# deevinandu/Distributed-Multi-Agent-SLAM-Swarm-Robotics-System

Measured on NVIDIA B200. Metric: beam_cell_updates_per_sec, higher is better.
Workload: dtype f64+u32

## Files before the change

distributed-multi-agent-slam-swarm-robotics-system_b200/_native.py:

```python
from __future__ import annotations

import ctypes as C
import os
import subprocess

PKG_DIR = os.path.dirname(os.path.abspath(__file__))
CSRC = os.path.join(PKG_DIR, 'csrc')
LIB_PATH = os.path.join(PKG_DIR, 'liboccgrid_b200.so')
SOURCES = ['occgrid_integrate.cu', 'occgrid_tiled.cu', 'occgrid_route.cu', 'occgrid_band.cu', 'mapmerge.cu', 'frontier.cu', 'icp.cu', 'render.cu', 'map_fuse.cu', 'frontier_assign.cu', 'slam_chain.cpp']
HEADERS = ['common.cuh', 'beam_expand.cuh', 'block_ops.cuh', 'sincos_dd.cuh', os.path.join('..', '..', 'include', 'occgrid_b200.h')]

STRATEGY = {'auto': -1, 'global_atomic': 0, 'tiled': 1}
COUNTER_NAMES = ('packets', 'accepted', 'dropped', 'bad_pose', 'beams', 'hits', 'updates', 'slowpath',
                 'owned_updates', 'records')
N_COUNTERS = 16


class OccGridError(RuntimeError):
    pass


class Geom(C.Structure):
    _fields_ = [('ox', C.c_double), ('oy', C.c_double), ('res', C.c_double),
                ('size_x', C.c_int32), ('size_y', C.c_int32),
                ('win_x0', C.c_int32), ('win_y0', C.c_int32),
                ('win_w', C.c_int32), ('win_h', C.c_int32)]


class RouteJob(C.Structure):
    _fields_ = [('d_packets', C.c_void_p), ('n', C.c_int64), ('stride', C.c_int32), ('rec_len', C.c_int32),
                ('d_agent_idx', C.c_void_p), ('d_drift', C.c_void_p), ('d_agent_off', C.c_void_p), ('n_agents', C.c_int32),
                ('ordinal_base', C.c_uint32), ('ox', C.c_double), ('oy', C.c_double), ('res', C.c_double),
                ('size_x', C.c_int32), ('n_bands', C.c_int32), ('src_rank', C.c_int32), ('band_y0', C.c_int32 * 33),
                ('d_peer_recs', C.c_void_p), ('d_peer_tiles', C.c_void_p), ('seg_capacity', C.c_int64), ('d_resv', C.c_void_p), ('d_status', C.c_void_p),
                ('d_counters', C.c_void_p)]


class BandCtx(C.Structure):
    _fields_ = [('band_geom', Geom), ('n_bands', C.c_int32), ('rank', C.c_int32), ('seg_capacity', C.c_int64),
                ('d_recv', C.c_void_p * 2), ('d_recv_tiles', C.c_void_p * 2), ('d_seg_counts', C.c_void_p * 2),
                ('d_peer_recs', C.c_void_p * 2), ('d_peer_tiles', C.c_void_p * 2), ('d_peer_seg_counts', C.c_void_p * 2),
                ('d_peer_flags', C.c_void_p), ('d_my_flags', C.c_void_p), ('d_resv', C.c_void_p), ('d_status', C.c_void_p),
                ('d_grid', C.c_void_p), ('d_workspace', C.c_void_p), ('workspace_bytes', C.c_size_t), ('d_counters', C.c_void_p),
                ('ev_fused', C.c_void_p), ('ev_published', C.c_void_p), ('published_pending', C.c_int32)]


def _stale():
    if not os.path.exists(LIB_PATH):
        return True
    t = os.path.getmtime(LIB_PATH)
    deps = [os.path.join(CSRC, s) for s in SOURCES + HEADERS]
    return any(os.path.exists(d) and os.path.getmtime(d) > t for d in deps)


def build(force=False, verbose=False):
    if not force and not _stale():
        return LIB_PATH
    srcs = [os.path.join(CSRC, s) for s in SOURCES if os.path.exists(os.path.join(CSRC, s))]
    cmd = ['nvcc', '-gencode', 'arch=compute_100a,code=sm_100a', '-O3', '-lineinfo', '-std=c++17',
           '-Xcompiler', '-fPIC', '-Xcompiler', '-ffp-contract=off', '-shared', '-o', LIB_PATH] + srcs
    if verbose:
        cmd.insert(1, '-Xptxas=-v')
    r = subprocess.run(cmd, capture_output=True, text=True)
    if r.returncode != 0:
        raise OccGridError('nvcc failed:\n' + r.stdout + r.stderr)
    if verbose:
        print(r.stderr)
    return LIB_PATH


_lib = None


def lib():
    global _lib
    if _lib is not None:
        return _lib
    if not os.path.exists(LIB_PATH):
        raise OccGridError(f'{LIB_PATH} is missing: run `python -c "import __graft_entry__ as g; g.build()"` '
                           '(needs nvcc).  There is no CPU fallback.')
    L = C.CDLL(LIB_PATH)
    vp, i64, i32, u32, sz = C.c_void_p, C.c_int64, C.c_int, C.c_uint32, C.c_size_t
    gp = C.POINTER(Geom)
    L.occgrid_abi_version.restype = i32
    L.occgrid_last_error.restype = C.c_char_p
    L.occgrid_workspace_bytes.restype = sz
    L.occgrid_workspace_bytes.argtypes = [gp, i64, i32]
    L.occgrid_workspace_reset.restype = i32
    L.occgrid_workspace_reset.argtypes = [vp, sz, vp]
    L.occgrid_integrate_packets.restype = i32
    L.occgrid_integrate_packets.argtypes = [gp, vp, i64, i32, i32, vp, vp, vp, i32, vp, vp, sz, vp, i32, vp]
    L.occgrid_agent_maps_workspace_bytes.restype = sz
    L.occgrid_agent_maps_workspace_bytes.argtypes = [gp, i32, i64, i32]
    L.occgrid_integrate_packets_agent_maps.restype = i32
    L.occgrid_integrate_packets_agent_maps.argtypes = [gp, vp, i64, i32, i32, vp, vp, vp, i32, vp, vp, sz, vp, i32, vp]
    L.occgrid_update_rays.restype = i32
    L.occgrid_update_rays.argtypes = [gp, vp, vp, i64, vp, vp, sz, vp, i32, vp]
    L.occgrid_scatter_probe.restype = i32
    L.occgrid_scatter_probe.argtypes = [i32, vp, i64, i64, u32, vp]
    L.occgrid_route_workspace_bytes.restype = sz
    L.occgrid_route_workspace_bytes.argtypes = [i64, i32]
    L.occgrid_route_packets.restype = i32
    L.occgrid_route_packets.argtypes = [gp, i32, vp, vp, i64, i32, i32, vp, vp, vp, i32, vp, i64, vp, vp, vp,
                                        vp, sz, vp]
    L.occgrid_integrate_poses.restype = i32
    L.occgrid_integrate_poses.argtypes = [gp, vp, i64, i32, vp, vp, sz, vp, i32, vp]
    L.occgrid_band_workspace_bytes.restype = sz
    L.occgrid_band_workspace_bytes.argtypes = [gp, i32, i64]
    L.occgrid_band_prepare.restype = i32
    L.occgrid_band_prepare.argtypes = [gp, vp, vp, i32, i64, vp, vp, sz, vp, vp]
    L.occgrid_band_raycast_route.restype = i32
    L.occgrid_band_raycast_route.argtypes = [gp, vp, i32, i64, i32, C.POINTER(RouteJob), vp, vp, sz, vp, vp]
    L.occgrid_band_step.restype = i32
    L.occgrid_band_step.argtypes = [C.POINTER(BandCtx), i64, i32, C.POINTER(RouteJob), i32, vp, vp]
    L.occgrid_band_join.restype = i32
    L.occgrid_band_join.argtypes = [C.POINTER(BandCtx), vp]
    L.occgrid_band_publish.restype = i32
    L.occgrid_band_publish.argtypes = [i32, i32, vp, i64, vp, vp, vp, u32, i32, vp, vp]
    L.occgrid_frontier_workspace_bytes.restype = sz
    L.occgrid_frontier_workspace_bytes.argtypes = [i64, i64]
    L.occgrid_frontiers.restype = i32
    L.occgrid_frontiers.argtypes = [vp, i32, i32, vp, i64, vp, vp, vp, sz, vp]
    L.occgrid_frontier_clusters.restype = i32
    L.occgrid_frontier_clusters.argtypes = [vp, vp, i64, i32, i32, C.c_double, C.c_double, C.c_double, vp, vp, vp, vp, vp,
                                            vp, sz, vp]
    L.occgrid_render_overlay.restype = i32
    L.occgrid_render_overlay.argtypes = [vp, i32, i32, C.c_double, C.c_double, C.c_double, C.c_double, C.c_double, C.c_double,
                                         i32, i32, vp, vp, vp, vp]
    L.occgrid_set_raycast_ctas_per_sm.restype = i32
    L.occgrid_set_raycast_ctas_per_sm.argtypes = [i32]
    L.occgrid_profile_begin.restype = i32
    L.occgrid_profile_end.restype = i32
    L.occgrid_profile_end.argtypes = [vp, vp, i32]
    _bind_merge(L)
    _lib = L
    return L


def _bind_merge(L):
    vp, i64, i32, sz, dbl = C.c_void_p, C.c_int64, C.c_int32, C.c_size_t, C.c_double
    L.mapmerge_count_occupied.restype = C.c_int
    L.mapmerge_count_occupied.argtypes = [vp, i64, vp, vp]
    L.mapmerge_extract_workspace_bytes.restype = sz
    L.mapmerge_extract_workspace_bytes.argtypes = [i64]
    L.mapmerge_extract_transform.restype = C.c_int
    L.mapmerge_extract_transform.argtypes = [vp, i32, i32, dbl, dbl, dbl, vp, vp, vp, i64, vp, vp, vp, vp, sz, vp]
    L.mapmerge_extract_batch_workspace_bytes.restype = sz
    L.mapmerge_extract_batch_workspace_bytes.argtypes = [i64, i32]
    L.mapmerge_extract_batch_count.restype = C.c_int
    L.mapmerge_extract_batch_count.argtypes = [vp, i32, i32, i32, vp, vp, sz, i32, vp]
    L.mapmerge_extract_batch_write.restype = C.c_int
    L.mapmerge_extract_batch_write.argtypes = [vp, i32, i32, i32, dbl, vp, vp, vp, vp, vp, vp, i64, vp, vp, vp, vp, sz, vp]
    L.mapmerge_append_slice.restype = C.c_int
    L.mapmerge_append_slice.argtypes = [vp, vp, vp, i32, vp, vp, i64, vp, vp, vp, vp]
    L.mapmerge_bounds_workspace_bytes.restype = sz
    L.mapmerge_bounds.restype = C.c_int
    L.mapmerge_bounds.argtypes = [vp, vp, vp, vp, vp, sz, vp]
    L.mapmerge_voxel_workspace_bytes.restype = sz
    L.mapmerge_voxel_workspace_bytes.argtypes = [i64, i64]
    L.mapmerge_voxel_downsample.restype = C.c_int
    L.mapmerge_voxel_downsample.argtypes = [vp, vp, vp, i64, dbl, vp, vp, i64, vp, vp, vp, vp, vp, sz, vp]
    L.mapmerge_bounds_enc_reset.restype = C.c_int
    L.mapmerge_bounds_enc_reset.argtypes = [vp, vp]
    L.mapmerge_chain_workspace_bytes.restype = sz
    L.mapmerge_chain_workspace_bytes.argtypes = [vp, i32]
    L.mapmerge_chain_init.restype = C.c_int
    L.mapmerge_chain_init.argtypes = [vp, sz, vp, i32, vp, vp, vp, vp, i32, vp, vp, vp, vp]
    L.mapmerge_chain_run.restype = C.c_int
    L.mapmerge_chain_run.argtypes = [vp, vp, i32, i32, i32, vp, vp, vp, dbl, vp, vp, i64, vp, vp, vp]
    L.mapmerge_chain_poll.restype = C.c_int
    L.mapmerge_chain_poll.argtypes = [vp, vp, i32, vp, vp]
    L.mapmerge_chain_rebounds.restype = C.c_int
    L.mapmerge_chain_rebounds.argtypes = [vp, vp, i32, vp, vp, vp, vp]
    L.mapmerge_chain_rebuild.restype = C.c_int
    L.mapmerge_chain_rebuild.argtypes = [vp, vp, i32, vp, vp, vp, i32, dbl, vp, vp, i64, vp, vp, vp, vp, vp, vp, sz, i64, vp]
    L.mapmerge_icp_workspace_bytes.restype = sz
    L.mapmerge_icp_workspace_bytes.argtypes = [i64, i64, i32, i32]
    L.mapmerge_icp_register.restype = C.c_int
    L.mapmerge_icp_register.argtypes = [vp, vp, i64, vp, vp, i64, dbl, dbl, dbl, i32, i32, dbl, i32, dbl, dbl, vp, vp, sz, vp]
    L.occgrid_slam_create.restype = vp
    L.occgrid_slam_create.argtypes = []
    L.occgrid_slam_destroy.restype = None
    L.occgrid_slam_destroy.argtypes = [vp]
    L.occgrid_slam_drift_table.restype = C.c_int
    L.occgrid_slam_drift_table.argtypes = [vp, vp, i64, i32, i32, vp, dbl, vp]
    L.occgrid_slam_counts.restype = C.c_int
    L.occgrid_slam_counts.argtypes = [vp, vp, vp, vp]
    L.occgrid_slam_closures.restype = C.c_int
    L.occgrid_slam_closures.argtypes = [vp, i64, vp, vp, vp, vp]
    L.occgrid_slam_correction_for_agent.restype = C.c_int
    L.occgrid_slam_correction_for_agent.argtypes = [vp, i32, vp]
    L.occgrid_accumulate_packets.restype = C.c_int
    L.occgrid_accumulate_packets.argtypes = [C.POINTER(Geom), vp, i64, i32, i32, vp, vp, vp, i32, vp, vp, sz, vp, i32, vp]
    L.occgrid_counts_to_logodds.restype = C.c_int
    L.occgrid_counts_to_logodds.argtypes = [vp, i64, dbl, dbl, dbl, dbl, vp, vp]
    L.mapmerge_rasterise.restype = C.c_int
    L.mapmerge_rasterise.argtypes = [vp, vp, vp, dbl, vp, i32, i32, vp, vp]
    L.mapmerge_fuse_max.restype = C.c_int
    L.mapmerge_fuse_max.argtypes = [vp, vp, i64, vp]
    L.mapmerge_warp_fuse_workspace_bytes.restype = sz
    L.mapmerge_warp_fuse_workspace_bytes.argtypes = [C.c_int, i32, i32]
    L.mapmerge_warp_fuse.restype = C.c_int
    L.mapmerge_warp_fuse.argtypes = [vp, C.c_int, i32, i32, dbl, vp, vp, dbl, dbl, dbl, i32, i32, vp, vp, sz, vp]
    L.occgrid_frontier_assign_workspace_bytes.restype = sz
    L.occgrid_frontier_assign_workspace_bytes.argtypes = [i32, i32, i32, i32, i64]
    L.occgrid_frontier_assign.restype = C.c_int
    L.occgrid_frontier_assign.argtypes = [vp, i32, i32, dbl, dbl, dbl, vp, i32, vp, vp, vp, vp, vp, vp, i32, i64,
                                          vp, vp, vp, vp, vp, vp, vp, vp, sz, vp]
    L.occgrid_geodesic_field.restype = C.c_int
    L.occgrid_geodesic_field.argtypes = [vp, i32, i32, dbl, dbl, dbl, vp, i64, vp, vp, vp, vp, sz, vp]


KERNEL_NAMES = ('integrate_global', 'resolve', 'update_rays', 'tile_count', 'tile_scan', 'tile_scatter',
                'tile_raycast', 'tile_resolve', 'merge_extract', 'merge_bounds', 'merge_voxel', 'merge_raster',
                'merge_fuse', 'probe', 'route', 'frontier', 'frontier_cluster', 'chain_probe', 'chain_incremental',
                'chain_rebuild', 'icp', 'band_barrier', 'render', 'merge_scan', 'merge_warp_fuse', 'frontier_assign')


def profile_begin():
    check(lib().occgrid_profile_begin(), 'occgrid_profile_begin')


def profile_end():
    n = len(KERNEL_NAMES)
    ms = (C.c_double * n)()
    cnt = (C.c_int64 * n)()
    check(lib().occgrid_profile_end(ms, cnt, n), 'occgrid_profile_end')
    return {KERNEL_NAMES[i]: (ms[i], cnt[i]) for i in range(n) if cnt[i]}


def check(rc, what):
    if rc != 0:
        msg = lib().occgrid_last_error().decode('utf-8', 'replace')
        raise OccGridError(f'{what} failed (rc={rc}): {msg}')


def last_error():
    return lib().occgrid_last_error().decode('utf-8', 'replace')
```

distributed-multi-agent-slam-swarm-robotics-system_b200/csrc/common.cuh:

```cuda
#pragma once
#include <cuda_runtime.h>
#include <stdarg.h>
#include <stdint.h>
#include <stdio.h>

#include "../../include/occgrid_b200.h"
#include "beam_expand.cuh"
#include "block_ops.cuh"

namespace occ {

void set_last_error(const char* fmt, ...);
bool cuda_ok(cudaError_t e, const char* what);

#define OCC_CUDA_TRY(call)                                  \
    do {                                                    \
        if (!occ::cuda_ok((call), #call)) return OCCGRID_E_CUDA; \
    } while (0)

inline Geom to_geom(const occgrid_geom* g) {
    Geom o;
    o.ox = g->ox; o.oy = g->oy; o.res = g->res; o.inv_res = 1.0 / g->res;
    o.size_x = g->size_x; o.size_y = g->size_y;
    o.win_x0 = g->win_x0; o.win_y0 = g->win_y0; o.win_w = g->win_w; o.win_h = g->win_h;
    return o;
}

int validate_geom(const occgrid_geom* g);

int device_sm_count();

struct __align__(16) PoseRec {
    double rx, ry;
    float yaw;
    float d[4];
    unsigned int k;
    int tile;
    unsigned int pad;
};
static_assert(sizeof(PoseRec) == 48, "PoseRec must be 48 bytes");

enum KernelId { K_INTEGRATE_GLOBAL = 0, K_RESOLVE, K_UPDATE_RAYS, K_TILE_COUNT, K_TILE_SCAN, K_TILE_SCATTER,
                K_TILE_RAYCAST, K_TILE_RESOLVE, K_MERGE_EXTRACT, K_MERGE_BOUNDS, K_MERGE_VOXEL, K_MERGE_RASTER,
                K_MERGE_FUSE, K_PROBE, K_ROUTE, K_FRONTIER, K_FRONTIER_CLUSTER, K_CHAIN_PROBE, K_CHAIN_INCR,
                K_CHAIN_REBUILD, K_ICP, K_BAND_BARRIER, K_RENDER, K_MERGE_SCAN, K_MERGE_WARP_FUSE, K_FRONTIER_ASSIGN, K_N_KERNELS };
bool profile_enabled();
void profile_mark(int kernel_id, cudaStream_t st, bool begin, int n_kernels);

struct ProfileScope {
    int id; cudaStream_t st; bool on; int nk;
    ProfileScope(int id_, cudaStream_t st_, int n_kernels = 1) : id(id_), st(st_), on(profile_enabled()), nk(n_kernels) {
        if (on) profile_mark(id, st, true, nk);
    }
    ~ProfileScope() { if (on) profile_mark(id, st, false, nk); }
};

inline size_t align_up(size_t v, size_t a) { return (v + a - 1) / a * a; }

constexpr int kMaxRecStride = 64;

struct PacketBatch {
    const uint8_t* pkts; int64_t n; int stride;
    const int32_t* agent_idx; const double* drift; const double* agent_off; int n_agents;
};

enum class Output { kGrid, kAgentMaps, kCounts };

int check_packet_batch(const PacketBatch& b, int rec_len, const char* who);

__device__ __forceinline__ void stage_records(const uint8_t* __restrict__ src, size_t bytes, uint8_t* smem) {
    const size_t nvec = ((reinterpret_cast<uintptr_t>(src) & 15) == 0) ? bytes / 16 : 0;
    const uint4* s4 = reinterpret_cast<const uint4*>(src);
    uint4* d4 = reinterpret_cast<uint4*>(smem);
    for (size_t i = threadIdx.x; i < nvec; i += blockDim.x) d4[i] = __ldg(s4 + i);
    for (size_t i = nvec * 16 + threadIdx.x; i < bytes; i += blockDim.x) smem[i] = __ldg(src + i);
}

constexpr int kTile = 64;
constexpr int kTileShift = 6;

__host__ __device__ __forceinline__ int reach_cells(double res) { return (int)ceil(OCC_MAX_DIST_M / res) + 2; }

struct TileGeom {
    int reach;
    int pad;
    int tiles_x, tiles_y, n_tiles;
    int win_side;
    int pitch;
};

inline TileGeom tile_geom(double res, int win_w, int win_h) {
    TileGeom t;
    t.reach = reach_cells(res);
    t.pad = ((t.reach + kTile - 1) / kTile) * kTile;
    t.tiles_x = (win_w + 2 * t.pad + kTile - 1) >> kTileShift;
    t.tiles_y = (win_h + 2 * t.pad + kTile - 1) >> kTileShift;
    t.n_tiles = t.tiles_x * t.tiles_y;
    t.win_side = kTile + 2 * t.reach;
    t.pitch = t.win_side | 1;
    return t;
}
inline TileGeom tile_geom(const occgrid_geom* g) { return tile_geom(g->res, g->win_w, g->win_h); }

constexpr int kSegChunk = 2048;
constexpr int kRouteItemPk = 512;
constexpr int kRouteSubsPerItem = 2;
constexpr int kMaxBands = 32;

struct SegInfo {
    int n_segs;
    unsigned int seg_cap;
    const unsigned int* d_counts;
    unsigned int host_count;
};

struct RouteJob {
    const uint8_t* pkts; long long n; int stride;
    const int32_t* agent_idx; const double* drift; const double* agent_off; int n_agents;
    unsigned int ordinal_base;
    double ox, oy, res, inv_res;
    int size_x;
    int reach, pad, tiles_x;
    int n_bands, src_rank;
    int band_y0[kMaxBands + 1];
    PoseRec* const* peer_recs;
    int* const* peer_tiles;
    unsigned int seg_cap;
    unsigned int* resv;
    int* status;
    uint64_t* counters;
    unsigned int n_route_items;
};

bool tiled_supported(const occgrid_geom* geom, int n_maps);
size_t tiled_workspace_bytes(const occgrid_geom* geom, int n_maps, int64_t max_packets);
int integrate_tiled(const occgrid_geom* geom, const PacketBatch& batch, const PoseRec* d_poses, int ordinals_in_records, Output kind,
                    void* d_out, void* d_ws, size_t ws_bytes, uint64_t* d_counters, cudaStream_t st);
void set_raycast_cta_cap(int cap);
size_t tiled_band_workspace_bytes(const occgrid_geom* geom, int n_segs, int64_t seg_cap);
int tiled_prepare_poses(const occgrid_geom* geom, const PoseRec* d_recs, const int* d_tiles, const SegInfo& seg, int tiles_in_records,
                        void* d_ws, size_t ws_bytes, uint64_t* d_counters, cudaStream_t st);
int tiled_raycast_route(const occgrid_geom* geom, const PoseRec* d_recs, int have_items, const RouteJob* job,
                        int8_t* d_grid, void* d_ws, size_t ws_bytes, int64_t max_records, uint64_t* d_counters, cudaStream_t st,
                        cudaEvent_t after_fused = nullptr);

template <int N>
__device__ __forceinline__ void block_add_counters(const unsigned long long (&v)[N],
                                                   unsigned long long* smem_acc , uint64_t* d_counters) {
    if (d_counters == nullptr) return;
    const int lane = threadIdx.x & 31, warp = threadIdx.x >> 5, nwarps = (blockDim.x + 31) >> 5;
#pragma unroll
    for (int i = 0; i < N; ++i) {
        unsigned long long x = v[i];
#pragma unroll
        for (int o = 16; o > 0; o >>= 1) x += __shfl_xor_sync(0xffffffffu, x, o);
        if (lane == 0) smem_acc[i * 32 + warp] = x;
    }
    __syncthreads();
    if (threadIdx.x < N) {
        unsigned long long t = 0;
        for (int w = 0; w < nwarps; ++w) t += smem_acc[threadIdx.x * 32 + w];
        if (t) atomicAdd(reinterpret_cast<unsigned long long*>(d_counters) + threadIdx.x, t);
    }
}

}
```

distributed-multi-agent-slam-swarm-robotics-system_b200/csrc/mapmerge.cu:

```cuda
#include <cstddef>
#include <vector>

#include "common.cuh"

namespace occ {

constexpr int kMT = 256;
constexpr int kLoadCells = 16;
constexpr int kCellsPerThread = 64;
constexpr int kChunk = kMT * kCellsPerThread;

enum { ST_POINT_OVERFLOW = 1, ST_LATTICE_OVERFLOW = 2, ST_CHAIN_ABORTED = 4 };

struct Xform { double m[16]; int identity; };


__device__ __forceinline__ unsigned int occupied_mask16(const int8_t* __restrict__ grid, long long base, long long n) {
    unsigned int mask = 0;
    if (base + 16 <= n && ((reinterpret_cast<uintptr_t>(grid + base) & 15) == 0)) {
        const int4 v = __ldg(reinterpret_cast<const int4*>(grid + base));
        const int w[4] = {v.x, v.y, v.z, v.w};
#pragma unroll
        for (int i = 0; i < 4; ++i)
#pragma unroll
            for (int b = 0; b < 4; ++b)
                if ((int8_t)((w[i] >> (8 * b)) & 0xff) > 50) mask |= 1u << (4 * i + b);
    } else {
        for (int i = 0; i < 16 && base + i < n; ++i)
            if (grid[base + i] > 50) mask |= 1u << i;
    }
    return mask;
}

__device__ __forceinline__ unsigned long long occupied_mask64(const int8_t* __restrict__ grid, long long base, long long n) {
    unsigned int m[4];
#pragma unroll
    for (int q = 0; q < 4; ++q) m[q] = occupied_mask16(grid, base + 16 * q, n);
    return (unsigned long long)m[0] | ((unsigned long long)m[1] << 16) | ((unsigned long long)m[2] << 32) |
           ((unsigned long long)m[3] << 48);
}

__global__ void __launch_bounds__(kMT)
k_extract_count(const int8_t* __restrict__ grid, long long n_cells, unsigned int* __restrict__ block_counts) {
    __shared__ unsigned int s_warp[33];
    const long long base = ((long long)blockIdx.x * kMT + threadIdx.x) * kCellsPerThread;
    unsigned int c = base < n_cells ? __popcll(occupied_mask64(grid, base, n_cells)) : 0u;
    unsigned int total;
    block_exclusive_scan(c, s_warp, &total);
    if (threadIdx.x == 0) block_counts[blockIdx.x] = total;
}

__global__ void __launch_bounds__(kMT)
k_count_occupied(const int8_t* __restrict__ grid, long long n_cells, long long* __restrict__ out) {
    unsigned int c = 0;
    for (long long base = ((long long)blockIdx.x * kMT + threadIdx.x) * kLoadCells; base < n_cells;
         base += (long long)gridDim.x * kMT * kLoadCells)
        c += __popc(occupied_mask16(grid, base, n_cells));
#pragma unroll
    for (int o = 16; o > 0; o >>= 1) c += __shfl_xor_sync(0xffffffffu, c, o);
    if ((threadIdx.x & 31) == 0 && c) atomicAdd(reinterpret_cast<unsigned long long*>(out), (unsigned long long)c);
}

__global__ void __launch_bounds__(1024)
k_extract_reserve(unsigned int* __restrict__ block_counts, int n_blocks, long long* __restrict__ d_count,
                  long long capacity, long long* __restrict__ ws_base, int* __restrict__ status,
                  long long* __restrict__ d_last_appended) {
    const unsigned long long sum = cta_scan_in_place<1>(block_counts, n_blocks, 0ull);
    if (threadIdx.x == 0) {
        const long long base = *d_count;
        long long total = (long long)sum;
        if (base + total > capacity) { atomicOr(status, ST_POINT_OVERFLOW); total = 0; }
        ws_base[0] = base;
        ws_base[1] = total;
        *d_count = base + total;
        if (d_last_appended) *d_last_appended = total;
    }
}

__global__ void __launch_bounds__(kMT)
k_extract_write(const int8_t* __restrict__ grid, long long n_cells, int width, double res, double origin_x,
                double origin_y, Xform T, const unsigned int* __restrict__ block_offsets,
                const long long* __restrict__ ws_base, double* __restrict__ px, double* __restrict__ py) {
    __shared__ unsigned int s_warp[33];
    if (ws_base[1] == 0) return;
    const long long base = ((long long)blockIdx.x * kMT + threadIdx.x) * kCellsPerThread;
    const unsigned long long mask = base < n_cells ? occupied_mask64(grid, base, n_cells) : 0ull;
    unsigned int total;
    unsigned int off = block_exclusive_scan(__popcll(mask), s_warp, &total);
    long long dst = ws_base[0] + block_offsets[blockIdx.x] + off;
    unsigned long long m = mask;
    while (m) {
        const int i = __ffsll((long long)m) - 1;
        m &= m - 1;
        const long long c = base + i;
        const long long row = c / width, col = c - row * width;
        double x = OCC_DADD(OCC_DMUL((double)col, res), origin_x);
        double y = OCC_DADD(OCC_DMUL((double)row, res), origin_y);
        if (!T.identity) {
            const double w = OCC_DADD(OCC_DADD(OCC_DMUL(T.m[12], x), OCC_DMUL(T.m[13], y)), T.m[15]);
            const double tx = OCC_DADD(OCC_DADD(OCC_DMUL(T.m[0], x), OCC_DMUL(T.m[1], y)), T.m[3]);
            const double ty = OCC_DADD(OCC_DADD(OCC_DMUL(T.m[4], x), OCC_DMUL(T.m[5], y)), T.m[7]);
            if (w == 1.0) { x = tx; y = ty; }
            else { x = OCC_DDIV(tx, w); y = OCC_DDIV(ty, w); }
        }
        px[dst] = x;
        py[dst] = y;
        ++dst;
    }
}

__device__ __forceinline__ double warp_min(double v) {
#pragma unroll
    for (int o = 16; o > 0; o >>= 1) v = fmin(v, __shfl_xor_sync(0xffffffffu, v, o));
    return v;
}
__device__ __forceinline__ double warp_max(double v) {
#pragma unroll
    for (int o = 16; o > 0; o >>= 1) v = fmax(v, __shfl_xor_sync(0xffffffffu, v, o));
    return v;
}

template <class F>
__device__ __forceinline__ void block_min_max(double mnx, double mny, double mxx, double mxy, F&& use) {
    __shared__ double s_b[4][32];
    mnx = warp_min(mnx); mny = warp_min(mny); mxx = warp_max(mxx); mxy = warp_max(mxy);
    const int lane = threadIdx.x & 31, warp = threadIdx.x >> 5;
    if (lane == 0) { s_b[0][warp] = mnx; s_b[1][warp] = mny; s_b[2][warp] = mxx; s_b[3][warp] = mxy; }
    __syncthreads();
    if (threadIdx.x == 0) {
        for (int w = 1; w < (int)(blockDim.x >> 5); ++w) {
            mnx = fmin(mnx, s_b[0][w]); mny = fmin(mny, s_b[1][w]); mxx = fmax(mxx, s_b[2][w]); mxy = fmax(mxy, s_b[3][w]);
        }
        use(mnx, mny, mxx, mxy);
    }
}

__device__ __forceinline__ unsigned long long enc_double(double d) {
    const unsigned long long u = (unsigned long long)__double_as_longlong(d);
    return (u & 0x8000000000000000ull) ? ~u : (u | 0x8000000000000000ull);
}
__device__ __forceinline__ double dec_double(unsigned long long k) {
    const unsigned long long u = (k & 0x8000000000000000ull) ? (k & 0x7fffffffffffffffull) : ~k;
    return __longlong_as_double((long long)u);
}

__device__ __forceinline__ void block_bounds_atomic(double mnx, double mny, double mxx, double mxy,
                                                    unsigned long long* __restrict__ benc) {
    block_min_max(mnx, mny, mxx, mxy, [&](double x0, double y0, double x1, double y1) {
        if (x0 <= x1) {
            atomicMin(&benc[0], enc_double(x0)); atomicMin(&benc[1], enc_double(y0));
            atomicMax(&benc[2], enc_double(x1)); atomicMax(&benc[3], enc_double(y1));
        }
    });
}

__global__ void k_benc_reset(unsigned long long* __restrict__ benc) {
    benc[0] = benc[1] = enc_double(INFINITY);
    benc[2] = benc[3] = enc_double(-INFINITY);
}

struct BatchXform { double m[6]; double w[3]; int identity; int use; };

__global__ void __launch_bounds__(kMT)
k_batch_count(const int8_t* const* __restrict__ grids, long long n_cells, int blocks_per_grid,
              unsigned int* __restrict__ block_counts ,
              unsigned long long* __restrict__ masks ) {
    __shared__ unsigned int s_warp[33];
    const int a = blockIdx.y;
    const long long base = ((long long)blockIdx.x * kMT + threadIdx.x) * kCellsPerThread;
    const unsigned long long mask = base < n_cells ? occupied_mask64(grids[a], base, n_cells) : 0ull;
    masks[((size_t)a * blocks_per_grid + blockIdx.x) * kMT + threadIdx.x] = mask;
    unsigned int total;
    block_exclusive_scan(__popcll(mask), s_warp, &total);
    if (threadIdx.x == 0) block_counts[(size_t)a * blocks_per_grid + blockIdx.x] = total;
}

constexpr int kScanStages = 4;
constexpr int kScanCtasPerSm = 3;
constexpr int kScanStageBytes = kChunk;

__device__ __forceinline__ unsigned int smem_u32(const void* p) { return (unsigned int)__cvta_generic_to_shared(p); }

__device__ __forceinline__ void mbar_init(unsigned long long* bar, unsigned int count) {
    asm volatile("mbarrier.init.shared::cta.b64 [%0], %1;" ::"r"(smem_u32(bar)), "r"(count) : "memory");
}
__device__ __forceinline__ void mbar_expect_tx(unsigned long long* bar, unsigned int bytes) {
    asm volatile("mbarrier.arrive.expect_tx.shared::cta.b64 _, [%0], %1;" ::"r"(smem_u32(bar)), "r"(bytes) : "memory");
}
__device__ __forceinline__ void mbar_wait(unsigned long long* bar, unsigned int parity) {
    asm volatile(
        "{\n\t.reg .pred p;\n\t"
        "WAIT_%=:\n\t"
        "mbarrier.try_wait.parity.shared::cta.b64 p, [%0], %1;\n\t"
        "@p bra DONE_%=;\n\t"
        "bra WAIT_%=;\n\t"
        "DONE_%=:\n\t}" ::"r"(smem_u32(bar)), "r"(parity) : "memory");
}
__device__ __forceinline__ void bulk_load(void* smem_dst, const void* gmem_src, unsigned int bytes, unsigned long long* bar) {
    asm volatile("cp.async.bulk.shared::cluster.global.mbarrier::complete_tx::bytes [%0], [%1], %2, [%3];"
                 ::"r"(smem_u32(smem_dst)), "l"(gmem_src), "r"(bytes), "r"(smem_u32(bar)) : "memory");
}

__device__ __forceinline__ unsigned int occupied_bits16(uint4 v) {
    const unsigned int w[4] = {v.x, v.y, v.z, v.w};
    unsigned int bits = 0;
#pragma unroll
    for (int i = 0; i < 4; ++i) {
        const unsigned int gt = __vcmpgts4(w[i], 0x32323232u) & 0x80808080u;
        bits |= (((gt >> 7) * 0x00204081u) >> 21 & 0xfu) << (4 * i);
    }
    return bits;
}

__global__ void __launch_bounds__(kMT)
k_batch_count_tma(const int8_t* const* __restrict__ grids, long long n_cells, int blocks_per_grid, int n_agents,
                  unsigned int* __restrict__ block_counts, unsigned long long* __restrict__ masks) {
    extern __shared__ __align__(128) unsigned char s_stage[];
    __shared__ __align__(8) unsigned long long s_full[kScanStages];
    __shared__ unsigned int s_cnt[kScanStages];
    const long long total = (long long)n_agents * blocks_per_grid;
    auto chunk_of = [&](long long i) { return (long long)blockIdx.x + i * gridDim.x; };
    auto issue = [&](long long i) {
        const long long c = chunk_of(i);
        if (c >= total) return;
        const int a = (int)(c / blocks_per_grid), blk = (int)(c - (long long)a * blocks_per_grid);
        const long long base = (long long)blk * kChunk;
        const unsigned int bytes = (unsigned int)min((long long)kChunk, n_cells - base);
        const int st = (int)(i % kScanStages);
        mbar_expect_tx(&s_full[st], bytes);
        bulk_load(s_stage + (size_t)st * kScanStageBytes, grids[a] + base, bytes, &s_full[st]);
    };
    if (threadIdx.x == 0) {
        for (int s = 0; s < kScanStages; ++s) mbar_init(&s_full[s], 1);
        asm volatile("fence.mbarrier_init.release.cluster;" ::: "memory");
        asm volatile("fence.proxy.async.shared::cta;" ::: "memory");
    }
    if (threadIdx.x < kScanStages) s_cnt[threadIdx.x] = 0u;
    __syncthreads();
    if (threadIdx.x == 0)
        for (int i = 0; i < kScanStages; ++i) issue(i);
    for (long long i = 0; chunk_of(i) < total; ++i) {
        const long long c = chunk_of(i);
        const int st = (int)(i % kScanStages);
        const int a = (int)(c / blocks_per_grid), blk = (int)(c - (long long)a * blocks_per_grid);
        const long long base = (long long)blk * kChunk;
        const int valid = (int)min((long long)kChunk, n_cells - base);
        mbar_wait(&s_full[st], (unsigned int)((i / kScanStages) & 1));
        const uint4* src = reinterpret_cast<const uint4*>(s_stage + (size_t)st * kScanStageBytes) + threadIdx.x * 4;
        unsigned long long mask = 0ull;
#pragma unroll
        for (int q = 0; q < 4; ++q)
            if ((int)threadIdx.x * kCellsPerThread + 16 * q < valid)
                mask |= (unsigned long long)occupied_bits16(src[q]) << (16 * q);
        masks[((size_t)a * blocks_per_grid + blk) * kMT + threadIdx.x] = mask;
        unsigned int n = __popcll(mask);
#pragma unroll
        for (int o = 16; o > 0; o >>= 1) n += __shfl_xor_sync(0xffffffffu, n, o);
        if ((threadIdx.x & 31) == 0 && n) atomicAdd(&s_cnt[st], n);
        __syncthreads();
        if (threadIdx.x == 0) {
            block_counts[(size_t)a * blocks_per_grid + blk] = s_cnt[st];
            s_cnt[st] = 0u;
            issue(i + kScanStages);
        }
    }
}

__global__ void __launch_bounds__(1024)
k_batch_scan(unsigned int* __restrict__ block_counts, int blocks_per_grid, long long* __restrict__ agent_total) {
    const unsigned long long total = cta_scan_in_place<1>(block_counts + (size_t)blockIdx.x * blocks_per_grid, blocks_per_grid, 0ull);
    if (threadIdx.x == 0) agent_total[blockIdx.x] = (long long)total;
}

__global__ void __launch_bounds__(1024)
k_batch_offsets(const long long* __restrict__ agent_total, const BatchXform* __restrict__ T, int n_agents,
                long long capacity, long long* __restrict__ agent_offset, int* __restrict__ status) {
    __shared__ unsigned long long s_warp[33];
    __shared__ long long s_carry;
    if (threadIdx.x == 0) s_carry = 0;
    __syncthreads();
    for (int start = 0; start < n_agents; start += blockDim.x) {
        const int a = start + threadIdx.x;
        const unsigned long long v = (a < n_agents && T[a].use) ? (unsigned long long)agent_total[a] : 0ull;
        unsigned long long total;
        const unsigned long long ex = block_exclusive_scan(v, s_warp, &total);
        if (a < n_agents) agent_offset[a] = s_carry + (long long)ex;
        __syncthreads();
        if (threadIdx.x == 0) s_carry += (long long)total;
        __syncthreads();
    }
    if (threadIdx.x == 0) {
        agent_offset[n_agents] = s_carry;
        if (s_carry > capacity) atomicOr(status, ST_POINT_OVERFLOW);
    }
}

__global__ void __launch_bounds__(kMT)
k_batch_write(const unsigned long long* __restrict__ masks, long long n_cells, int width, double res,
              const double* __restrict__ origins , const BatchXform* __restrict__ T, int blocks_per_grid,
              const unsigned int* __restrict__ block_offsets, const long long* __restrict__ agent_offset, long long capacity,
              double* __restrict__ px, double* __restrict__ py) {
    __shared__ unsigned int s_warp[33];
    __shared__ unsigned short s_cell[kChunk];
    const int a = blockIdx.y;
    const BatchXform t = T[a];
    if (!t.use || agent_offset[gridDim.y] > capacity) return;
    const long long chunk_base = (long long)blockIdx.x * kChunk;
    const unsigned long long mask = masks[((size_t)a * blocks_per_grid + blockIdx.x) * kMT + threadIdx.x];
    unsigned int total;
    unsigned int off = block_exclusive_scan(__popcll(mask), s_warp, &total);
    unsigned long long m = mask;
    while (m) {
        const int i = __ffsll((long long)m) - 1;
        m &= m - 1;
        s_cell[off++] = (unsigned short)(threadIdx.x * kCellsPerThread + i);
    }
    __syncthreads();
    const long long dst0 = agent_offset[a] + block_offsets[(size_t)a * blocks_per_grid + blockIdx.x];
    const double ox = origins[2 * a], oy = origins[2 * a + 1];
    for (unsigned int i = threadIdx.x; i < total; i += kMT) {
        const long long c = chunk_base + s_cell[i];
        long long row, col;
        if (n_cells <= 0x7fffffffll) { row = (int)c / width; col = (int)c - (int)row * width; }
        else { row = c / width; col = c - row * width; }
        double x = OCC_DADD(OCC_DMUL((double)col, res), ox);
        double y = OCC_DADD(OCC_DMUL((double)row, res), oy);
        if (!t.identity) {
            const double w = OCC_DADD(OCC_DADD(OCC_DMUL(t.w[0], x), OCC_DMUL(t.w[1], y)), t.w[2]);
            const double tx = OCC_DADD(OCC_DADD(OCC_DMUL(t.m[0], x), OCC_DMUL(t.m[1], y)), t.m[2]);
            const double ty = OCC_DADD(OCC_DADD(OCC_DMUL(t.m[3], x), OCC_DMUL(t.m[4], y)), t.m[5]);
            if (w == 1.0) { x = tx; y = ty; }
            else { x = OCC_DDIV(tx, w); y = OCC_DDIV(ty, w); }
        }
        px[dst0 + i] = x;
        py[dst0 + i] = y;
    }
}

__global__ void __launch_bounds__(kMT)
k_append_slice(const double* __restrict__ sx, const double* __restrict__ sy, const long long* __restrict__ agent_offset, int a,
               double* __restrict__ px, double* __restrict__ py, long long capacity, long long* __restrict__ d_count,
               int* __restrict__ status, unsigned long long* __restrict__ benc) {
    const long long b = agent_offset[a], e = agent_offset[a + 1];
    const long long n0 = *d_count;
    const long long k = e - b;
    if (n0 + k > capacity) { if (blockIdx.x == 0 && threadIdx.x == 0) atomicOr(status, ST_POINT_OVERFLOW); return; }
    double mnx = INFINITY, mny = INFINITY, mxx = -INFINITY, mxy = -INFINITY;
    for (long long i = (long long)blockIdx.x * kMT + threadIdx.x; i < k; i += (long long)gridDim.x * kMT) {
        const double x = sx[b + i], y = sy[b + i];
        px[n0 + i] = x;
        py[n0 + i] = y;
        mnx = fmin(mnx, x); mxx = fmax(mxx, x); mny = fmin(mny, y); mxy = fmax(mxy, y);
    }
    if (benc) block_bounds_atomic(mnx, mny, mxx, mxy, benc);
}

__global__ void k_bump_count(const long long* __restrict__ agent_offset, int a, long long capacity, long long* __restrict__ d_count) {
    const long long k = agent_offset[a + 1] - agent_offset[a];
    if (*d_count + k <= capacity) *d_count += k;
}


__global__ void __launch_bounds__(kMT)
k_bounds_partial(const double* __restrict__ px, const double* __restrict__ py, const long long* __restrict__ d_count,
                 double* __restrict__ partial ) {
    const long long n = *d_count;
    double mnx = INFINITY, mny = INFINITY, mxx = -INFINITY, mxy = -INFINITY;
    for (long long i = (long long)blockIdx.x * kMT + threadIdx.x; i < n; i += (long long)gridDim.x * kMT) {
        const double x = px[i], y = py[i];
        mnx = fmin(mnx, x); mxx = fmax(mxx, x);
        mny = fmin(mny, y); mxy = fmax(mxy, y);
    }
    block_min_max(mnx, mny, mxx, mxy, [&](double x0, double y0, double x1, double y1) {
        partial[blockIdx.x * 4 + 0] = x0; partial[blockIdx.x * 4 + 1] = y0;
        partial[blockIdx.x * 4 + 2] = x1; partial[blockIdx.x * 4 + 3] = y1;
    });
}

__global__ void __launch_bounds__(kMT)
k_bounds_final(const double* __restrict__ partial, int n_partial, double* __restrict__ bounds) {
    double mnx = INFINITY, mny = INFINITY, mxx = -INFINITY, mxy = -INFINITY;
    for (int i = threadIdx.x; i < n_partial; i += kMT) {
        mnx = fmin(mnx, partial[i * 4 + 0]); mny = fmin(mny, partial[i * 4 + 1]);
        mxx = fmax(mxx, partial[i * 4 + 2]); mxy = fmax(mxy, partial[i * 4 + 3]);
    }
    block_min_max(mnx, mny, mxx, mxy, [&](double x0, double y0, double x1, double y1) {
        bounds[0] = x0; bounds[1] = y0; bounds[2] = x1; bounds[3] = y1;
    });
}


struct VoxelHeader {
    double mbx, mby;
    long long nx, ny, cells;
    long long n_points;
    unsigned int total_slots, total_voxels;
};

__global__ void k_voxel_setup(const double* __restrict__ bounds_in, unsigned long long* __restrict__ benc,
                              const long long* __restrict__ d_count, double voxel,
                              long long capacity_cells, long long point_capacity, VoxelHeader* __restrict__ hdr,
                              int* __restrict__ status) {
    const long long n = *d_count;
    double bounds[4];
    if (benc) {
        for (int j = 0; j < 4; ++j) bounds[j] = dec_double(benc[j]);
        benc[0] = benc[1] = enc_double(INFINITY);
        benc[2] = benc[3] = enc_double(-INFINITY);
    } else {
        for (int j = 0; j < 4; ++j) bounds[j] = bounds_in[j];
    }
    VoxelHeader h;
    h.n_points = n;
    h.total_slots = h.total_voxels = 0;
    h.mbx = OCC_DADD(bounds[0], -OCC_DMUL(voxel, 0.5));
    h.mby = OCC_DADD(bounds[1], -OCC_DMUL(voxel, 0.5));
    if (n <= 0) { h.nx = h.ny = h.cells = 0; h.n_points = 0; *hdr = h; return; }
    h.nx = (long long)floor(OCC_DDIV(OCC_DADD(bounds[2], -h.mbx), voxel)) + 1;
    h.ny = (long long)floor(OCC_DDIV(OCC_DADD(bounds[3], -h.mby), voxel)) + 1;
    h.cells = h.nx * h.ny;
    if (h.nx <= 0 || h.ny <= 0 || h.cells > capacity_cells || h.cells >= 0xffffffffll || n > point_capacity ||
        n >= 0xfffffff0ll) {
        atomicOr(status, n > point_capacity ? ST_POINT_OVERFLOW : ST_LATTICE_OVERFLOW);
        h.cells = 0; h.n_points = 0;
    }
    *hdr = h;
}

constexpr unsigned int kSingle = 0xffffffffu;

__global__ void __launch_bounds__(kMT)
k_voxel_mark(const double* __restrict__ px, const double* __restrict__ py, double voxel,
             const VoxelHeader* __restrict__ hdr, uint2* __restrict__ lattice, unsigned int* __restrict__ key) {
    const long long n = hdr->n_points;
    const double mbx = hdr->mbx, mby = hdr->mby;
    const long long nx = hdr->nx;
    for (long long i = (long long)blockIdx.x * kMT + threadIdx.x; i < n; i += (long long)gridDim.x * kMT) {
        const long long ix = (long long)floor(OCC_DDIV(OCC_DADD(px[i], -mbx), voxel));
        const long long iy = (long long)floor(OCC_DDIV(OCC_DADD(py[i], -mby), voxel));
        const unsigned int k = (unsigned int)(iy * nx + ix);
        key[i] = k;
        atomicMax(&lattice[k].x, 0xffffffffu - (unsigned int)i);
        atomicAdd(&lattice[k].y, 1u);
    }
}

__global__ void __launch_bounds__(kMT)
k_voxel_gather(const VoxelHeader* __restrict__ hdr, uint2* __restrict__ lattice, const unsigned int* __restrict__ key,
               unsigned int* __restrict__ head, unsigned int* __restrict__ hcnt) {
    const long long n = hdr->n_points;
    for (long long i = (long long)blockIdx.x * kMT + threadIdx.x; i < n; i += (long long)gridDim.x * kMT) {
        const unsigned int k = key[i];
        const uint2 v = lattice[k];
        if (v.y == 1u) {
            head[i] = kSingle;
            hcnt[i] = 1u;
            lattice[k] = make_uint2(0u, 0u);
            continue;
        }
        const unsigned int h = 0xffffffffu - v.x;
        head[i] = h;
        hcnt[i] = (h == (unsigned int)i) ? v.y : 0u;
    }
}

constexpr int kScanItems = 8;
constexpr int kScanChunk = kMT * kScanItems;

__global__ void __launch_bounds__(kMT)
k_pscan_partial(const VoxelHeader* __restrict__ hdr, const unsigned int* __restrict__ hcnt, uint2* __restrict__ block_sums) {
    __shared__ unsigned int s_warp[33];
    const long long n = hdr->n_points;
    const long long nblocks = (n + kScanChunk - 1) / kScanChunk;
    for (long long b = blockIdx.x; b < nblocks; b += gridDim.x) {
        const long long base = b * kScanChunk + (long long)threadIdx.x * kScanItems;
        unsigned int s = 0, f = 0;
#pragma unroll
        for (int j = 0; j < kScanItems; ++j) {
            const unsigned int c = (base + j < n) ? hcnt[base + j] : 0u;
            s += c; f += c ? 1u : 0u;
        }
        unsigned int ts, tf;
        block_exclusive_scan(s, s_warp, &ts);
        block_exclusive_scan(f, s_warp, &tf);
        if (threadIdx.x == 0) block_sums[b] = make_uint2(ts, tf);
    }
}

__global__ void __launch_bounds__(1024)
k_pscan_top(uint2* __restrict__ block_sums, VoxelHeader* __restrict__ hdr) {
    __shared__ unsigned int s_warp[33];
    __shared__ unsigned int s_c0, s_c1;
    const long long n = hdr->n_points;
    const long long nblocks = (n + kScanChunk - 1) / kScanChunk;
    if (threadIdx.x == 0) { s_c0 = 0; s_c1 = 0; }
    __syncthreads();
    for (long long start = 0; start < nblocks; start += blockDim.x) {
        const long long i = start + threadIdx.x;
        const uint2 v = i < nblocks ? block_sums[i] : make_uint2(0u, 0u);
        unsigned int t0, t1;
        const unsigned int e0 = block_exclusive_scan(v.x, s_warp, &t0);
        const unsigned int e1 = block_exclusive_scan(v.y, s_warp, &t1);
        if (i < nblocks) block_sums[i] = make_uint2(s_c0 + e0, s_c1 + e1);
        __syncthreads();
        if (threadIdx.x == 0) { s_c0 += t0; s_c1 += t1; }
        __syncthreads();
    }
    if (threadIdx.x == 0) { hdr->total_slots = s_c0; hdr->total_voxels = s_c1; }
}

__global__ void __launch_bounds__(kMT)
k_pscan_apply(const VoxelHeader* __restrict__ hdr, const unsigned int* __restrict__ hcnt,
              const uint2* __restrict__ block_sums, unsigned int* __restrict__ vrank, unsigned int* __restrict__ soff) {
    __shared__ unsigned int s_warp[33];
    const long long n = hdr->n_points;
    const long long nblocks = (n + kScanChunk - 1) / kScanChunk;
    for (long long b = blockIdx.x; b < nblocks; b += gridDim.x) {
        const long long base = b * kScanChunk + (long long)threadIdx.x * kScanItems;
        unsigned int c[kScanItems];
        unsigned int s = 0, f = 0;
#pragma unroll
        for (int j = 0; j < kScanItems; ++j) {
            c[j] = (base + j < n) ? hcnt[base + j] : 0u;
            s += c[j]; f += c[j] ? 1u : 0u;
        }
        unsigned int ts, tf;
        unsigned int es = block_exclusive_scan(s, s_warp, &ts);
        unsigned int ef = block_exclusive_scan(f, s_warp, &tf);
        const uint2 carry = block_sums[b];
        es += carry.x;
        ef += carry.y;
#pragma unroll
        for (int j = 0; j < kScanItems; ++j) {
            if (c[j]) { vrank[base + j] = ef; soff[base + j] = es; }
            es += c[j];
            ef += c[j] ? 1u : 0u;
        }
    }
}

__global__ void __launch_bounds__(kMT)
k_voxel_fill(const VoxelHeader* __restrict__ hdr, const unsigned int* __restrict__ key, uint2* __restrict__ lattice,
             const unsigned int* __restrict__ head, const unsigned int* __restrict__ soff, unsigned int* __restrict__ slots) {
    const long long n = hdr->n_points;
    for (long long i = (long long)blockIdx.x * kMT + threadIdx.x; i < n; i += (long long)gridDim.x * kMT) {
        const unsigned int h = head[i];
        if (h == kSingle) continue;
        const unsigned int k = key[i];
        const unsigned int r = atomicSub(&lattice[k].y, 1u) - 1u;
        if (r == 0u) lattice[k].x = 0u;
        slots[soff[h] + r] = (unsigned int)i;
    }
}

__global__ void __launch_bounds__(kMT)
k_voxel_reduce(const double* __restrict__ px, const double* __restrict__ py, const VoxelHeader* __restrict__ hdr,
               const unsigned int* __restrict__ hcnt, const unsigned int* __restrict__ vrank,
               const unsigned int* __restrict__ soff, const unsigned int* __restrict__ slots,
               double* __restrict__ out_x, double* __restrict__ out_y, long long* __restrict__ out_count,
               unsigned long long* __restrict__ benc) {
    const long long n = hdr->n_points;
    if (blockIdx.x == 0 && threadIdx.x == 0) *out_count = (long long)hdr->total_voxels;
    double mnx = INFINITY, mny = INFINITY, mxx = -INFINITY, mxy = -INFINITY;
    for (long long i = (long long)blockIdx.x * kMT + threadIdx.x; i < n; i += (long long)gridDim.x * kMT) {
        const unsigned int c = hcnt[i];
        if (c == 0u) continue;
        double sx = px[i], sy = py[i];
        if (c > 1u) {
            const unsigned int b = soff[i], e = b + c;
            long long last = i;
            for (unsigned int r = b + 1; r < e; ++r) {
                unsigned int best = 0xffffffffu;
                for (unsigned int q = b; q < e; ++q) {
                    const unsigned int idx = slots[q];
                    if ((long long)idx > last && idx < best) best = idx;
                }
                last = best;
                sx = OCC_DADD(sx, px[best]);
                sy = OCC_DADD(sy, py[best]);
            }
        }
        const double cnt = (double)c;
        const double ox_ = OCC_DDIV(sx, cnt), oy_ = OCC_DDIV(sy, cnt);
        out_x[vrank[i]] = ox_;
        out_y[vrank[i]] = oy_;
        mnx = fmin(mnx, ox_); mxx = fmax(mxx, ox_); mny = fmin(mny, oy_); mxy = fmax(mxy, oy_);
    }
    if (benc) block_bounds_atomic(mnx, mny, mxx, mxy, benc);
}


struct ChainHeader {
    VoxelHeader v;
    double mbx, mby;
    unsigned long long gb_enc[4];
    unsigned long long gb2_enc[4];
    int have_lattice, force_rebuild, bounds_dirty;
    int stalled;
    int cursor;
    int aborted;
};
enum { CHAIN_RUN = 0, CHAIN_REBUILD = 1, CHAIN_OVERFLOW = 2, CHAIN_REBOUND = 3, CHAIN_ABORTED = 4 };

__device__ __forceinline__ bool voxel_key_of(double x, double y, double mbx, double mby, double voxel, long long W,
                                             long long H, unsigned int* key) {
    const long long ix = (long long)floor(OCC_DDIV(OCC_DADD(x, -mbx), voxel));
    const long long iy = (long long)floor(OCC_DDIV(OCC_DADD(y, -mby), voxel));
    if (ix < 0 || iy < 0 || ix >= W || iy >= H) return false;
    *key = (unsigned int)(iy * W + ix);
    return true;
}

__device__ __forceinline__ int chain_decide(const ChainHeader* h, const unsigned long long* sb , double voxel,
                                            long long W, long long H, double* nmbx, double* nmby) {
    const unsigned long long g0 = __ldcg(&h->gb_enc[0]), g1 = __ldcg(&h->gb_enc[1]), g2 = __ldcg(&h->gb_enc[2]), g3 = __ldcg(&h->gb_enc[3]);
    const int dirty = __ldcg(&h->bounds_dirty), have = __ldcg(&h->have_lattice), force = __ldcg(&h->force_rebuild);
    const double hmbx = __ldcg(&h->mbx), hmby = __ldcg(&h->mby);
    const double b0 = fmin(dec_double(g0), dec_double(sb[0]));
    const double b1 = fmin(dec_double(g1), dec_double(sb[1]));
    const double b2 = fmax(dec_double(g2), dec_double(sb[2]));
    const double b3 = fmax(dec_double(g3), dec_double(sb[3]));
    *nmbx = OCC_DADD(b0, -OCC_DMUL(voxel, 0.5));
    *nmby = OCC_DADD(b1, -OCC_DMUL(voxel, 0.5));
    if (dirty) return CHAIN_REBOUND;
    const long long nx = (long long)floor(OCC_DDIV(OCC_DADD(b2, -*nmbx), voxel)) + 1;
    const long long ny = (long long)floor(OCC_DDIV(OCC_DADD(b3, -*nmby), voxel)) + 1;
    if (!(nx > 0 && ny > 0 && nx <= W && ny <= H)) return CHAIN_OVERFLOW;
    if (!have || force || *nmbx != hmbx || *nmby != hmby) return CHAIN_REBUILD;
    return CHAIN_RUN;
}

__global__ void k_chain_reset(ChainHeader* __restrict__ h) {
    h->gb_enc[0] = h->gb_enc[1] = h->gb2_enc[0] = h->gb2_enc[1] = enc_double(INFINITY);
    h->gb_enc[2] = h->gb_enc[3] = h->gb2_enc[2] = h->gb2_enc[3] = enc_double(-INFINITY);
    h->have_lattice = h->force_rebuild = 0;
    h->bounds_dirty = 1;
    h->stalled = 0;
    h->cursor = 0;
    h->aborted = 0;
}

__global__ void k_chain_slice_bounds_init(unsigned long long* __restrict__ slice_benc, int n_agents) {
    for (int a = blockIdx.x * blockDim.x + threadIdx.x; a < n_agents; a += gridDim.x * blockDim.x) {
        slice_benc[4 * a + 0] = slice_benc[4 * a + 1] = enc_double(INFINITY);
        slice_benc[4 * a + 2] = slice_benc[4 * a + 3] = enc_double(-INFINITY);
    }
}
__global__ void __launch_bounds__(kMT)
k_chain_slice_bounds(const double* __restrict__ sx, const double* __restrict__ sy, const long long* __restrict__ agent_offset,
                     unsigned long long* __restrict__ slice_benc) {
    const int a = blockIdx.y;
    const long long b = agent_offset[a], e = agent_offset[a + 1];
    if (b + (long long)blockIdx.x * kMT >= e) return;
    double mnx = INFINITY, mny = INFINITY, mxx = -INFINITY, mxy = -INFINITY;
    for (long long i = b + (long long)blockIdx.x * kMT + threadIdx.x; i < e; i += (long long)gridDim.x * kMT) {
        const double x = sx[i], y = sy[i];
        mnx = fmin(mnx, x); mxx = fmax(mxx, x); mny = fmin(mny, y); mxy = fmax(mxy, y);
    }
    block_bounds_atomic(mnx, mny, mxx, mxy, slice_benc + 4 * a);
}

struct ChainRun {
    ChainHeader* h;
    const int* order;
    int n_order, n_callbacks;
    const long long* agent_offset;
    const unsigned long long* slice_benc;
    const double* sx;
    const double* sy;
    double voxel;
    long long W, H;
    uint2* LM;
    unsigned int *lkey, *next, *gkey, *flag, *blockcount;
    double *gx, *gy, *resx, *resy;
    long long* d_count;
    long long capacity;
    int* status;
    unsigned int* bar;
    int bc_stride;
};

__device__ __forceinline__ void chain_link(const ChainRun& p, long long b, long long n, double mbx, double mby) {
    for (long long j = (long long)blockIdx.x * kMT + threadIdx.x; j < n; j += (long long)gridDim.x * kMT) {
        unsigned int k = 0;
        voxel_key_of(p.sx[b + j], p.sy[b + j], mbx, mby, p.voxel, p.W, p.H, &k);
        p.lkey[j] = k;
        p.next[j] = atomicExch(&p.LM[k].y, (unsigned int)j + 1u);
    }
}

__device__ __forceinline__ void chain_fold(const ChainRun& p, long long b, long long n, double mbx, double mby,
                                           unsigned int* bc) {
    ChainHeader* h = p.h;
    const double g0 = dec_double(h->gb_enc[0]), g1 = dec_double(h->gb_enc[1]);
    double mnx = INFINITY, mny = INFINITY, mxx = -INFINITY, mxy = -INFINITY;
    const int lane = threadIdx.x & 31;
    for (long long j0 = (long long)blockIdx.x * kMT + (threadIdx.x & ~31); j0 < n; j0 += (long long)gridDim.x * kMT) {
        const long long j = j0 + lane;
        int parked = -1;
        unsigned int k = 0;
        uint2 e = make_uint2(0u, 0u);
        if (j < n) { k = p.lkey[j]; e = p.LM[k]; }
        if (j < n && e.y == (unsigned int)j + 1u) {
            unsigned int cnt = 0, head = (unsigned int)j;
            for (unsigned int q = e.y; q; q = p.next[q - 1]) { ++cnt; head = min(head, q - 1u); }
            double ax, ay;
            long long last;
            unsigned int remaining, total;
            if (e.x) { ax = p.gx[e.x - 1]; ay = p.gy[e.x - 1]; last = -1; remaining = cnt; total = cnt + 1u; }
            else     { ax = p.sx[b + head]; ay = p.sy[b + head]; last = head; remaining = cnt - 1u; total = cnt; }
            for (unsigned int r = 0; r < remaining; ++r) {
                unsigned int best = 0xffffffffu;
                for (unsigned int q = e.y; q; q = p.next[q - 1]) {
                    const unsigned int idx = q - 1u;
                    if ((long long)idx > last && idx < best) best = idx;
                }
                last = best;
                ax = OCC_DADD(ax, p.sx[b + best]);
                ay = OCC_DADD(ay, p.sy[b + best]);
            }
            const double c = (double)total;
            const double x = OCC_DDIV(ax, c), y = OCC_DDIV(ay, c);
            if (e.x) {
                const unsigned int g = e.x - 1u;
                const double oldx = p.gx[g], oldy = p.gy[g];
                if ((oldx <= g0 && x > oldx) || (oldy <= g1 && y > oldy)) h->bounds_dirty = 1;
                p.gx[g] = x; p.gy[g] = y;
                unsigned int k2 = 0;
                if (!voxel_key_of(x, y, mbx, mby, p.voxel, p.W, p.H, &k2) || k2 != k) h->force_rebuild = 1;
                mnx = fmin(mnx, x); mxx = fmax(mxx, x); mny = fmin(mny, y); mxy = fmax(mxy, y);
            } else {
                p.resx[head] = x; p.resy[head] = y;
                p.flag[head] = 1u;
                parked = (int)(head / kMT);
            }
            p.LM[k].y = 0u;
        }
        __syncwarp();
        const unsigned int peers = __match_any_sync(0xffffffffu, parked);
        if (parked >= 0 && lane == __ffs(peers) - 1) atomicAdd(&bc[parked], (unsigned int)__popc(peers));
    }
    block_bounds_atomic(mnx, mny, mxx, mxy, h->gb_enc);
}

__device__ __forceinline__ unsigned int chain_append(const ChainRun& p, long long n, long long n_g, double mbx, double mby,
                                                     const unsigned int* bc, unsigned int* s_warp) {
    ChainHeader* h = p.h;
    const unsigned int nb = (unsigned int)((n + kMT - 1) / kMT);
    double mnx = INFINITY, mny = INFINITY, mxx = -INFINITY, mxy = -INFINITY;
    unsigned int all = 0;
    for (unsigned int c0 = 0; c0 < nb; c0 += gridDim.x) {
        const unsigned int chunk = c0 + blockIdx.x;
        unsigned int part = 0, whole = 0;
        for (unsigned int q = threadIdx.x; q < nb; q += kMT) {
            const unsigned int v = bc[q];
            if (q < chunk) part += v;
            whole += v;
        }
        unsigned int before;
        block_exclusive_scan(part, s_warp, &before);
        if (c0 == 0) block_exclusive_scan(whole, s_warp, &all);
        const long long j = (long long)chunk * kMT + threadIdx.x;
        const unsigned int f = (chunk < nb && j < n) ? p.flag[j] : 0u;
        unsigned int mine;
        const unsigned int pos = block_exclusive_scan(f, s_warp, &mine);
        if (f) {
            p.flag[j] = 0u;
            const long long idx = n_g + before + pos;
            if (idx >= p.capacity) {
                atomicOr(p.status, ST_POINT_OVERFLOW);
            } else {
                const double x = p.resx[j], y = p.resy[j];
                p.gx[idx] = x; p.gy[idx] = y;
                unsigned int k = 0;
                if (!voxel_key_of(x, y, mbx, mby, p.voxel, p.W, p.H, &k)) { p.gkey[idx] = 0xffffffffu; h->force_rebuild = 1; }
                else {
                    p.gkey[idx] = k;
                    if (atomicExch(&p.LM[k].x, (unsigned int)idx + 1u) != 0u) h->force_rebuild = 1;
                }
                mnx = fmin(mnx, x); mxx = fmax(mxx, x); mny = fmin(mny, y); mxy = fmax(mxy, y);
            }
        }
    }
    block_bounds_atomic(mnx, mny, mxx, mxy, h->gb_enc);
    return all;
}

__global__ void __launch_bounds__(kMT)
k_chain_persistent(const ChainRun p) {
    __shared__ unsigned int s_warp[33];
    ChainHeader* h = p.h;
    unsigned int target = 0;
    int done = 0;
    bool alive = true;
    if (!h->stalled) {
        int cur = h->cursor;
        long long n_g = *p.d_count;
        const double mbx = h->mbx, mby = h->mby;
        bool linked = false;
        if (p.n_callbacks > 0 && cur < p.n_order) {
            const int agent = p.order[cur];
            double nmbx, nmby;
            const int need = chain_decide(h, p.slice_benc + 4 * agent, p.voxel, p.W, p.H, &nmbx, &nmby);
            if (need != CHAIN_RUN) {
                if (blockIdx.x == 0 && threadIdx.x == 0) {
                    h->stalled = need;
                    if (need == CHAIN_OVERFLOW) atomicOr(p.status, ST_LATTICE_OVERFLOW);
                }
            } else {
                const long long b = p.agent_offset[agent];
                chain_link(p, b, p.agent_offset[agent + 1] - b, mbx, mby);
                alive = grid_barrier(p.bar, target, &h->aborted);
                linked = alive;
            }
        }
        for (int it = 0; linked; ++it) {
            const int agent = p.order[cur];
            const long long b = p.agent_offset[agent], n = p.agent_offset[agent + 1] - b;
            unsigned int* bc = p.blockcount + (size_t)(it & 1) * p.bc_stride;
            unsigned int* bc_other = p.blockcount + (size_t)((it & 1) ^ 1) * p.bc_stride;
            if (blockIdx.x == 0 && it > 0)
                for (int q = threadIdx.x; q < p.bc_stride; q += kMT) bc_other[q] = 0u;
            chain_fold(p, b, n, mbx, mby, bc);
            if (!(alive = grid_barrier(p.bar, target, &h->aborted))) break;
            const unsigned int added = chain_append(p, n, n_g, mbx, mby, bc, s_warp);
            n_g += added;
            if (n_g > p.capacity) n_g = p.capacity;
            cur += 1;
            done = it + 1;
            if (blockIdx.x == 0 && threadIdx.x == 0) { *p.d_count = n_g; h->cursor = cur; }
            const bool more = it + 1 < p.n_callbacks && cur < p.n_order;
            int next_agent = 0;
            long long nb = 0, nn = 0;
            if (more) {
                next_agent = p.order[cur];
                nb = p.agent_offset[next_agent];
                nn = p.agent_offset[next_agent + 1] - nb;
                chain_link(p, nb, nn, mbx, mby);
            }
            int need = CHAIN_RUN;
            alive = grid_barrier(p.bar, target, &h->aborted, &need, [&] {
                if (!more) return (int)CHAIN_RUN;
                double ax, ay;
                return chain_decide(h, p.slice_benc + 4 * next_agent, p.voxel, p.W, p.H, &ax, &ay);
            });
            if (!alive || !more) break;
            if (need != CHAIN_RUN) {
                for (long long j = (long long)blockIdx.x * kMT + threadIdx.x; j < nn; j += (long long)gridDim.x * kMT)
                    p.LM[p.lkey[j]].y = 0u;
                if (blockIdx.x == 0 && threadIdx.x == 0) {
                    h->stalled = need;
                    if (need == CHAIN_OVERFLOW) atomicOr(p.status, ST_LATTICE_OVERFLOW);
                }
                break;
            }
        }
    }
    if (!alive) {
        if (threadIdx.x == 0) { h->stalled = CHAIN_ABORTED; atomicOr(p.status, ST_CHAIN_ABORTED); }
        return;
    }
    if (blockIdx.x == 0 && done)
        for (int q = threadIdx.x; q < p.bc_stride; q += kMT) p.blockcount[(size_t)((done - 1) & 1) * p.bc_stride + q] = 0u;
    __syncthreads();
    if (threadIdx.x == 0) {
        __threadfence();
        if (atomicAdd(p.bar + 1, 1u) == gridDim.x - 1) { p.bar[0] = 0u; p.bar[1] = 0u; p.bar[2] = 0u; p.bar[3] = 0u; }
    }
}

__global__ void __launch_bounds__(kMT)
k_chain_rebounds(const double* __restrict__ gx, const double* __restrict__ gy, const long long* __restrict__ n_ptr,
                 ChainHeader* __restrict__ h) {
    const long long n = *n_ptr;
    double mnx = INFINITY, mny = INFINITY, mxx = -INFINITY, mxy = -INFINITY;
    for (long long i = (long long)blockIdx.x * kMT + threadIdx.x; i < n; i += (long long)gridDim.x * kMT) {
        const double x = gx[i], y = gy[i];
        mnx = fmin(mnx, x); mxx = fmax(mxx, x); mny = fmin(mny, y); mxy = fmax(mxy, y);
    }
    block_bounds_atomic(mnx, mny, mxx, mxy, h->gb2_enc);
}
__global__ void k_chain_rebounds_apply(ChainHeader* __restrict__ h) {
    h->gb_enc[0] = h->gb2_enc[0]; h->gb_enc[1] = h->gb2_enc[1];
    h->gb_enc[2] = max(h->gb_enc[2], h->gb2_enc[2]); h->gb_enc[3] = max(h->gb_enc[3], h->gb2_enc[3]);
    h->gb2_enc[0] = h->gb2_enc[1] = enc_double(INFINITY);
    h->gb2_enc[2] = h->gb2_enc[3] = enc_double(-INFINITY);
    h->bounds_dirty = 0;
    if (h->stalled == CHAIN_REBOUND) h->stalled = CHAIN_RUN;
}

__global__ void __launch_bounds__(kMT)
k_chain_lm_clear(ChainHeader* __restrict__ h, uint2* __restrict__ LM, const unsigned int* __restrict__ gkey,
                 const long long* __restrict__ d_count) {
    if (!h->have_lattice) return;
    const long long n = *d_count;
    for (long long i = (long long)blockIdx.x * kMT + threadIdx.x; i < n; i += (long long)gridDim.x * kMT) {
        const unsigned int k = gkey[i];
        if (k != 0xffffffffu) LM[k] = make_uint2(0u, 0u);
    }
}

__global__ void k_chain_rebuild_hdr(ChainHeader* __restrict__ h, const unsigned long long* __restrict__ slice_benc, int agent,
                                    const long long* __restrict__ d_count, double voxel, long long W, long long H,
                                    long long point_capacity, int* __restrict__ status) {
    double nmbx, nmby;
    const int dirty = h->bounds_dirty;
    h->bounds_dirty = 0;
    int need = chain_decide(h, slice_benc + 4 * agent, voxel, W, H, &nmbx, &nmby);
    h->bounds_dirty = dirty;
    long long n = *d_count;
    if (n > point_capacity || n >= 0x7ffffff0ll) { atomicOr(status, ST_POINT_OVERFLOW); n = 0; }
    if (need == CHAIN_OVERFLOW) { atomicOr(status, ST_LATTICE_OVERFLOW); n = 0; }
    h->v.mbx = nmbx; h->v.mby = nmby;
    h->v.nx = W; h->v.ny = H; h->v.cells = W * H;
    h->v.n_points = n;
    h->v.total_slots = h->v.total_voxels = 0;
    h->force_rebuild = 0;
    h->gb_enc[0] = h->gb_enc[1] = enc_double(INFINITY);
    h->gb_enc[2] = h->gb_enc[3] = enc_double(-INFINITY);
}

__global__ void __launch_bounds__(kMT)
k_chain_lm_build(ChainHeader* __restrict__ h, const double* __restrict__ gx, const double* __restrict__ gy,
                 const long long* __restrict__ d_count, double voxel, uint2* __restrict__ LM, unsigned int* __restrict__ gkey) {
    const long long n = *d_count;
    const double mbx = h->v.mbx, mby = h->v.mby;
    const long long W = h->v.nx, H = h->v.ny;
    for (long long i = (long long)blockIdx.x * kMT + threadIdx.x; i < n; i += (long long)gridDim.x * kMT) {
        unsigned int k;
        if (!voxel_key_of(gx[i], gy[i], mbx, mby, voxel, W, H, &k)) { gkey[i] = 0xffffffffu; h->force_rebuild = 1; continue; }
        gkey[i] = k;
        if (atomicExch(&LM[k].x, (unsigned int)i + 1u) != 0u) h->force_rebuild = 1;
    }
}

__global__ void k_chain_rebuild_done(ChainHeader* __restrict__ h) {
    h->mbx = h->v.mbx; h->mby = h->v.mby;
    h->have_lattice = 1;
    h->bounds_dirty = 0;
    h->stalled = CHAIN_RUN;
    h->cursor += 1;
}


__global__ void __launch_bounds__(kMT)
k_raster_fill(int8_t* __restrict__ grid, long long n) {
    const long long n16 = ((reinterpret_cast<uintptr_t>(grid) & 15) == 0) ? n / 16 : 0;
    int4* g4 = reinterpret_cast<int4*>(grid);
    const int4 v = make_int4(-1, -1, -1, -1);
    for (long long i = (long long)blockIdx.x * kMT + threadIdx.x; i < n16; i += (long long)gridDim.x * kMT) g4[i] = v;
    for (long long i = n16 * 16 + (long long)blockIdx.x * kMT + threadIdx.x; i < n; i += (long long)gridDim.x * kMT) grid[i] = -1;
}

__global__ void __launch_bounds__(kMT)
k_raster_scatter(const double* __restrict__ px, const double* __restrict__ py, const long long* __restrict__ d_count,
                 const double* __restrict__ bounds, double res, int width, int height, int8_t* __restrict__ grid) {
    const long long n = *d_count;
    const double min_x = bounds[0], min_y = bounds[1];
    for (long long i = (long long)blockIdx.x * kMT + threadIdx.x; i < n; i += (long long)gridDim.x * kMT) {
        long long xi = (long long)OCC_DDIV(OCC_DADD(px[i], -min_x), res);
        long long yi = (long long)OCC_DDIV(OCC_DADD(py[i], -min_y), res);
        xi = xi < 0 ? 0 : (xi > width - 1 ? width - 1 : xi);
        yi = yi < 0 ? 0 : (yi > height - 1 ? height - 1 : yi);
        grid[yi * width + xi] = OCCGRID_CELL_OCCUPIED;
    }
}

__global__ void __launch_bounds__(kMT)
k_fuse_max(int8_t* __restrict__ dst, const int8_t* __restrict__ src, long long n) {
    for (long long i = (long long)blockIdx.x * kMT + threadIdx.x; i < n; i += (long long)gridDim.x * kMT) {
        const int8_t a = dst[i], b = src[i];
        dst[i] = a > b ? a : b;
    }
}

static int grid_for(long long work_items) {
    long long b = (work_items + kMT - 1) / kMT;
    if (b < 1) b = 1;
    if (b > device_sm_count() * 16) b = device_sm_count() * 16;
    return (int)b;
}

}

using namespace occ;

extern "C" {

int mapmerge_count_occupied(const int8_t* d_grid, int64_t n_cells, int64_t* d_out, void* stream) {
    if (!d_grid || !d_out || n_cells < 0) { set_last_error("mapmerge_count_occupied: bad arguments"); return OCCGRID_E_ARG; }
    if (n_cells == 0) return OCCGRID_OK;
    cudaStream_t st = (cudaStream_t)stream;
    ProfileScope ps(K_MERGE_EXTRACT, st, 1);
    k_count_occupied<<<grid_for(n_cells / kLoadCells + 1), kMT, 0, st>>>(d_grid, n_cells, (long long*)d_out);
    OCC_CUDA_TRY(cudaGetLastError());
    return OCCGRID_OK;
}

size_t mapmerge_extract_workspace_bytes(int64_t n_cells) {
    const int64_t blocks = (n_cells + kChunk - 1) / kChunk;
    return align_up((size_t)blocks * sizeof(unsigned int), 256) + 256;
}

int mapmerge_extract_transform(const int8_t* d_grid, int32_t width, int32_t height, double res, double origin_x,
                               double origin_y, const double* T_host, double* d_px, double* d_py, int64_t capacity,
                               int64_t* d_count, int64_t* d_last_appended, int32_t* d_status, void* d_ws, size_t ws_bytes,
                               void* stream) {
    if (!d_grid || !d_px || !d_py || !d_count || !d_status || !d_ws || width <= 0 || height <= 0 || !(res > 0.0)) {
        set_last_error("mapmerge_extract_transform: bad arguments");
        return OCCGRID_E_ARG;
    }
    const long long n_cells = (long long)width * height;
    if (ws_bytes < mapmerge_extract_workspace_bytes(n_cells)) { set_last_error("mapmerge_extract_transform: workspace too small"); return OCCGRID_E_WORKSPACE; }
    cudaStream_t st = (cudaStream_t)stream;
    const int blocks = (int)((n_cells + kChunk - 1) / kChunk);
    long long* ws_base = reinterpret_cast<long long*>(d_ws);
    unsigned int* block_counts = reinterpret_cast<unsigned int*>(reinterpret_cast<char*>(d_ws) + 256);
    Xform T;
    T.identity = 1;
    for (int i = 0; i < 16; ++i) T.m[i] = (i % 5 == 0) ? 1.0 : 0.0;
    if (T_host) {
        for (int i = 0; i < 16; ++i) { T.m[i] = T_host[i]; if (T_host[i] != ((i % 5 == 0) ? 1.0 : 0.0)) T.identity = 0; }
    }
    ProfileScope ps(K_MERGE_EXTRACT, st, 3);
    k_extract_count<<<blocks, kMT, 0, st>>>(d_grid, n_cells, block_counts);
    k_extract_reserve<<<1, 1024, 0, st>>>(block_counts, blocks, (long long*)d_count, capacity, ws_base, d_status,
                                           (long long*)d_last_appended);
    k_extract_write<<<blocks, kMT, 0, st>>>(d_grid, n_cells, width, res, origin_x, origin_y, T, block_counts, ws_base, d_px, d_py);
    OCC_CUDA_TRY(cudaGetLastError());
    return OCCGRID_OK;
}

static size_t batch_counts_bytes(int64_t n_cells, int n_agents) {
    const int64_t blocks = (n_cells + kChunk - 1) / kChunk;
    return align_up((size_t)blocks * (size_t)n_agents * sizeof(unsigned int), 256);
}

size_t mapmerge_extract_batch_workspace_bytes(int64_t n_cells, int n_agents) {
    const int64_t blocks = (n_cells + kChunk - 1) / kChunk;
    return batch_counts_bytes(n_cells, n_agents) + align_up((size_t)blocks * kMT * (size_t)n_agents * sizeof(unsigned long long), 256);
}

int mapmerge_extract_batch_count(const int8_t* const* d_grids, int n_agents, int32_t width, int32_t height,
                                 int64_t* d_agent_total, void* d_ws, size_t ws_bytes, int grids_bulk_ok, void* stream) {
    if (!d_grids || n_agents <= 0 || n_agents > 65535 || width <= 0 || height <= 0 || !d_agent_total || !d_ws) {
        set_last_error("mapmerge_extract_batch_count: bad arguments");
        return OCCGRID_E_ARG;
    }
    const long long n_cells = (long long)width * height;
    if (ws_bytes < mapmerge_extract_batch_workspace_bytes(n_cells, n_agents)) { set_last_error("mapmerge_extract_batch_count: workspace too small"); return OCCGRID_E_WORKSPACE; }
    cudaStream_t st = (cudaStream_t)stream;
    const int bpg = (int)((n_cells + kChunk - 1) / kChunk);
    unsigned int* block_counts = reinterpret_cast<unsigned int*>(d_ws);
    ProfileScope ps(K_MERGE_EXTRACT, st, 1);
    dim3 grid((unsigned)bpg, (unsigned)n_agents);
    unsigned long long* masks = reinterpret_cast<unsigned long long*>(reinterpret_cast<char*>(d_ws) + batch_counts_bytes(n_cells, n_agents));
    {
        ProfileScope scan(K_MERGE_SCAN, st, 1);
        if (grids_bulk_ok && (n_cells % 16) == 0) {
            const int ctas = device_sm_count() * kScanCtasPerSm;
            const size_t smem = (size_t)kScanStages * kScanStageBytes;
            static bool configured = false;
            if (!configured) {
                OCC_CUDA_TRY(cudaFuncSetAttribute(k_batch_count_tma, cudaFuncAttributeMaxDynamicSharedMemorySize, (int)smem));
                configured = true;
            }
            k_batch_count_tma<<<ctas, kMT, smem, st>>>(d_grids, n_cells, bpg, n_agents, block_counts, masks);
        } else {
            k_batch_count<<<grid, kMT, 0, st>>>(d_grids, n_cells, bpg, block_counts, masks);
        }
    }
    k_batch_scan<<<n_agents, 1024, 0, st>>>(block_counts, bpg, (long long*)d_agent_total);
    OCC_CUDA_TRY(cudaGetLastError());
    return OCCGRID_OK;
}

int mapmerge_extract_batch_write(const int8_t* const* d_grids, int n_agents, int32_t width, int32_t height, double res,
                                 const double* d_origins, const double* T_host ,
                                 const uint8_t* use_host , void* d_xforms ,
                                 double* d_px, double* d_py, int64_t capacity, const int64_t* d_agent_total,
                                 int64_t* d_agent_offset, int32_t* d_status, void* d_ws, size_t ws_bytes, void* stream) {
    if (!d_grids || n_agents <= 0 || n_agents > 65535 || width <= 0 || height <= 0 || !(res > 0.0) || !d_origins || !d_xforms ||
        !d_px || !d_py || !d_agent_total || !d_agent_offset || !d_status || !d_ws) {
        set_last_error("mapmerge_extract_batch_write: bad arguments");
        return OCCGRID_E_ARG;
    }
    const long long n_cells = (long long)width * height;
    if (ws_bytes < mapmerge_extract_batch_workspace_bytes(n_cells, n_agents)) { set_last_error("mapmerge_extract_batch_write: workspace too small"); return OCCGRID_E_WORKSPACE; }
    static_assert(sizeof(BatchXform) <= 96, "BatchXform must fit the 96-byte slot");
    cudaStream_t st = (cudaStream_t)stream;
    std::vector<BatchXform> hx((size_t)n_agents);
    for (int a = 0; a < n_agents; ++a) {
        BatchXform& t = hx[a];
        t.use = use_host ? (use_host[a] != 0) : 1;
        t.identity = 1;
        const double I[16] = {1, 0, 0, 0, 0, 1, 0, 0, 0, 0, 1, 0, 0, 0, 0, 1};
        const double* M = T_host ? T_host + 16 * (size_t)a : I;
        for (int i = 0; i < 16; ++i) if (M[i] != I[i]) t.identity = 0;
        t.m[0] = M[0]; t.m[1] = M[1]; t.m[2] = M[3];
        t.m[3] = M[4]; t.m[4] = M[5]; t.m[5] = M[7];
        t.w[0] = M[12]; t.w[1] = M[13]; t.w[2] = M[15];
    }
    OCC_CUDA_TRY(cudaMemcpyAsync(d_xforms, hx.data(), sizeof(BatchXform) * (size_t)n_agents, cudaMemcpyHostToDevice, st));
    OCC_CUDA_TRY(cudaStreamSynchronize(st));
    const int bpg = (int)((n_cells + kChunk - 1) / kChunk);
    unsigned int* block_counts = reinterpret_cast<unsigned int*>(d_ws);
    const BatchXform* dT = reinterpret_cast<const BatchXform*>(d_xforms);
    ProfileScope ps(K_MERGE_EXTRACT, st, 2);
    dim3 grid((unsigned)bpg, (unsigned)n_agents);
    k_batch_offsets<<<1, 1024, 0, st>>>((const long long*)d_agent_total, dT, n_agents, capacity, (long long*)d_agent_offset, d_status);
    const unsigned long long* masks = reinterpret_cast<const unsigned long long*>(reinterpret_cast<const char*>(d_ws) + batch_counts_bytes(n_cells, n_agents));
    k_batch_write<<<grid, kMT, 0, st>>>(masks, n_cells, width, res, d_origins, dT, bpg, block_counts, (const long long*)d_agent_offset,
                                        capacity, d_px, d_py);
    OCC_CUDA_TRY(cudaGetLastError());
    return OCCGRID_OK;
}

int mapmerge_bounds_enc_reset(uint64_t* d_bounds_enc, void* stream) {
    if (!d_bounds_enc) { set_last_error("mapmerge_bounds_enc_reset: NULL"); return OCCGRID_E_ARG; }
    k_benc_reset<<<1, 1, 0, (cudaStream_t)stream>>>((unsigned long long*)d_bounds_enc);
    OCC_CUDA_TRY(cudaGetLastError());
    return OCCGRID_OK;
}

int mapmerge_append_slice(const double* d_sx, const double* d_sy, const int64_t* d_agent_offset, int agent,
                          double* d_px, double* d_py, int64_t capacity, int64_t* d_count, int32_t* d_status,
                          uint64_t* d_bounds_enc, void* stream) {
    if (!d_sx || !d_sy || !d_agent_offset || agent < 0 || !d_px || !d_py || !d_count || !d_status) {
        set_last_error("mapmerge_append_slice: bad arguments");
        return OCCGRID_E_ARG;
    }
    cudaStream_t st = (cudaStream_t)stream;
    ProfileScope ps(K_MERGE_EXTRACT, st, 2);
    k_append_slice<<<device_sm_count(), kMT, 0, st>>>(d_sx, d_sy, (const long long*)d_agent_offset, agent, d_px, d_py, capacity,
                                         (long long*)d_count, d_status, (unsigned long long*)d_bounds_enc);
    k_bump_count<<<1, 1, 0, st>>>((const long long*)d_agent_offset, agent, capacity, (long long*)d_count);
    OCC_CUDA_TRY(cudaGetLastError());
    return OCCGRID_OK;
}

size_t mapmerge_bounds_workspace_bytes(void) { return (size_t)1024 * 8 * 4 * sizeof(double); }

int mapmerge_bounds(const double* d_px, const double* d_py, const int64_t* d_count, double* d_bounds, void* d_ws,
                    size_t ws_bytes, void* stream) {
    if (!d_px || !d_py || !d_count || !d_bounds || !d_ws || ws_bytes < mapmerge_bounds_workspace_bytes()) {
        set_last_error("mapmerge_bounds: bad arguments");
        return OCCGRID_E_ARG;
    }
    cudaStream_t st = (cudaStream_t)stream;
    const int blocks = device_sm_count() * 8;
    ProfileScope ps(K_MERGE_BOUNDS, st, 2);
    k_bounds_partial<<<blocks, kMT, 0, st>>>(d_px, d_py, (const long long*)d_count, (double*)d_ws);
    k_bounds_final<<<1, kMT, 0, st>>>((const double*)d_ws, blocks, d_bounds);
    OCC_CUDA_TRY(cudaGetLastError());
    return OCCGRID_OK;
}

static size_t voxel_layout(int64_t cells, int64_t points, size_t off[9]) {
    size_t o = 0;
    off[0] = o; o += 256;
    off[1] = o; o += align_up((size_t)(cells + 1) * 8, 256);
    off[2] = o; o += align_up((size_t)((points + kScanChunk - 1) / kScanChunk + 1) * 8, 256);
    for (int j = 3; j < 9; ++j) { off[j] = o; o += align_up((size_t)points * 4, 256); }
    return o;
}

size_t mapmerge_voxel_workspace_bytes(int64_t lattice_capacity_cells, int64_t point_capacity) {
    size_t off[9];
    return voxel_layout(lattice_capacity_cells, point_capacity, off);
}

struct VoxelArrays {
    VoxelHeader* hdr;
    uint2* lattice;
    uint2* block_sums;
    unsigned int *key, *head, *hcnt, *vrank, *soff, *slots;
};

static VoxelArrays voxel_arrays(void* d_ws, const size_t off[9]) {
    char* ws = reinterpret_cast<char*>(d_ws);
    VoxelArrays a;
    a.hdr = reinterpret_cast<VoxelHeader*>(ws + off[0]);
    a.lattice = reinterpret_cast<uint2*>(ws + off[1]);
    a.block_sums = reinterpret_cast<uint2*>(ws + off[2]);
    a.key = reinterpret_cast<unsigned int*>(ws + off[3]);
    a.head = reinterpret_cast<unsigned int*>(ws + off[4]);
    a.hcnt = reinterpret_cast<unsigned int*>(ws + off[5]);
    a.vrank = reinterpret_cast<unsigned int*>(ws + off[6]);
    a.soff = reinterpret_cast<unsigned int*>(ws + off[7]);
    a.slots = reinterpret_cast<unsigned int*>(ws + off[8]);
    return a;
}

static void launch_voxel_core(const double* px, const double* py, const VoxelHeader* hdr_c, VoxelHeader* hdr, const VoxelArrays& a,
                              int64_t launch_points, double voxel, double* out_px, double* out_py, long long* out_count,
                              unsigned long long* benc, cudaStream_t st) {
    const int gp = grid_for(launch_points);
    const int gs = grid_for((launch_points + kScanItems - 1) / kScanItems);
    k_voxel_mark<<<gp, kMT, 0, st>>>(px, py, voxel, hdr_c, a.lattice, a.key);
    k_voxel_gather<<<gp, kMT, 0, st>>>(hdr_c, a.lattice, a.key, a.head, a.hcnt);
    k_pscan_partial<<<gs, kMT, 0, st>>>(hdr_c, a.hcnt, a.block_sums);
    k_pscan_top<<<1, 1024, 0, st>>>(a.block_sums, hdr);
    k_pscan_apply<<<gs, kMT, 0, st>>>(hdr_c, a.hcnt, a.block_sums, a.vrank, a.soff);
    k_voxel_fill<<<gp, kMT, 0, st>>>(hdr_c, a.key, a.lattice, a.head, a.soff, a.slots);
    k_voxel_reduce<<<gp, kMT, 0, st>>>(px, py, hdr_c, a.hcnt, a.vrank, a.soff, a.slots, out_px, out_py, out_count, benc);
}

int mapmerge_voxel_downsample(const double* d_px, const double* d_py, const int64_t* d_count, int64_t point_capacity,
                              double voxel, const double* d_bounds, uint64_t* d_bounds_enc, int64_t lattice_capacity_cells,
                              double* d_out_px, double* d_out_py, int64_t* d_out_count, int32_t* d_status,
                              void* d_ws, size_t ws_bytes, void* stream) {
    if (!d_px || !d_py || !d_count || (!d_bounds && !d_bounds_enc) || !d_out_px || !d_out_py || !d_out_count || !d_status || !d_ws ||
        !(voxel > 0.0) || lattice_capacity_cells <= 0 || point_capacity <= 0) {
        set_last_error("mapmerge_voxel_downsample: bad arguments");
        return OCCGRID_E_ARG;
    }
    size_t off[9];
    if (ws_bytes < voxel_layout(lattice_capacity_cells, point_capacity, off)) {
        set_last_error("mapmerge_voxel_downsample: workspace too small");
        return OCCGRID_E_WORKSPACE;
    }
    const VoxelArrays a = voxel_arrays(d_ws, off);
    cudaStream_t st = (cudaStream_t)stream;
    ProfileScope ps(K_MERGE_VOXEL, st, 8);
    k_voxel_setup<<<1, 1, 0, st>>>(d_bounds, (unsigned long long*)d_bounds_enc, (const long long*)d_count, voxel,
                                   lattice_capacity_cells, point_capacity, a.hdr, d_status);
    launch_voxel_core(d_px, d_py, a.hdr, a.hdr, a, point_capacity, voxel, d_out_px, d_out_py, (long long*)d_out_count,
                      (unsigned long long*)d_bounds_enc, st);
    OCC_CUDA_TRY(cudaGetLastError());
    return OCCGRID_OK;
}

struct ChainArrays {
    ChainHeader* h;
    uint2* LM;
    unsigned int *gkey, *lkey, *next, *flag, *blockcount, *bar;
    double *resx, *resy;
    int bc_stride;
    unsigned long long* slice_benc;
    int* order;
};

static size_t chain_layout(const int64_t* dims, int n_agents, ChainArrays* a, void* base) {
    const size_t cells = (size_t)dims[0] * (size_t)dims[1], points = (size_t)dims[2], sl = (size_t)dims[3] + 16;
    char* ws = reinterpret_cast<char*>(base);
    size_t o = 0;
    auto take = [&](size_t bytes) { size_t at = o; o += align_up(bytes, 256); return at; };
    const size_t o_h = take(sizeof(ChainHeader)), o_lm = take((cells + 1) * 8), o_gk = take(points * 4);
    const size_t bc_stride = sl / kMT + 2;
    const size_t o_lk = take(sl * 4), o_nx = take(sl * 4), o_fl = take(sl * 4), o_bc = take(2 * bc_stride * 4), o_bar = take(16);
    const size_t o_rx = take(sl * 8), o_ry = take(sl * 8), o_sb = take((size_t)n_agents * 32), o_or = take((size_t)n_agents * 4);
    if (a) {
        a->h = reinterpret_cast<ChainHeader*>(ws + o_h);
        a->LM = reinterpret_cast<uint2*>(ws + o_lm);
        a->gkey = reinterpret_cast<unsigned int*>(ws + o_gk);
        a->lkey = reinterpret_cast<unsigned int*>(ws + o_lk);
        a->next = reinterpret_cast<unsigned int*>(ws + o_nx);
        a->flag = reinterpret_cast<unsigned int*>(ws + o_fl);
        a->blockcount = reinterpret_cast<unsigned int*>(ws + o_bc);
        a->bar = reinterpret_cast<unsigned int*>(ws + o_bar);
        a->bc_stride = (int)bc_stride;
        a->resx = reinterpret_cast<double*>(ws + o_rx);
        a->resy = reinterpret_cast<double*>(ws + o_ry);
        a->slice_benc = reinterpret_cast<unsigned long long*>(ws + o_sb);
        a->order = reinterpret_cast<int*>(ws + o_or);
    }
    return o;
}

static bool chain_dims_ok(const int64_t* dims, int n_agents) {
    return dims && n_agents > 0 && n_agents <= 65535 && dims[0] > 0 && dims[1] > 0 && dims[2] > 0 && dims[3] > 0 &&
           dims[0] * dims[1] < 0x7fffffffll && dims[2] < 0x7ffffff0ll && dims[3] < 0x7ffffff0ll;
}

size_t mapmerge_chain_workspace_bytes(const int64_t* dims, int n_agents) {
    if (!chain_dims_ok(dims, n_agents)) return 0;
    return chain_layout(dims, n_agents, nullptr, nullptr);
}

int mapmerge_chain_init(void* d_chain, size_t chain_bytes, const int64_t* dims, int n_agents, const double* d_sx,
                        const double* d_sy, const int64_t* d_agent_offset, const int32_t* order_host, int n_order,
                        const double* d_px, const double* d_py, const int64_t* d_count, void* stream) {
    if (!d_chain || !chain_dims_ok(dims, n_agents) || !d_sx || !d_sy || !d_agent_offset || !order_host || n_order < 0 ||
        n_order > n_agents || !d_px || !d_py || !d_count) {
        set_last_error("mapmerge_chain_init: bad arguments");
        return OCCGRID_E_ARG;
    }
    if (chain_bytes < chain_layout(dims, n_agents, nullptr, nullptr)) { set_last_error("mapmerge_chain_init: workspace too small"); return OCCGRID_E_WORKSPACE; }
    for (int i = 0; i < n_order; ++i)
        if (order_host[i] < 0 || order_host[i] >= n_agents) { set_last_error("mapmerge_chain_init: order entry out of range"); return OCCGRID_E_ARG; }
    ChainArrays c;
    chain_layout(dims, n_agents, &c, d_chain);
    cudaStream_t st = (cudaStream_t)stream;
    if (n_order) {
        OCC_CUDA_TRY(cudaMemcpyAsync(c.order, order_host, sizeof(int) * (size_t)n_order, cudaMemcpyHostToDevice, st));
        OCC_CUDA_TRY(cudaStreamSynchronize(st));
    }
    ProfileScope ps(K_CHAIN_PROBE, st, 5);
    k_chain_reset<<<1, 1, 0, st>>>(c.h);
    k_chain_slice_bounds_init<<<(n_agents + 255) / 256, 256, 0, st>>>(c.slice_benc, n_agents);
    dim3 grid((unsigned)grid_for(dims[3]), (unsigned)n_agents);
    if (grid.x > 64) grid.x = 64;
    k_chain_slice_bounds<<<grid, kMT, 0, st>>>(d_sx, d_sy, (const long long*)d_agent_offset, c.slice_benc);
    k_chain_rebounds<<<device_sm_count() * 8, kMT, 0, st>>>(d_px, d_py, (const long long*)d_count, c.h);
    k_chain_rebounds_apply<<<1, 1, 0, st>>>(c.h);
    OCC_CUDA_TRY(cudaGetLastError());
    return OCCGRID_OK;
}

int mapmerge_chain_run(void* d_chain, const int64_t* dims, int n_agents, int n_order, int n_callbacks, const double* d_sx,
                       const double* d_sy, const int64_t* d_agent_offset, double voxel, double* d_px, double* d_py,
                       int64_t capacity, int64_t* d_count, int32_t* d_status, void* stream) {
    if (!d_chain || !chain_dims_ok(dims, n_agents) || n_order < 0 || n_order > n_agents || n_callbacks < 0 || !d_sx || !d_sy ||
        !d_agent_offset || !(voxel > 0.0) || !d_px || !d_py || capacity > dims[2] || !d_count || !d_status) {
        set_last_error("mapmerge_chain_run: bad arguments");
        return OCCGRID_E_ARG;
    }
    if (n_callbacks == 0) return OCCGRID_OK;
    ChainArrays c;
    chain_layout(dims, n_agents, &c, d_chain);
    cudaStream_t st = (cudaStream_t)stream;
    static int resident_by_device[64] = {};
    int dev = 0;
    OCC_CUDA_TRY(cudaGetDevice(&dev));
    int resident_ctas = (dev >= 0 && dev < 64) ? resident_by_device[dev] : 0;
    if (resident_ctas == 0) {
        int sms = 0, per_sm = 0;
        OCC_CUDA_TRY(cudaDeviceGetAttribute(&sms, cudaDevAttrMultiProcessorCount, dev));
        OCC_CUDA_TRY(cudaOccupancyMaxActiveBlocksPerMultiprocessor(&per_sm, k_chain_persistent, kMT, 0));
        if (sms <= 0 || per_sm <= 0) { set_last_error("mapmerge_chain_run: persistent kernel does not fit the device"); return OCCGRID_E_CUDA; }
        resident_ctas = sms * per_sm;
        if (dev >= 0 && dev < 64) resident_by_device[dev] = resident_ctas;
    }
    int grid = grid_for(dims[3]);
    if (grid > resident_ctas) grid = resident_ctas;
    ChainRun r;
    r.h = c.h; r.order = c.order; r.n_order = n_order; r.n_callbacks = n_callbacks;
    r.agent_offset = (const long long*)d_agent_offset; r.slice_benc = c.slice_benc;
    r.sx = d_sx; r.sy = d_sy; r.voxel = voxel; r.W = dims[0]; r.H = dims[1];
    r.LM = c.LM; r.lkey = c.lkey; r.next = c.next; r.gkey = c.gkey; r.flag = c.flag; r.blockcount = c.blockcount;
    r.gx = d_px; r.gy = d_py; r.resx = c.resx; r.resy = c.resy;
    r.d_count = (long long*)d_count; r.capacity = capacity; r.status = d_status; r.bar = c.bar; r.bc_stride = c.bc_stride;
    void* args[] = {&r};
    ProfileScope ps(K_CHAIN_INCR, st, 1);
    OCC_CUDA_TRY(cudaLaunchCooperativeKernel((const void*)k_chain_persistent, dim3((unsigned)grid), dim3(kMT), args, 0, st));
    return OCCGRID_OK;
}

int mapmerge_chain_poll(void* d_chain, const int64_t* dims, int n_agents, int32_t* state_out, void* stream) {
    if (!d_chain || !chain_dims_ok(dims, n_agents) || !state_out) { set_last_error("mapmerge_chain_poll: bad arguments"); return OCCGRID_E_ARG; }
    ChainArrays c;
    chain_layout(dims, n_agents, &c, d_chain);
    cudaStream_t st = (cudaStream_t)stream;
    int two[2] = {0, 0};
    static_assert(offsetof(ChainHeader, cursor) == offsetof(ChainHeader, stalled) + sizeof(int), "stalled and cursor are read as one pair");
    OCC_CUDA_TRY(cudaMemcpyAsync(two, &c.h->stalled, sizeof(two), cudaMemcpyDeviceToHost, st));
    OCC_CUDA_TRY(cudaStreamSynchronize(st));
    state_out[0] = two[1];
    state_out[1] = two[0];
    return OCCGRID_OK;
}

int mapmerge_chain_rebounds(void* d_chain, const int64_t* dims, int n_agents, const double* d_px, const double* d_py,
                            const int64_t* d_count, void* stream) {
    if (!d_chain || !chain_dims_ok(dims, n_agents) || !d_px || !d_py || !d_count) { set_last_error("mapmerge_chain_rebounds: bad arguments"); return OCCGRID_E_ARG; }
    ChainArrays c;
    chain_layout(dims, n_agents, &c, d_chain);
    cudaStream_t st = (cudaStream_t)stream;
    ProfileScope ps(K_CHAIN_PROBE, st, 2);
    k_chain_rebounds<<<device_sm_count() * 8, kMT, 0, st>>>(d_px, d_py, (const long long*)d_count, c.h);
    k_chain_rebounds_apply<<<1, 1, 0, st>>>(c.h);
    OCC_CUDA_TRY(cudaGetLastError());
    return OCCGRID_OK;
}

int mapmerge_chain_rebuild(void* d_chain, const int64_t* dims, int n_agents, const double* d_sx, const double* d_sy,
                           const int64_t* d_agent_offset, int agent, double voxel, double* d_px, double* d_py, int64_t capacity,
                           int64_t* d_count, double* d_out_px, double* d_out_py, int64_t* d_out_count, int32_t* d_status,
                           void* d_voxel_ws, size_t voxel_ws_bytes, int64_t lattice_capacity_cells, void* stream) {
    if (!d_chain || !chain_dims_ok(dims, n_agents) || !d_sx || !d_sy || !d_agent_offset || agent < 0 || agent >= n_agents ||
        !(voxel > 0.0) || !d_px || !d_py || capacity > dims[2] || !d_count || !d_out_px || !d_out_py || !d_out_count || !d_status) {
        set_last_error("mapmerge_chain_rebuild: bad arguments");
        return OCCGRID_E_ARG;
    }
    size_t off[9];
    if (!d_voxel_ws || lattice_capacity_cells < dims[0] * dims[1] || voxel_ws_bytes < voxel_layout(lattice_capacity_cells, dims[2], off)) {
        set_last_error("mapmerge_chain_rebuild: voxel workspace too small");
        return OCCGRID_E_WORKSPACE;
    }
    const VoxelArrays va = voxel_arrays(d_voxel_ws, off);
    ChainArrays c;
    chain_layout(dims, n_agents, &c, d_chain);
    cudaStream_t st = (cudaStream_t)stream;
    const int gp = grid_for(capacity);
    ProfileScope ps(K_CHAIN_REBUILD, st, 13);
    k_chain_lm_clear<<<gp, kMT, 0, st>>>(c.h, c.LM, c.gkey, (const long long*)d_count);
    k_append_slice<<<device_sm_count(), kMT, 0, st>>>(d_sx, d_sy, (const long long*)d_agent_offset, agent, d_px, d_py, capacity, (long long*)d_count,
                                         d_status, nullptr);
    k_bump_count<<<1, 1, 0, st>>>((const long long*)d_agent_offset, agent, capacity, (long long*)d_count);
    k_chain_rebuild_hdr<<<1, 1, 0, st>>>(c.h, c.slice_benc, agent, (const long long*)d_count, voxel, dims[0], dims[1], dims[2], d_status);
    launch_voxel_core(d_px, d_py, &c.h->v, &c.h->v, va, capacity, voxel, d_out_px, d_out_py, (long long*)d_out_count, c.h->gb_enc, st);
    k_chain_lm_build<<<gp, kMT, 0, st>>>(c.h, d_out_px, d_out_py, (const long long*)d_out_count, voxel, c.LM, c.gkey);
    k_chain_rebuild_done<<<1, 1, 0, st>>>(c.h);
    OCC_CUDA_TRY(cudaGetLastError());
    return OCCGRID_OK;
}

int mapmerge_rasterise(const double* d_px, const double* d_py, const int64_t* d_count, double res, const double* d_bounds,
                       int32_t width, int32_t height, int8_t* d_grid_out, void* stream) {
    if (!d_px || !d_py || !d_count || !d_bounds || !d_grid_out || width <= 0 || height <= 0 || !(res > 0.0)) {
        set_last_error("mapmerge_rasterise: bad arguments");
        return OCCGRID_E_ARG;
    }
    cudaStream_t st = (cudaStream_t)stream;
    const long long n = (long long)width * height;
    ProfileScope ps(K_MERGE_RASTER, st, 2);
    k_raster_fill<<<grid_for(n / 16 + 1), kMT, 0, st>>>(d_grid_out, n);
    k_raster_scatter<<<device_sm_count() * 8, kMT, 0, st>>>(d_px, d_py, (const long long*)d_count, d_bounds, res, width, height, d_grid_out);
    OCC_CUDA_TRY(cudaGetLastError());
    return OCCGRID_OK;
}

int mapmerge_fuse_max(int8_t* d_dst, const int8_t* d_src, int64_t n, void* stream) {
    if (!d_dst || !d_src || n < 0) { set_last_error("mapmerge_fuse_max: bad arguments"); return OCCGRID_E_ARG; }
    if (n == 0) return OCCGRID_OK;
    cudaStream_t st = (cudaStream_t)stream;
    ProfileScope ps(K_MERGE_FUSE, st);
    k_fuse_max<<<grid_for(n), kMT, 0, st>>>(d_dst, d_src, n);
    OCC_CUDA_TRY(cudaGetLastError());
    return OCCGRID_OK;
}

}
```

distributed-multi-agent-slam-swarm-robotics-system_b200/csrc/occgrid_tiled.cu:

```cuda
#include "common.cuh"

namespace occ {

constexpr int kTT = 256;
constexpr int kChunkPk = 2048;
constexpr int kChunkMin = 256;
constexpr int kItemsPerCta = 3;
constexpr int kMaxWindowBytes = 100 * 1024;

struct TilePlanHeader {
    unsigned int n_items, n_active, total_records, work_counter, resolve_counter, overflow;
    unsigned int active_count;
    unsigned int pad;
};

__device__ __forceinline__ int home_tile(const Geom& g, const TileGeom& tg, double rx, double ry) {
    const double qx = cell_quotient(rx, g.ox, g.res), qy = cell_quotient(ry, g.oy, g.res);
    if (!quotient_in_range(qx) || !quotient_in_range(qy)) return -1;
    const int px = trunc_cell(qx) - g.win_x0 + tg.pad, py = trunc_cell(qy) - g.win_y0 + tg.pad;
    if (px < tg.pad - tg.reach || py < tg.pad - tg.reach || px >= tg.pad + g.win_w + tg.reach ||
        py >= tg.pad + g.win_h + tg.reach)
        return -1;
    return (py >> kTileShift) * tg.tiles_x + (px >> kTileShift);
}

constexpr int kPkPerCta = 2048;
constexpr int kSub = kPkPerCta / kTT;
constexpr int kHash = 4096;
constexpr unsigned int kEmpty = 0xffffffffu;
static_assert(kHash >= 2 * kPkPerCta, "hash table must stay at most half full");

__device__ __forceinline__ int hash_insert(unsigned int* keys, unsigned int tile) {
    unsigned int h = (tile * 2654435761u) >> 20;
    for (;;) {
        const unsigned int old = atomicCAS(&keys[h], kEmpty, tile);
        if (old == kEmpty || old == tile) return (int)h;
        h = (h + 1) & (kHash - 1);
    }
}

constexpr int kHashPerThread = kHash / kTT;

__device__ __forceinline__ void flush_tile_counts(const unsigned int* s_keys, const unsigned int* s_vals,
                                                  unsigned int* __restrict__ tile_count, unsigned int* __restrict__ active,
                                                  TilePlanHeader* __restrict__ hdr) {
    unsigned int key[kHashPerThread], old[kHashPerThread];
#pragma unroll
    for (int j = 0; j < kHashPerThread; ++j) {
        const int i = j * kTT + threadIdx.x;
        key[j] = s_keys[i];
        old[j] = 1u;
        if (key[j] != kEmpty) old[j] = atomicAdd(&tile_count[key[j]], s_vals[i]);
    }
#pragma unroll
    for (int j = 0; j < kHashPerThread; ++j)
        if (key[j] != kEmpty && old[j] == 0u) active[atomicAdd(&hdr->active_count, 1u)] = key[j];
}

__device__ __forceinline__ void reserve_tile_ranges(const unsigned int* s_keys, unsigned int* s_vals,
                                                    const unsigned int* __restrict__ tile_offset, unsigned int* __restrict__ tile_cursor) {
    unsigned int key[kHashPerThread], base[kHashPerThread], off[kHashPerThread];
#pragma unroll
    for (int j = 0; j < kHashPerThread; ++j) {
        const int i = j * kTT + threadIdx.x;
        key[j] = s_keys[i];
        base[j] = off[j] = 0u;
        if (key[j] != kEmpty) { off[j] = tile_offset[key[j]]; base[j] = atomicAdd(&tile_cursor[key[j]], s_vals[i]); }
    }
#pragma unroll
    for (int j = 0; j < kHashPerThread; ++j)
        if (key[j] != kEmpty) s_vals[j * kTT + threadIdx.x] = off[j] + base[j];
}

constexpr size_t kBinSmem = (size_t)kTT * kMaxRecStride + 2 * kHash * sizeof(unsigned int) + kPkPerCta * sizeof(unsigned short);
constexpr unsigned int kNoSlot = 0xffffu;

template <bool kMaps = false>
__global__ void __launch_bounds__(kTT)
k_home_bin(Geom g, TileGeom tg, const uint8_t* __restrict__ pkts, long long n, int stride,
           const int32_t* __restrict__ agent_idx, const double* __restrict__ drift,
           const double* __restrict__ agent_off, int n_agents,
           unsigned int* __restrict__ tile_count, PoseRec* __restrict__ recs, unsigned int* __restrict__ local_bins, uint2* __restrict__ runs,
           unsigned int* __restrict__ seg_count, unsigned int* __restrict__ active, TilePlanHeader* __restrict__ hdr,
           uint64_t* counters) {
    extern __shared__ __align__(16) uint8_t s_bin[];
    uint8_t* const s_rec = s_bin;
    unsigned int* const s_keys = reinterpret_cast<unsigned int*>(s_bin + kTT * kMaxRecStride);
    unsigned int* const s_vals = s_keys + kHash;
    unsigned short* const s_slot = reinterpret_cast<unsigned short*>(s_vals + kHash);
    __shared__ unsigned int s_wsum[kTT / 32];
    for (int i = threadIdx.x; i < kHash; i += kTT) { s_keys[i] = kEmpty; s_vals[i] = 0u; }
    unsigned long long c[OCCGRID_C_HITS + 1] = {};
    const long long cta_first = (long long)blockIdx.x * kPkPerCta;
    constexpr int kVec = (kTT * kMaxRecStride / 16 + kTT - 1) / kTT;
    uint4 pre[kVec];
    auto prefetch = [&](int sub) {
        const long long first = cta_first + (long long)sub * kTT;
        const long long left = n - first;
        const size_t bytes = left <= 0 ? 0 : (size_t)min((long long)kTT, left) * stride;
        const uint4* s4 = reinterpret_cast<const uint4*>(pkts + (size_t)first * stride);
#pragma unroll
        for (int j = 0; j < kVec; ++j) {
            const size_t i = (size_t)j * kTT + threadIdx.x;
            pre[j] = (i * 16 + 16 <= bytes) ? __ldg(s4 + i) : make_uint4(0u, 0u, 0u, 0u);
        }
    };
    const bool vec_ok = (reinterpret_cast<uintptr_t>(pkts) & 15) == 0 && ((kTT * stride) & 15) == 0;
    if (vec_ok) prefetch(0);
    for (int sub = 0; sub < kSub; ++sub) {
        const long long first = cta_first + (long long)sub * kTT;
        if (first >= n) break;
        const int count = (int)min((long long)kTT, n - first);
        __syncthreads();
        if (vec_ok) {
            const size_t bytes = (size_t)count * stride;
            uint4* d4 = reinterpret_cast<uint4*>(s_rec);
#pragma unroll
            for (int j = 0; j < kVec; ++j) {
                const size_t i = (size_t)j * kTT + threadIdx.x;
                if (i * 16 + 16 <= bytes) d4[i] = pre[j];
            }
            for (size_t i = (bytes / 16) * 16 + threadIdx.x; i < bytes; i += kTT) s_rec[i] = __ldg(pkts + (size_t)first * stride + i);
            if (sub + 1 < kSub) prefetch(sub + 1);
        } else {
            stage_records(pkts + (size_t)first * stride, (size_t)count * stride, s_rec);
        }
        __syncthreads();
        if ((int)threadIdx.x < count) {
            const long long k = first + threadIdx.x;
            double rx, ry, ryaw;
            float dist[4];
            c[OCCGRID_C_PACKETS] += 1;
            unsigned int slot = kNoSlot;
            int agent = 1;
            const int st = decode_packet(s_rec + threadIdx.x * stride, k, agent_idx, drift, agent_off, n_agents, &rx, &ry, &ryaw, dist,
                                         kMaps ? &agent : nullptr);
            if (st == PKT_DROPPED) c[OCCGRID_C_DROPPED] += 1;
            else if (st == PKT_BAD_POSE) c[OCCGRID_C_BAD_POSE] += 1;
            else {
                c[OCCGRID_C_ACCEPTED] += 1;
                c[OCCGRID_C_BEAMS] += 4;
#pragma unroll
                for (int s = 0; s < 4; ++s) {
                    const double d = (double)dist[s];
                    c[OCCGRID_C_HITS] += (OCC_MIN_DIST_M < d && d <= OCC_MAX_DIST_M) ? 1 : 0;
                }
                int tile = home_tile(g, tg, rx, ry);
                if (kMaps && tile >= 0) tile += (agent - 1) * tg.n_tiles;
                if (tile >= 0) {
                    slot = (unsigned int)hash_insert(s_keys, (unsigned int)tile);
                    atomicAdd(&s_vals[slot], 1u);
                    PoseRec r;
                    r.rx = rx; r.ry = ry; r.yaw = (float)ryaw;
                    r.d[0] = dist[0]; r.d[1] = dist[1]; r.d[2] = dist[2]; r.d[3] = dist[3];
                    r.k = (unsigned int)k;
                    r.tile = tile; r.pad = 0;
                    recs[k] = r;
                }
            }
            s_slot[sub * kTT + threadIdx.x] = (unsigned short)slot;
        }
    }
    __syncthreads();
    unsigned int key[kHashPerThread], rank[kHashPerThread];
#pragma unroll
    for (int j = 0; j < kHashPerThread; ++j) {
        const int i = j * kTT + threadIdx.x;
        key[j] = s_keys[i];
        rank[j] = 0u;
        if (key[j] != kEmpty) rank[j] = atomicAdd(&tile_count[key[j]], s_vals[i]);
    }
    const int lane = threadIdx.x & 31, warp = threadIdx.x >> 5;
    unsigned int mine = 0u;
#pragma unroll
    for (int j = 0; j < kHashPerThread; ++j) mine += key[j] != kEmpty ? s_vals[j * kTT + threadIdx.x] + 0x10000u : 0u;
    unsigned int inc = mine;
#pragma unroll
    for (int o = 1; o < 32; o <<= 1) { const unsigned int u = __shfl_up_sync(0xffffffffu, inc, o); if (lane >= o) inc += u; }
    if (lane == 31) s_wsum[warp] = inc;
    __syncthreads();
    unsigned int pos = inc - mine, n_local = 0u;
#pragma unroll
    for (int w = 0; w < kTT / 32; ++w) {
        pos += w < warp ? s_wsum[w] : 0u;
        n_local += s_wsum[w];
    }
    n_local &= 0xffffu;
    if (threadIdx.x == 0) seg_count[blockIdx.x] = n_local;
    const size_t seg0 = (size_t)blockIdx.x * kPkPerCta;
#pragma unroll
    for (int j = 0; j < kHashPerThread; ++j) {
        if (key[j] == kEmpty) continue;
        const int i = j * kTT + threadIdx.x;
        const unsigned int run = pos >> 16, begin = pos & 0xffffu;
        runs[seg0 + run] = make_uint2(key[j], rank[j] - begin);
        pos += s_vals[i] + 0x10000u;
        s_keys[i] = run;
        s_vals[i] = begin;
        if (rank[j] == 0u) active[atomicAdd(&hdr->active_count, 1u)] = key[j];
    }
    __syncthreads();
    unsigned int* const s_local = reinterpret_cast<unsigned int*>(s_rec);
    const int n_seg = (int)min((long long)kPkPerCta, n - (long long)seg0);
    for (int j = threadIdx.x; j < n_seg; j += kTT) {
        const unsigned int slot = s_slot[j];
        if (slot != kNoSlot) s_local[atomicAdd(&s_vals[slot], 1u)] = (s_keys[slot] << 16) | (unsigned int)j;
    }
    __syncthreads();
    for (unsigned int j = threadIdx.x; j < n_local; j += kTT) local_bins[seg0 + j] = s_local[j];
    __syncthreads();
    block_add_counters(c, reinterpret_cast<unsigned long long*>(s_rec), counters);
}

__global__ void __launch_bounds__(kTT)
k_place_runs(const unsigned int* __restrict__ local_bins, const uint2* __restrict__ runs, const unsigned int* __restrict__ seg_count,
             const unsigned int* __restrict__ tile_offset, const TilePlanHeader* __restrict__ hdr, unsigned int* __restrict__ bins) {
    if (hdr->overflow) return;
    const size_t seg0 = (size_t)blockIdx.x * kPkPerCta;
    const int n_local = (int)seg_count[blockIdx.x];
    unsigned int e[kSub], off[kSub];
    uint2 d[kSub];
#pragma unroll
    for (int sub = 0; sub < kSub; ++sub) {
        const int j = sub * kTT + threadIdx.x;
        e[sub] = j < n_local ? local_bins[seg0 + j] : kEmpty;
    }
#pragma unroll
    for (int sub = 0; sub < kSub; ++sub) d[sub] = e[sub] != kEmpty ? runs[seg0 + (e[sub] >> 16)] : make_uint2(0u, 0u);
#pragma unroll
    for (int sub = 0; sub < kSub; ++sub) off[sub] = e[sub] != kEmpty ? tile_offset[d[sub].x] : 0u;
#pragma unroll
    for (int sub = 0; sub < kSub; ++sub)
        if (e[sub] != kEmpty) bins[off[sub] + d[sub].y + (unsigned int)(sub * kTT + threadIdx.x)] = (unsigned int)(seg0 + (e[sub] & 0xffffu));
}

__device__ __forceinline__ int chunk_valid(const SegInfo& seg, long long chunk, long long* addr0) {
    const long long a0 = chunk * kSegChunk;
    *addr0 = a0;
    const unsigned int sg = (unsigned int)(a0 / seg.seg_cap);
    const unsigned int j0 = (unsigned int)(a0 - (long long)sg * seg.seg_cap);
    unsigned int cnt = seg.d_counts ? seg.d_counts[sg] : seg.host_count;
    if (cnt > seg.seg_cap) cnt = seg.seg_cap;
    return cnt > j0 ? (int)min((unsigned int)kSegChunk, cnt - j0) : 0;
}

__global__ void __launch_bounds__(kTT)
k_home_count_poses(Geom g, TileGeom tg, const PoseRec* __restrict__ recs, const int* __restrict__ in_tiles, SegInfo seg, long long n_chunks,
                   int tiles_in_records,
                   unsigned int* __restrict__ tile_count, int* __restrict__ tile_ids,
                   unsigned int* __restrict__ active, TilePlanHeader* __restrict__ hdr, uint64_t* counters) {
    __shared__ unsigned int s_keys[kHash];
    __shared__ unsigned int s_vals[kHash];
    __shared__ unsigned long long s_acc[(OCCGRID_C_HITS + 1) * 32];
    unsigned long long c[OCCGRID_C_HITS + 1] = {};
    for (long long chunk = blockIdx.x; chunk < n_chunks; chunk += gridDim.x) {
        long long addr0;
        const int valid = chunk_valid(seg, chunk, &addr0);
        if (valid == 0) continue;
        for (int i = threadIdx.x; i < kHash; i += kTT) { s_keys[i] = kEmpty; s_vals[i] = 0u; }
        __syncthreads();
        if (tiles_in_records) {
            int tl[kSub];
#pragma unroll
            for (int sub = 0; sub < kSub; ++sub) {
                const int j = sub * kTT + threadIdx.x;
                tl[sub] = -1;
                if (j < valid) tl[sub] = in_tiles ? in_tiles[addr0 + j] : recs[addr0 + j].tile;
            }
#pragma unroll
            for (int sub = 0; sub < kSub; ++sub) {
                const int j = sub * kTT + threadIdx.x;
                if (j >= valid) continue;
                int tile = tl[sub];
                if (tile >= tg.n_tiles) tile = -1;
                if (tile >= 0) atomicAdd(&s_vals[hash_insert(s_keys, (unsigned int)tile)], 1u);
                tile_ids[addr0 + j] = tile;
            }
        } else {
            for (int sub = 0; sub < kSub; ++sub) {
                const int j = sub * kTT + threadIdx.x;
                if (j >= valid) break;
                const long long k = addr0 + j;
                int tile = -1;
                const PoseRec r = recs[k];
                c[OCCGRID_C_PACKETS] += 1;
                if (!(isfinite(r.rx) && isfinite(r.ry) && isfinite(r.yaw))) c[OCCGRID_C_BAD_POSE] += 1;
                else {
                    c[OCCGRID_C_ACCEPTED] += 1;
                    c[OCCGRID_C_BEAMS] += 4;
#pragma unroll
                    for (int s2 = 0; s2 < 4; ++s2) {
                        const double dd = (double)r.d[s2];
                        c[OCCGRID_C_HITS] += (OCC_MIN_DIST_M < dd && dd <= OCC_MAX_DIST_M) ? 1 : 0;
                    }
                    tile = home_tile(g, tg, r.rx, r.ry);
                }
                if (tile >= 0) atomicAdd(&s_vals[hash_insert(s_keys, (unsigned int)tile)], 1u);
                tile_ids[k] = tile;
            }
        }
        __syncthreads();
        flush_tile_counts(s_keys, s_vals, tile_count, active, hdr);
        __syncthreads();
    }
    block_add_counters(c, s_acc, counters);
}

__global__ void __launch_bounds__(kTT)
k_home_scatter_segs(SegInfo seg, long long n_chunks, const int* __restrict__ tile_ids, const unsigned int* __restrict__ tile_offset,
                    unsigned int* __restrict__ tile_cursor, const TilePlanHeader* __restrict__ hdr, unsigned int* __restrict__ bins) {
    __shared__ unsigned int s_keys[kHash];
    __shared__ unsigned int s_vals[kHash];
    if (hdr->overflow) return;
    for (long long chunk = blockIdx.x; chunk < n_chunks; chunk += gridDim.x) {
        long long addr0;
        const int valid = chunk_valid(seg, chunk, &addr0);
        if (valid == 0) continue;
        for (int i = threadIdx.x; i < kHash; i += kTT) { s_keys[i] = kEmpty; s_vals[i] = 0u; }
        __syncthreads();
        unsigned int where[kSub];
        int tl[kSub];
#pragma unroll
        for (int sub = 0; sub < kSub; ++sub) {
            const int j = sub * kTT + threadIdx.x;
            tl[sub] = j < valid ? tile_ids[addr0 + j] : -1;
        }
#pragma unroll
        for (int sub = 0; sub < kSub; ++sub) {
            const int j = sub * kTT + threadIdx.x;
            where[sub] = kEmpty;
            if (j < valid) {
                const int tile = tl[sub];
                if (tile >= 0) {
                    const int h = hash_insert(s_keys, (unsigned int)tile);
                    where[sub] = ((unsigned int)h << 16) | atomicAdd(&s_vals[h], 1u);
                }
            }
        }
        __syncthreads();
        reserve_tile_ranges(s_keys, s_vals, tile_offset, tile_cursor);
        __syncthreads();
#pragma unroll
        for (int sub = 0; sub < kSub; ++sub)
            if (where[sub] != kEmpty)
                bins[s_vals[where[sub] >> 16] + (where[sub] & 0xffffu)] = (unsigned int)(addr0 + sub * kTT + threadIdx.x);
        __syncthreads();
    }
}

__global__ void __launch_bounds__(1024)
k_tile_plan(unsigned int* __restrict__ tile_count, unsigned int* __restrict__ tile_offset,
            unsigned int* __restrict__ tile_cursor, uint4* __restrict__ items, unsigned int max_items,
            const unsigned int* __restrict__ active, unsigned long long max_records, TilePlanHeader* __restrict__ hdr,
            uint64_t* counters, unsigned int target_items) {
    __shared__ unsigned int s_warp[2][33];
    __shared__ unsigned int s_carry[2];
    __shared__ unsigned int s_total;
    if (threadIdx.x < 2) s_carry[threadIdx.x] = 0;
    if (threadIdx.x == 0) s_total = 0;
    __syncthreads();
    const int n_active = (int)hdr->active_count;
    const int lane = threadIdx.x & 31, warp = threadIdx.x >> 5;
    {
        unsigned int mine = 0;
        for (int i = threadIdx.x; i < n_active; i += blockDim.x) mine += tile_count[active[i]];
#pragma unroll
        for (int o = 16; o > 0; o >>= 1) mine += __shfl_xor_sync(0xffffffffu, mine, o);
        if (lane == 0 && mine) atomicAdd(&s_total, mine);
    }
    __syncthreads();
    unsigned int chunk_pk = (s_total / target_items + kChunkMin) / kChunkMin * kChunkMin;
    chunk_pk = chunk_pk > (unsigned int)kChunkPk ? (unsigned int)kChunkPk : chunk_pk;
    for (int start = 0; start < n_active; start += blockDim.x) {
        const int i = start + threadIdx.x;
        const unsigned int t = i < n_active ? active[i] : 0u;
        const unsigned int cnt = i < n_active ? tile_count[t] : 0u;
        unsigned int v[2] = {cnt, (cnt + chunk_pk - 1) / chunk_pk};
        unsigned int ex[2];
#pragma unroll
        for (int j = 0; j < 2; ++j) {
            unsigned int inc = v[j];
#pragma unroll
            for (int o = 1; o < 32; o <<= 1) { unsigned int u = __shfl_up_sync(0xffffffffu, inc, o); if (lane >= o) inc += u; }
            if (lane == 31) s_warp[j][warp] = inc;
            ex[j] = inc - v[j];
        }
        __syncthreads();
        if (warp < 2) {
            unsigned int w = s_warp[warp][lane], winc = w;
#pragma unroll
            for (int o = 1; o < 32; o <<= 1) { unsigned int u = __shfl_up_sync(0xffffffffu, winc, o); if (lane >= o) winc += u; }
            s_warp[warp][lane] = winc - w;
            if (lane == 31) s_warp[warp][32] = winc;
        }
        __syncthreads();
        const unsigned int off = s_carry[0] + s_warp[0][warp] + ex[0];
        const unsigned int item0 = s_carry[1] + s_warp[1][warp] + ex[1];
        if (i < n_active) {
            tile_offset[t] = off;
            tile_cursor[t] = 0u;
            tile_count[t] = 0u;
            for (unsigned int j = 0; j < v[1]; ++j) {
                const unsigned int b = off + j * chunk_pk;
                const unsigned int e = min(off + cnt, b + chunk_pk);
                if (item0 + j < max_items) items[item0 + j] = make_uint4(t, b, e, 0u);
            }
        }
        __syncthreads();
        if (threadIdx.x < 2) s_carry[threadIdx.x] += s_warp[threadIdx.x][32];
        __syncthreads();
    }
    if (threadIdx.x == 0) {
        TilePlanHeader h;
        h.total_records = s_carry[0];
        h.n_items = s_carry[1];
        h.n_active = (unsigned int)n_active;
        h.work_counter = 0;
        h.resolve_counter = 0;
        h.active_count = 0;
        h.overflow = (s_carry[0] > max_records || s_carry[1] > max_items) ? 1u : 0u;
        if (h.overflow) { h.n_items = 0; h.n_active = 0; }
        h.pad = 0;
        *hdr = h;
        if (counters) atomicAdd(reinterpret_cast<unsigned long long*>(counters) + OCCGRID_C_RECORDS, (unsigned long long)s_carry[0]);
    }
}

__device__ __noinline__ void draw_beam_smem(unsigned int* __restrict__ s_win, int side, int pitch, int x, int y,
                                               int ddx, int ddy, unsigned int free_stamp, bool hit, bool skip_first) {
    const int dx = abs(ddx), dy = abs(ddy);
    int err = dx - dy;
    const int n = max(dx, dy);
    const unsigned int us = (unsigned int)side;
    if ((unsigned int)x < us && (unsigned int)y < us && (unsigned int)(x + ddx) < us && (unsigned int)(y + ddy) < us) {
        const int sxo = ddx > 0 ? 1 : -1;
        const int syo = ddy > 0 ? pitch : -pitch;
        const bool xmajor = dx >= dy;
        const int dmaj = xmajor ? dx : dy, dmin = xmajor ? dy : dx;
        const int step_maj = xmajor ? sxo : syo;
        const int step_both = sxo + syo;
        const int e_minor = dmaj - dmin;
        int E = dmaj - dmin;
        int off = y * pitch + x;
        int i = 0;
        if (skip_first) {
            if (n == 0) return;
            const bool minor = 2 * E < dmaj;
            off += minor ? step_both : step_maj;
            E += minor ? e_minor : -dmin;
            i = 1;
        }
        for (; i < n; ++i) {
            atomicMax(&s_win[off], free_stamp);
            const bool minor = 2 * E < dmaj;
            off += minor ? step_both : step_maj;
            E += minor ? e_minor : -dmin;
        }
        if (hit) atomicMax(&s_win[off], free_stamp | 1u);
        return;
    }
    const int sx = ddx > 0 ? 1 : -1, sy = ddy > 0 ? 1 : -1;
    for (int i = 0; i < n; ++i) {
        if (!(i == 0 && skip_first) && (unsigned int)x < us && (unsigned int)y < us) atomicMax(&s_win[y * pitch + x], free_stamp);
        const int e2 = 2 * err;
        if (e2 > -dy) { err -= dy; x += sx; }
        if (e2 < dx)  { err += dx; y += sy; }
    }
    if (hit && !(n == 0 && skip_first) && (unsigned int)x < us && (unsigned int)y < us) atomicMax(&s_win[y * pitch + x], free_stamp | 1u);
}

__device__ __noinline__ void count_beam_smem(unsigned int* __restrict__ s_win, int side, int pitch, int x, int y,
                                                int ddx, int ddy, bool hit) {
    const int dx = abs(ddx), dy = abs(ddy);
    const int n = max(dx, dy);
    const unsigned int us = (unsigned int)side;
    if ((unsigned int)x < us && (unsigned int)y < us && (unsigned int)(x + ddx) < us && (unsigned int)(y + ddy) < us) {
        const int sxo = ddx > 0 ? 1 : -1;
        const int syo = ddy > 0 ? pitch : -pitch;
        const bool xmajor = dx >= dy;
        const int dmaj = xmajor ? dx : dy, dmin = xmajor ? dy : dx;
        const int step_maj = xmajor ? sxo : syo;
        const int step_both = sxo + syo;
        const int e_minor = dmaj - dmin;
        int E = dmaj - dmin;
        int off = y * pitch + x;
        for (int i = 0; i < n; ++i) {
            atomicAdd(&s_win[off], 1u);
            const bool minor = 2 * E < dmaj;
            off += minor ? step_both : step_maj;
            E += minor ? e_minor : -dmin;
        }
        if (hit) atomicAdd(&s_win[off], 0x10000u);
        return;
    }
    int err = dx - dy;
    const int sx = ddx > 0 ? 1 : -1, sy = ddy > 0 ? 1 : -1;
    for (int i = 0; i < n; ++i) {
        if ((unsigned int)x < us && (unsigned int)y < us) atomicAdd(&s_win[y * pitch + x], 1u);
        const int e2 = 2 * err;
        if (e2 > -dy) { err -= dy; x += sx; }
        if (e2 < dx)  { err += dx; y += sy; }
    }
    if (hit && (unsigned int)x < us && (unsigned int)y < us) atomicAdd(&s_win[y * pitch + x], 0x10000u);
}



constexpr int kMaskMaxLen = 32;
constexpr int kMaskEntries = (kMaskMaxLen + 1) * (kMaskMaxLen + 2) / 2;

__device__ __forceinline__ unsigned int walk_mask_of(int dmaj, int dmin) {
    unsigned int m = 0u;
    int E = dmaj - dmin;
    for (int i = 0; i < dmaj; ++i) {
        const bool minor = 2 * E < dmaj;
        m |= (minor ? 1u : 0u) << i;
        E += minor ? (dmaj - dmin) : -dmin;
    }
    return m;
}

__device__ __forceinline__ void build_walk_masks(unsigned int* s_mask) {
    for (int e = threadIdx.x; e < kMaskEntries; e += blockDim.x) {
        int dmaj = 0;
        while ((dmaj + 1) * (dmaj + 2) / 2 <= e) ++dmaj;
        s_mask[e] = walk_mask_of(dmaj, e - dmaj * (dmaj + 1) / 2);
    }
}

template <bool kAdd>
__device__ __forceinline__ void smem_red(unsigned int addr, unsigned int v) {
    if (kAdd) asm volatile("red.shared.add.u32 [%0], %1;" ::"r"(addr), "r"(v) : "memory");
    else      asm volatile("red.shared.max.u32 [%0], %1;" ::"r"(addr), "r"(v) : "memory");
}

template <bool kAdd>
__device__ __forceinline__ void walk_beam_masked(unsigned int win, int pitch, int x, int y, int ddx, int ddy,
                                                 unsigned int v_free, bool hit, bool skip_first, const unsigned int* s_mask) {
    const int dx = abs(ddx), dy = abs(ddy);
    const bool xmajor = dx >= dy;
    const int dmaj = xmajor ? dx : dy, dmin = xmajor ? dy : dx;
    const int sx4 = ddx > 0 ? 4 : -4;
    const int sy4 = (ddy > 0 ? pitch : -pitch) * 4;
    const int step_maj = xmajor ? sx4 : sy4, step_min = xmajor ? sy4 : sx4;
    unsigned int mask = s_mask[dmaj * (dmaj + 1) / 2 + dmin];
    unsigned int a = win + (unsigned int)(y * pitch + x) * 4u;
    const unsigned int a_end = a + (unsigned int)((ddy * pitch + ddx) * 4);
    int rem = dmaj;
    if (rem > 0) {
        if (!skip_first) smem_red<kAdd>(a, v_free);
        a += step_maj + ((mask & 1u) ? step_min : 0);
        mask >>= 1;
        --rem;
    }
    while (rem >= 8) {
#pragma unroll
        for (int j = 0; j < 8; ++j) {
            smem_red<kAdd>(a, v_free);
            a += step_maj + ((mask & (1u << j)) ? step_min : 0);
        }
        mask >>= 8;
        rem -= 8;
    }
    if (rem >= 4) {
#pragma unroll
        for (int j = 0; j < 4; ++j) {
            smem_red<kAdd>(a, v_free);
            a += step_maj + ((mask & (1u << j)) ? step_min : 0);
        }
        mask >>= 4;
        rem -= 4;
    }
    for (; rem > 0; --rem) {
        smem_red<kAdd>(a, v_free);
        a += step_maj + ((mask & 1u) ? step_min : 0);
        mask >>= 1;
    }
    if (hit && !(dmaj == 0 && skip_first && !kAdd)) smem_red<kAdd>(a_end, kAdd ? 0x10000u : (v_free | 1u));
}

struct RouteSmem {
    unsigned int cnt[kMaxBands];
    unsigned int off[kMaxBands + 1];
    unsigned int base[kMaxBands];
};

__device__ __forceinline__ unsigned int lds_u32_at(const unsigned int* __restrict__ words, unsigned int byte_off) {
    const unsigned int w = byte_off >> 2, sh = (byte_off & 3u) * 8u;
    return __funnelshift_r(words[w], words[w + 1], sh);
}

__device__ __forceinline__ int decode_packet_smem(const unsigned int* __restrict__ words, unsigned int byte_off, long long k,
                                                  const int32_t* agent_idx, const double* drift, const double* agent_off,
                                                  int n_agents, double* rx, double* ry, float* yaw, float dist[4]) {
    if (lds_u32_at(words, byte_off) != 0x4c525351u) return PKT_DROPPED;
    const unsigned int b4 = lds_u32_at(words, byte_off + 4);
    const long long agent = agent_idx ? (long long)agent_idx[k] : (long long)(b4 & 0xffu);
    if (agent < 1 || agent > n_agents) return PKT_DROPPED;
    const unsigned int b8 = lds_u32_at(words, byte_off + 8), b12 = lds_u32_at(words, byte_off + 12),
                       b16 = lds_u32_at(words, byte_off + 16);
    double x = (double)__uint_as_float(__funnelshift_r(b4, b8, 8));
    double y = (double)__uint_as_float(__funnelshift_r(b8, b12, 8));
    const float fyaw = __uint_as_float(__funnelshift_r(b12, b16, 8));
    x = OCC_DADD(x, agent_off[2 * agent + 0]);
    y = OCC_DADD(y, agent_off[2 * agent + 1]);
    if (drift) {
        const double2 dv = *reinterpret_cast<const double2*>(drift + 2 * k);
        x = OCC_DADD(x, dv.x);
        y = OCC_DADD(y, dv.y);
    }
    if (!(isfinite(x) && isfinite(y) && isfinite(fyaw))) return PKT_BAD_POSE;
    *rx = x; *ry = y; *yaw = fyaw;
    const unsigned int c24 = lds_u32_at(words, byte_off + 24), c28 = lds_u32_at(words, byte_off + 28),
                       c32 = lds_u32_at(words, byte_off + 32), c36 = lds_u32_at(words, byte_off + 36),
                       c40 = lds_u32_at(words, byte_off + 40);
    dist[0] = __uint_as_float(__funnelshift_r(c24, c28, 8));
    dist[1] = __uint_as_float(__funnelshift_r(c28, c32, 8));
    dist[2] = __uint_as_float(__funnelshift_r(c32, c36, 8));
    dist[3] = __uint_as_float(__funnelshift_r(c36, c40, 8));
    return PKT_OK;
}

__device__ __forceinline__ bool robot_cell(double r, double o, double res, double inv_res, int* cell) {
    double q = OCC_DMUL(OCC_DADD(r, -o), inv_res);
    const double tol = OCC_DMUL(OCC_DMUL(fabs(r) + fabs(o) + 11.0, inv_res), 0x1p-47);
    if (near_cell_boundary(q, tol)) q = cell_quotient(r, o, res);
    if (!quotient_in_range(q)) return false;
    *cell = trunc_cell(q);
    return true;
}

struct RouteStats { unsigned int a, b; };

constexpr int kRouteSubs = kRouteSubsPerItem;
constexpr int kRoutePerThread = kRouteItemPk / kTT;
static_assert(kRouteItemPk % kTT == 0 && kRoutePerThread >= 1 && kRoutePerThread <= 4, "route sub-batch = 1..4 packets per thread");

struct RoutePk {
    double rx, ry;
    float yaw, d[4];
    int band0, nb, tile0, tile1;
    unsigned int rank0, rank1;
};

__device__ __forceinline__ void route_decode(const RouteJob& J, const unsigned int* s_buf, int slot, long long k, RoutePk& P,
                                             RouteStats& st_acc) {
    P.band0 = -1; P.nb = 0; P.tile0 = P.tile1 = -1; P.rank0 = P.rank1 = 0u;
    const int st = decode_packet_smem(s_buf, (unsigned int)slot * (unsigned int)J.stride, k, J.agent_idx, J.drift, J.agent_off,
                                      J.n_agents, &P.rx, &P.ry, &P.yaw, P.d);
    st_acc.a += 1u + (st == PKT_OK ? 0x10000u : 0u);
    st_acc.b += st == PKT_DROPPED ? 1u : 0u;
    if (st != PKT_OK) return;
    unsigned int hits = 0;
#pragma unroll
    for (int s2 = 0; s2 < 4; ++s2) {
        const double dd = (double)P.d[s2];
        hits += (OCC_MIN_DIST_M < dd && dd <= OCC_MAX_DIST_M) ? 1u : 0u;
    }
    st_acc.b += hits << 16;
    int gx, gy;
    if (!(robot_cell(P.rx, J.ox, J.res, J.inv_res, &gx) && robot_cell(P.ry, J.oy, J.res, J.inv_res, &gy))) return;
    const int reach = J.reach;
    if (gx < -reach || gx >= J.size_x + reach) return;
    const int tcol = (gx + J.pad) >> kTileShift;
    for (int b = 0; b < J.n_bands; ++b) {
        if (gy - reach < J.band_y0[b + 1]) {
            const int py = gy - J.band_y0[b];
            if (py >= -reach) {
                P.band0 = b; P.nb = 1;
                P.tile0 = ((py + J.pad) >> kTileShift) * J.tiles_x + tcol;
                if (b + 1 < J.n_bands && gy + reach >= J.band_y0[b + 1]) {
                    P.nb = 2;
                    P.tile1 = ((gy - J.band_y0[b + 1] + J.pad) >> kTileShift) * J.tiles_x + tcol;
                }
            }
            break;
        }
    }
}

__device__ __forceinline__ void route_rank(RouteSmem& S, RoutePk& P, int lane, unsigned int lt) {
    const unsigned int p0 = __match_any_sync(0xffffffffu, P.band0);
    if (P.band0 >= 0) {
        const int leader = __ffs(p0) - 1;
        unsigned int b0 = 0;
        if (lane == leader) b0 = atomicAdd(&S.cnt[P.band0], (unsigned int)__popc(p0));
        P.rank0 = __shfl_sync(p0, b0, leader) + __popc(p0 & lt);
    }
    if (__any_sync(0xffffffffu, P.nb == 2)) {
        const unsigned int p1 = __match_any_sync(0xffffffffu, P.nb == 2 ? P.band0 + 1 : -1);
        if (P.nb == 2) {
            const int leader = __ffs(p1) - 1;
            unsigned int b1 = 0;
            if (lane == leader) b1 = atomicAdd(&S.cnt[P.band0 + 1], (unsigned int)__popc(p1));
            P.rank1 = __shfl_sync(p1, b1, leader) + __popc(p1 & lt);
        }
    }
}

__device__ __forceinline__ void route_store(const RouteJob& J, uint4* s16, const RoutePk& P, unsigned int my_off, long long k) {
    const unsigned int o0 = __shfl_sync(0xffffffffu, my_off, P.band0 < 0 ? 0 : P.band0);
    const unsigned long long ux = (unsigned long long)__double_as_longlong(P.rx), uy = (unsigned long long)__double_as_longlong(P.ry);
    const uint4 w0 = make_uint4((unsigned int)ux, (unsigned int)(ux >> 32), (unsigned int)uy, (unsigned int)(uy >> 32));
    const uint4 w1 = make_uint4(__float_as_uint(P.yaw), __float_as_uint(P.d[0]), __float_as_uint(P.d[1]), __float_as_uint(P.d[2]));
    const unsigned int ord = J.ordinal_base + (unsigned int)k;
    if (P.band0 >= 0) {
        uint4* dst = s16 + (size_t)(o0 + P.rank0) * 3;
        dst[0] = w0; dst[1] = w1; dst[2] = make_uint4(__float_as_uint(P.d[3]), ord, (unsigned int)P.tile0, 0u);
    }
    if (__any_sync(0xffffffffu, P.nb == 2)) {
        const unsigned int o1 = __shfl_sync(0xffffffffu, my_off, P.nb == 2 ? P.band0 + 1 : 0);
        if (P.nb == 2) {
            uint4* dst = s16 + (size_t)(o1 + P.rank1) * 3;
            dst[0] = w0; dst[1] = w1; dst[2] = make_uint4(__float_as_uint(P.d[3]), ord, (unsigned int)P.tile1, 0u);
        }
    }
}

__device__ __noinline__ RouteStats route_item(const RouteJob& J, unsigned int item, unsigned int* s_buf ,
                                              RouteSmem& S, RouteStats st_in) {
    const int lane = threadIdx.x & 31, warp = threadIdx.x >> 5;
    const unsigned int lt = (1u << lane) - 1u;
    long long first = (long long)item * (kRouteItemPk * kRouteSubs);
    for (int sub = 0; sub < kRouteSubs; ++sub, first += kRouteItemPk) {
        const int count = (int)max(0ll, min((long long)kRouteItemPk, J.n - first));
        if (count == 0) break;
        __syncthreads();
        if (threadIdx.x < kMaxBands) S.cnt[threadIdx.x] = 0u;
        {
            const uint8_t* src = J.pkts + (size_t)first * J.stride;
            const size_t bytes = (size_t)count * J.stride;
            constexpr int kVec = kRouteItemPk * kMaxRecStride / 16 / kTT;
            if ((reinterpret_cast<uintptr_t>(src) & 15) == 0) {
                const uint4* s4 = reinterpret_cast<const uint4*>(src);
                uint4* d4 = reinterpret_cast<uint4*>(s_buf);
                const size_t nvec = bytes / 16;
                uint4 v[kVec];
#pragma unroll
                for (int j = 0; j < kVec; ++j) {
                    const size_t i = (size_t)j * kTT + threadIdx.x;
                    if (i < nvec) v[j] = __ldg(s4 + i);
                }
#pragma unroll
                for (int j = 0; j < kVec; ++j) {
                    const size_t i = (size_t)j * kTT + threadIdx.x;
                    if (i < nvec) d4[i] = v[j];
                }
                for (size_t i = nvec * 16 + threadIdx.x; i < bytes; i += kTT) reinterpret_cast<uint8_t*>(s_buf)[i] = __ldg(src + i);
            } else {
                stage_records(src, bytes, reinterpret_cast<uint8_t*>(s_buf));
            }
        }
        {
            const long long nf = first + kRouteItemPk;
            const long long nbytes = max(0ll, min((long long)kRouteItemPk, J.n - nf)) * J.stride;
            const long long o = (long long)threadIdx.x * 128;
            if (sub + 1 < kRouteSubs && o < nbytes) asm volatile("prefetch.global.L2 [%0];" ::"l"(J.pkts + (size_t)nf * J.stride + o));
        }
        __syncthreads();
        RoutePk P[kRoutePerThread];
#pragma unroll
        for (int u = 0; u < kRoutePerThread; ++u) {
            const int slot = u * kTT + threadIdx.x;
            P[u].band0 = -1; P[u].nb = 0;
            if (slot < count) route_decode(J, s_buf, slot, first + slot, P[u], st_in);
        }
#pragma unroll
        for (int u = 0; u < kRoutePerThread; ++u) route_rank(S, P[u], lane, lt);
        __syncthreads();
        const unsigned int n_b = lane < J.n_bands ? S.cnt[lane] : 0u;
        unsigned int inc = n_b;
#pragma unroll
        for (int o = 1; o < 32; o <<= 1) { const unsigned int t = __shfl_up_sync(0xffffffffu, inc, o); if (lane >= o) inc += t; }
        const unsigned int my_off = inc - n_b;
        if (warp == 0) {
            unsigned int base = 0u;
            if (n_b) {
                base = atomicAdd(&J.resv[lane], n_b);
                if (base + n_b > J.seg_cap) { atomicOr(J.status, 2); base = 0xffffffffu; }
            }
            S.base[lane] = base;
            S.off[lane] = my_off;
            if (lane == 31) S.off[32] = inc;
        }
        uint4* s16 = reinterpret_cast<uint4*>(s_buf);
#pragma unroll
        for (int u = 0; u < kRoutePerThread; ++u) route_store(J, s16, P[u], my_off, first + u * kTT + threadIdx.x);
        __syncthreads();
        for (int b = 0; b < J.n_bands; ++b) {
            const unsigned int base = S.base[b];
            const unsigned int n_rec = S.off[b + 1] - S.off[b];
            if (n_rec == 0u || base == 0xffffffffu) continue;
            const size_t slot0 = (size_t)J.src_rank * J.seg_cap + base;
            uint4* out = reinterpret_cast<uint4*>(J.peer_recs[b] + slot0);
            const uint4* in = s16 + (size_t)S.off[b] * 3;
            for (unsigned int q = threadIdx.x; q < n_rec * 3u; q += kTT) out[q] = in[q];
            int* tout = J.peer_tiles[b] + slot0;
            const unsigned int* tin = s_buf + (size_t)S.off[b] * 12 + 10;
            for (unsigned int q = threadIdx.x; q < n_rec; q += kTT) tout[q] = (int)tin[(size_t)q * 12];
        }
    }
    return st_in;
}

#define OCC_ROUTE_TAIL_DIV 2
__device__ __forceinline__ unsigned int route_items_before(unsigned int i, unsigned int n_items, unsigned int n_route) {
    const unsigned int tail = n_items ? n_route / OCC_ROUTE_TAIL_DIV : 0u;
    const unsigned int n_body = n_route - tail, n_head = n_items + n_body;
    if (i >= n_head) return n_body + (i - n_head);
    return (unsigned int)(((unsigned long long)i * n_body) / n_head);
}

template <bool kCounts, bool kRoute, bool kMaps = false>
__global__ void __launch_bounds__(kTT, 3)
k_home_raycast(Geom g, TileGeom tg, const uint4* __restrict__ items, TilePlanHeader* __restrict__ hdr,
               const unsigned int* __restrict__ bins, const PoseRec* __restrict__ recs, int ordinals_in_records,
               unsigned int* __restrict__ stamps, uint64_t* counters, int have_items, const RouteJob job) {
    extern __shared__ __align__(16) unsigned int s_win[];
    unsigned long long* const s_acc = reinterpret_cast<unsigned long long*>(s_win);
    __shared__ RouteSmem s_route;
    __shared__ unsigned int s_mask[kMaskEntries];
    __shared__ RouteJob s_job;
    if (kRoute && threadIdx.x == 0) s_job = job;
    build_walk_masks(s_mask);
    const unsigned int win_addr = (unsigned int)__cvta_generic_to_shared(s_win);
    const unsigned int n_items = have_items ? hdr->n_items : 0u;
    const unsigned int n_route = kRoute ? job.n_route_items : 0u;
    const unsigned int n_total = n_items + n_route;
    const int side = tg.win_side, pitch = tg.pitch, words = side * pitch;
    unsigned long long c[3] = {0, 0, 0};
    RouteStats rs = {0u, 0u};
    __shared__ unsigned int s_next[2];
    if (threadIdx.x == 0) s_next[0] = atomicAdd(&hdr->work_counter, 1u);
    for (int i = threadIdx.x; i < words; i += kTT) s_win[i] = 0u;
    __syncthreads();
    for (int turn = 0;; turn ^= 1) {
        unsigned int it = s_next[turn];
        if (it >= n_total) break;
        if (kRoute) {
            const unsigned int r0 = route_items_before(it, n_items, n_route), r1 = route_items_before(it + 1u, n_items, n_route);
            if (r1 > r0) {
                if (threadIdx.x == 0) s_next[turn ^ 1] = atomicAdd(&hdr->work_counter, 1u);
                rs = route_item(s_job, r0, s_win, s_route, rs);
                __syncthreads();
                continue;
            }
            it -= r0;
            for (int i = threadIdx.x; i < words; i += kTT) s_win[i] = 0u;
            __syncthreads();
        }
        const uint4 item = items[it];
        const unsigned int map = kMaps ? item.x / (unsigned int)tg.n_tiles : 0u;
        const unsigned int tile = item.x - map * (unsigned int)tg.n_tiles;
        unsigned int* __restrict__ const plane = kMaps ? stamps + (size_t)map * ((size_t)g.win_w * g.win_h) : stamps;
        const int ttx = tile % tg.tiles_x, tty = tile / tg.tiles_x;
        const int wx0 = g.win_x0 - tg.pad + (ttx << kTileShift) - tg.reach;
        const int wy0 = g.win_y0 - tg.pad + (tty << kTileShift) - tg.reach;
        for (unsigned int r = item.y + threadIdx.x; r < item.z; r += kTT) {
            const unsigned int idx = bins[r];
            const PoseRec rec = recs[idx];
            const unsigned int k = ordinals_in_records ? rec.k : idx;
            PacketFrame F;
            packet_frame(g, rec.rx, rec.ry, (double)rec.yaw, LibSinCos(), &F);
            const bool owned = F.x0 >= g.win_x0 && F.x0 < g.win_x0 + g.win_w && F.y0 >= g.win_y0 && F.y0 < g.win_y0 + g.win_h;
            const int lx = F.x0 - wx0, ly = F.y0 - wy0;
            const unsigned int us = (unsigned int)side;
            bool later_writes_first = false;
#pragma unroll 1
            for (int s = 3; s >= 0; --s) {
                Beam b;
                expand_beam_of(g, F, s, s == 0 ? rec.d[0] : (s == 1 ? rec.d[1] : (s == 2 ? rec.d[2] : rec.d[3])), LibSinCos(), &b);
                if (!b.valid) continue;
                const int cells = beam_cells(b);
                c[0] += cells;
                c[1] += b.slow;
                if (owned) c[2] += cells;
                const int ddx = b.x1 - b.x0, ddy = b.y1 - b.y0;
                const bool fast = (unsigned int)lx < us && (unsigned int)ly < us && (unsigned int)(lx + ddx) < us &&
                                  (unsigned int)(ly + ddy) < us && cells <= kMaskMaxLen + 1;
                if (kCounts) {
                    if (fast) walk_beam_masked<true>(win_addr, pitch, lx, ly, ddx, ddy, 1u, b.hit != 0, false, s_mask);
                    else count_beam_smem(s_win, side, pitch, lx, ly, ddx, ddy, b.hit != 0);
                } else {
                    const unsigned int stamp = (k * 4u + (unsigned int)s + 1u) << 1;
                    if (fast) walk_beam_masked<false>(win_addr, pitch, lx, ly, ddx, ddy, stamp, b.hit != 0, later_writes_first, s_mask);
                    else draw_beam_smem(s_win, side, pitch, lx, ly, ddx, ddy, stamp, b.hit != 0, later_writes_first);
                }
                later_writes_first = later_writes_first || (cells > 1 || b.hit);
            }
        }
        unsigned int next_pos = 0u;
        if (threadIdx.x == 0) next_pos = atomicAdd(&hdr->work_counter, 1u);
        __syncthreads();
        {
            const int lx_lo = max(0, g.win_x0 - wx0), lx_hi = min(side, g.win_x0 + g.win_w - wx0);
            const int ly_lo = max(0, g.win_y0 - wy0), ly_hi = min(side, g.win_y0 + g.win_h - wy0);
            const int lane = threadIdx.x & 31, warp = threadIdx.x >> 5;
            for (int ly = warp; ly < side; ly += kTT / 32) {
                unsigned int* row = s_win + ly * pitch;
                const bool row_in = ly >= ly_lo && ly < ly_hi;
                unsigned int* out = plane + (size_t)(wy0 + ly - g.win_y0) * g.win_w + (wx0 - g.win_x0);
                for (int lx = lane; lx < side; lx += 32) {
                    const unsigned int v = row[lx];
                    if (!v) continue;
                    if (!kRoute) row[lx] = 0u;
                    if (!(row_in && lx >= lx_lo && lx < lx_hi)) continue;
                    if (kCounts)
                        atomicAdd(reinterpret_cast<unsigned long long*>(plane) + ((size_t)(wy0 + ly - g.win_y0) * g.win_w + (wx0 - g.win_x0) + lx),
                                  ((unsigned long long)(v >> 16) << 32) | (unsigned long long)(v & 0xffffu));
                    else
                        atomicMax(out + lx, v);
                }
            }
        }
        if (threadIdx.x == 0) s_next[turn ^ 1] = next_pos;
        __syncthreads();
    }
    if (kRoute && job.counters) {
        __syncthreads();
        const unsigned long long pk = rs.a & 0xffffu, acc = rs.a >> 16, drp = rs.b & 0xffffu, hits = rs.b >> 16;
        const unsigned long long rc[6] = {pk, acc, drp, pk - acc - drp, 4ull * acc, hits};
        block_add_counters(rc, s_acc, job.counters);
    }
    if (counters) {
        __syncthreads();
        const int lane = threadIdx.x & 31, warp = threadIdx.x >> 5;
#pragma unroll
        for (int i = 0; i < 3; ++i) {
            unsigned long long x = c[i];
#pragma unroll
            for (int o = 16; o > 0; o >>= 1) x += __shfl_xor_sync(0xffffffffu, x, o);
            if (lane == 0) s_acc[i * 32 + warp] = x;
        }
        __syncthreads();
        if (threadIdx.x < 3) {
            unsigned long long t = 0;
            for (int w = 0; w < kTT / 32; ++w) t += s_acc[threadIdx.x * 32 + w];
            const int slot = threadIdx.x == 0 ? OCCGRID_C_UPDATES : (threadIdx.x == 1 ? OCCGRID_C_SLOWPATH : OCCGRID_C_OWNED_UPDATES);
            if (t) atomicAdd(reinterpret_cast<unsigned long long*>(counters) + slot, t);
        }
    }
}

constexpr int kResolveSplit = 8;

template <bool kMaps = false>
__global__ void __launch_bounds__(kTT)
k_home_resolve(Geom g, TileGeom tg, const unsigned int* __restrict__ active, TilePlanHeader* __restrict__ hdr,
               unsigned int* __restrict__ stamps, int8_t* __restrict__ grid) {
    __shared__ unsigned int s_item;
    const unsigned int n_work = hdr->n_active * kResolveSplit;
    const int side = tg.win_side;
    const int lane = threadIdx.x & 31, warp = threadIdx.x >> 5;
    for (;;) {
        __syncthreads();
        if (threadIdx.x == 0) s_item = atomicAdd(&hdr->resolve_counter, 1u);
        __syncthreads();
        const unsigned int it = s_item;
        if (it >= n_work) break;
        const unsigned int key = active[it / kResolveSplit];
        const unsigned int map = kMaps ? key / (unsigned int)tg.n_tiles : 0u;
        const unsigned int t = key - map * (unsigned int)tg.n_tiles;
        const size_t map_off = kMaps ? (size_t)map * ((size_t)g.win_w * g.win_h) : 0;
        unsigned int* __restrict__ const plane = stamps + map_off;
        int8_t* __restrict__ const map_grid = grid + map_off;
        const int part = (int)(it % kResolveSplit);
        const int ttx = t % tg.tiles_x, tty = t / tg.tiles_x;
        const int wx0 = -tg.pad + (ttx << kTileShift) - tg.reach;
        const int wy0 = -tg.pad + (tty << kTileShift) - tg.reach;
        const int lx_lo = max(0, -wx0), lx_hi = min(side, g.win_w - wx0);
        const int ly_lo = max(0, -wy0), ly_hi = min(side, g.win_h - wy0);
        if (lx_hi <= lx_lo) continue;
        for (int ly = ly_lo + part * (kTT / 32) + warp; ly < ly_hi; ly += kResolveSplit * (kTT / 32)) {
            const size_t row = (size_t)(wy0 + ly) * g.win_w + wx0;
            for (int lx = lx_lo + lane; lx < lx_hi; lx += 32) {
                const unsigned int s = plane[row + lx];
                if (s) {
                    map_grid[row + lx] = (s & 1u) ? OCCGRID_CELL_OCCUPIED : OCCGRID_CELL_FREE;
                    plane[row + lx] = 0u;
                }
            }
        }
    }
}


static int g_raycast_cta_cap = 0;
void set_raycast_cta_cap(int cap) { g_raycast_cta_cap = cap < 0 ? 0 : cap; }

struct TiledLayout {
    size_t off_stamps, off_count, off_offset, off_cursor, off_active, off_hdr, off_items, off_ids, off_bins, off_local, off_runs,
        off_segs, off_recs, total;
    unsigned long long max_records;
    unsigned int max_items;
};

static TiledLayout tiled_layout(const occgrid_geom* geom, int64_t max_records, bool packets, int n_maps = 1) {
    TiledLayout L;
    const TileGeom tg = tile_geom(geom);
    const size_t n_keys = (size_t)n_maps * tg.n_tiles;
    L.max_records = (unsigned long long)max_records;
    unsigned long long items = L.max_records / kChunkMin + (unsigned long long)n_keys + 1;
    if (items > L.max_records + 1) items = L.max_records + 1;
    L.max_items = (unsigned int)items;
    size_t o = 0;
    L.off_stamps = o; o += align_up((size_t)geom->win_w * geom->win_h * 4 * (size_t)n_maps, 256);
    L.off_count = o;  o += align_up((n_keys + 1) * 4, 256);
    L.off_offset = o; o += align_up((n_keys + 1) * 4, 256);
    L.off_cursor = o; o += align_up((n_keys + 1) * 4, 256);
    L.off_active = o; o += align_up((n_keys + 1) * 4, 256);
    L.off_hdr = o;    o += 256;
    L.off_items = o;  o += align_up((size_t)L.max_items * sizeof(uint4), 256);
    L.off_ids = o;    o += packets ? 0 : align_up((size_t)L.max_records * sizeof(int), 256);
    L.off_bins = o;   o += align_up((size_t)L.max_records * sizeof(unsigned int), 256);
    L.off_local = o;  o += packets ? align_up((size_t)L.max_records * sizeof(unsigned int), 256) : 0;
    L.off_runs = o;   o += packets ? align_up((size_t)L.max_records * sizeof(uint2), 256) : 0;
    L.off_segs = o;   o += packets ? align_up((size_t)(L.max_records + kPkPerCta - 1) / kPkPerCta * sizeof(unsigned int), 256) : 0;
    L.off_recs = o;   o += packets ? align_up((size_t)L.max_records * sizeof(PoseRec), 256) : 0;
    L.total = o;
    return L;
}

bool tiled_supported(const occgrid_geom* geom, int n_maps) {
    const TileGeom tg = tile_geom(geom);
    return (size_t)tg.win_side * tg.pitch * 4 <= (size_t)kMaxWindowBytes && (long long)n_maps * tg.n_tiles <= (1ll << 24);
}

size_t tiled_workspace_bytes(const occgrid_geom* geom, int n_maps, int64_t max_packets) {
    return tiled_layout(geom, max_packets < 1 ? 1 : max_packets, true, n_maps).total;
}

size_t tiled_band_workspace_bytes(const occgrid_geom* geom, int n_segs, int64_t seg_cap) {
    return tiled_layout(geom, (int64_t)n_segs * seg_cap, false).total;
}

struct TiledPtrs {
    unsigned int *stamps, *tile_count, *tile_offset, *tile_cursor, *active, *bins, *local_bins, *seg_count;
    TilePlanHeader* hdr;
    uint4* items;
    int* tile_ids;
    uint2* runs;
    PoseRec* recs;
};

static TiledPtrs tiled_ptrs(const TiledLayout& L, void* d_ws) {
    char* ws = reinterpret_cast<char*>(d_ws);
    TiledPtrs p;
    p.stamps = reinterpret_cast<unsigned int*>(ws + L.off_stamps);
    p.tile_count = reinterpret_cast<unsigned int*>(ws + L.off_count);
    p.tile_offset = reinterpret_cast<unsigned int*>(ws + L.off_offset);
    p.tile_cursor = reinterpret_cast<unsigned int*>(ws + L.off_cursor);
    p.active = reinterpret_cast<unsigned int*>(ws + L.off_active);
    p.hdr = reinterpret_cast<TilePlanHeader*>(ws + L.off_hdr);
    p.items = reinterpret_cast<uint4*>(ws + L.off_items);
    p.bins = reinterpret_cast<unsigned int*>(ws + L.off_bins);
    p.tile_ids = reinterpret_cast<int*>(ws + L.off_ids);
    p.local_bins = reinterpret_cast<unsigned int*>(ws + L.off_local);
    p.runs = reinterpret_cast<uint2*>(ws + L.off_runs);
    p.seg_count = reinterpret_cast<unsigned int*>(ws + L.off_segs);
    p.recs = reinterpret_cast<PoseRec*>(ws + L.off_recs);
    return p;
}

static size_t raycast_smem(const TileGeom& tg, bool route) {
    size_t b = (size_t)tg.win_side * tg.pitch * 4;
    const size_t r = (size_t)kRouteItemPk * 2 * sizeof(PoseRec);
    const size_t raw = (size_t)kRouteItemPk * kMaxRecStride;
    if (route) b = b > r ? b : r;
    if (route) b = b > raw ? b : raw;
    return b;
}

template <bool kCounts, bool kRoute, bool kMaps = false>
static int launch_raycast(const Geom& g, const TileGeom& tg, const TiledPtrs& P, const PoseRec* recs, int ordinals_in_records,
                          unsigned int* plane, uint64_t* d_counters, int have_items, const RouteJob& job, cudaStream_t st) {
    const size_t smem = raycast_smem(tg, kRoute);
    static thread_local size_t configured = 0;
    if (smem > configured) {
        OCC_CUDA_TRY(cudaFuncSetAttribute(k_home_raycast<kCounts, kRoute, kMaps>, cudaFuncAttributeMaxDynamicSharedMemorySize, (int)smem));
        configured = smem;
    }
    int ctas_per_sm = 1;
    if (cudaOccupancyMaxActiveBlocksPerMultiprocessor(&ctas_per_sm, k_home_raycast<kCounts, kRoute, kMaps>, kTT, smem) != cudaSuccess || ctas_per_sm < 1)
        ctas_per_sm = 1;
    if (g_raycast_cta_cap > 0 && ctas_per_sm > g_raycast_cta_cap) ctas_per_sm = g_raycast_cta_cap;
    ProfileScope ps(K_TILE_RAYCAST, st);
    k_home_raycast<kCounts, kRoute, kMaps><<<device_sm_count() * ctas_per_sm, kTT, smem, st>>>(g, tg, P.items, P.hdr, P.bins, recs,
                                                                                               ordinals_in_records, plane, d_counters,
                                                                                               have_items, job);
    return OCCGRID_OK;
}

static unsigned int plan_target_items() { return (unsigned int)device_sm_count() * 3u * (unsigned int)kItemsPerCta; }

static int grid_chunks(long long n_chunks) {
    long long b = n_chunks < 1 ? 1 : n_chunks;
    const long long cap = (long long)device_sm_count() * 8;
    return (int)(b < cap ? b : cap);
}

int integrate_tiled(const occgrid_geom* geom, const PacketBatch& batch, const PoseRec* d_poses, int ordinals_in_records, Output kind,
                    void* d_out, void* d_ws, size_t ws_bytes, uint64_t* d_counters, cudaStream_t st) {
    const int64_t n = batch.n;
    const bool maps = kind == Output::kAgentMaps;
    const TiledLayout L = tiled_layout(geom, n, d_poses == nullptr, maps ? batch.n_agents : 1);
    if (ws_bytes < L.total) {
        set_last_error("workspace %zu B < %zu B needed by TILED for %lld records", ws_bytes, L.total, (long long)n);
        return OCCGRID_E_WORKSPACE;
    }
    const TiledPtrs P = tiled_ptrs(L, d_ws);
    const PoseRec* recs = d_poses ? d_poses : P.recs;
    const Geom g = to_geom(geom);
    const TileGeom tg = tile_geom(geom);
    const unsigned int blocks = (unsigned int)((n + kPkPerCta - 1) / kPkPerCta);
    SegInfo seg;
    seg.n_segs = 1; seg.seg_cap = (unsigned int)align_up((size_t)n, kSegChunk); seg.d_counts = nullptr; seg.host_count = (unsigned int)n;
    const long long n_chunks = (n + kSegChunk - 1) / kSegChunk;
    {
        ProfileScope ps(K_TILE_COUNT, st);
        if (d_poses) {
            k_home_count_poses<<<grid_chunks(n_chunks), kTT, 0, st>>>(g, tg, d_poses, nullptr, seg, n_chunks, 0, P.tile_count, P.tile_ids, P.active,
                                                                      P.hdr, d_counters);
        } else {
            const auto bin = maps ? k_home_bin<true> : k_home_bin<false>;
            OCC_CUDA_TRY(cudaFuncSetAttribute(bin, cudaFuncAttributeMaxDynamicSharedMemorySize, (int)kBinSmem));
            bin<<<blocks, kTT, kBinSmem, st>>>(g, tg, batch.pkts, n, batch.stride, batch.agent_idx, batch.drift, batch.agent_off, batch.n_agents,
                                               P.tile_count, P.recs, P.local_bins, P.runs, P.seg_count, P.active, P.hdr, d_counters);
        }
    }
    {
        ProfileScope ps(K_TILE_SCAN, st);
        k_tile_plan<<<1, 1024, 0, st>>>(P.tile_count, P.tile_offset, P.tile_cursor, P.items, L.max_items, P.active, L.max_records, P.hdr,
                                        d_counters, plan_target_items());
    }
    {
        ProfileScope ps(K_TILE_SCATTER, st);
        if (d_poses) k_home_scatter_segs<<<grid_chunks(n_chunks), kTT, 0, st>>>(seg, n_chunks, P.tile_ids, P.tile_offset, P.tile_cursor, P.hdr, P.bins);
        else         k_place_runs<<<blocks, kTT, 0, st>>>(P.local_bins, P.runs, P.seg_count, P.tile_offset, P.hdr, P.bins);
    }
    RouteJob none = {};
    unsigned int* const plane = kind == Output::kCounts ? reinterpret_cast<unsigned int*>(d_out) : P.stamps;
    if (kind == Output::kCounts) launch_raycast<true, false>(g, tg, P, recs, ordinals_in_records, plane, d_counters, 1, none, st);
    else if (maps)               launch_raycast<false, false, true>(g, tg, P, recs, ordinals_in_records, plane, d_counters, 1, none, st);
    else                         launch_raycast<false, false>(g, tg, P, recs, ordinals_in_records, plane, d_counters, 1, none, st);
    if (kind != Output::kCounts) {
        ProfileScope ps(K_TILE_RESOLVE, st);
        const auto resolve = maps ? k_home_resolve<true> : k_home_resolve<false>;
        resolve<<<device_sm_count() * 8, kTT, 0, st>>>(g, tg, P.active, P.hdr, P.stamps, reinterpret_cast<int8_t*>(d_out));
    }
    OCC_CUDA_TRY(cudaGetLastError());
    return OCCGRID_OK;
}

int tiled_prepare_poses(const occgrid_geom* geom, const PoseRec* d_recs, const int* d_tiles, const SegInfo& seg, int tiles_in_records,
                        void* d_ws, size_t ws_bytes, uint64_t* d_counters, cudaStream_t st) {
    const int64_t max_records = (int64_t)seg.n_segs * seg.seg_cap;
    const TiledLayout L = tiled_layout(geom, max_records, false);
    if (ws_bytes < L.total) {
        set_last_error("workspace %zu B < %zu B needed by the band step for %lld record addresses", ws_bytes, L.total, (long long)max_records);
        return OCCGRID_E_WORKSPACE;
    }
    const TiledPtrs P = tiled_ptrs(L, d_ws);
    const Geom g = to_geom(geom);
    const TileGeom tg = tile_geom(geom);
    const long long n_chunks = max_records / kSegChunk;
    {
        ProfileScope ps(K_TILE_COUNT, st);
        k_home_count_poses<<<grid_chunks(n_chunks), kTT, 0, st>>>(g, tg, d_recs, d_tiles, seg, n_chunks, tiles_in_records, P.tile_count, P.tile_ids,
                                                                  P.active, P.hdr, d_counters);
    }
    {
        ProfileScope ps(K_TILE_SCAN, st);
        k_tile_plan<<<1, 1024, 0, st>>>(P.tile_count, P.tile_offset, P.tile_cursor, P.items, L.max_items, P.active, L.max_records, P.hdr,
                                        d_counters, plan_target_items());
    }
    {
        ProfileScope ps(K_TILE_SCATTER, st);
        k_home_scatter_segs<<<grid_chunks(n_chunks), kTT, 0, st>>>(seg, n_chunks, P.tile_ids, P.tile_offset, P.tile_cursor, P.hdr, P.bins);
    }
    OCC_CUDA_TRY(cudaGetLastError());
    return OCCGRID_OK;
}

int tiled_raycast_route(const occgrid_geom* geom, const PoseRec* d_recs, int have_items, const RouteJob* job,
                        int8_t* d_grid, void* d_ws, size_t ws_bytes, int64_t max_records, uint64_t* d_counters, cudaStream_t st,
                        cudaEvent_t after_fused) {
    const TiledLayout L = tiled_layout(geom, max_records, false);
    if (ws_bytes < L.total) { set_last_error("workspace too small for the band step"); return OCCGRID_E_WORKSPACE; }
    const TiledPtrs P = tiled_ptrs(L, d_ws);
    const Geom g = to_geom(geom);
    const TileGeom tg = tile_geom(geom);
    if (!have_items) {
        OCC_CUDA_TRY(cudaMemsetAsync(P.hdr, 0, sizeof(TilePlanHeader), st));
    }
    if (job) {
        launch_raycast<false, true>(g, tg, P, d_recs, 1, P.stamps, d_counters, have_items, *job, st);
    } else {
        RouteJob none = {};
        launch_raycast<false, false>(g, tg, P, d_recs, 1, P.stamps, d_counters, have_items, none, st);
    }
    if (after_fused) OCC_CUDA_TRY(cudaEventRecord(after_fused, st));
    if (have_items) {
        ProfileScope ps(K_TILE_RESOLVE, st);
        k_home_resolve<false><<<device_sm_count() * 8, kTT, 0, st>>>(g, tg, P.active, P.hdr, P.stamps, d_grid);
    }
    OCC_CUDA_TRY(cudaGetLastError());
    return OCCGRID_OK;
}

}
```

Baseline: 674.2 billion.

## Fuse tile binning, planning and run placement into one persistent cooperative kernel with TMA ring

Replaces the three-kernel front end for raw packets (bin, single-CTA tile plan, place runs) with one persistent cooperative kernel. Packet records are staged through a three-stage shared-memory ring filled by cp.async.bulk with mbarrier waits, and a grid-wide barrier counter in the workspace header slot separates binning, planning and run placement. The aim is to remove two kernel launches and their gaps and to overlap packet loads with decoding. The cost is cooperative-launch constraints, a grid limited to resident CTAs, and the tile plan running inside the fused kernel.

```diff
diff --git a/distributed-multi-agent-slam-swarm-robotics-system_b200/_native.py b/distributed-multi-agent-slam-swarm-robotics-system_b200/_native.py
--- a/distributed-multi-agent-slam-swarm-robotics-system_b200/_native.py
+++ b/distributed-multi-agent-slam-swarm-robotics-system_b200/_native.py
@@ -8,7 +8,7 @@
 CSRC = os.path.join(PKG_DIR, 'csrc')
 LIB_PATH = os.path.join(PKG_DIR, 'liboccgrid_b200.so')
 SOURCES = ['occgrid_integrate.cu', 'occgrid_tiled.cu', 'occgrid_route.cu', 'occgrid_band.cu', 'mapmerge.cu', 'frontier.cu', 'icp.cu', 'render.cu', 'map_fuse.cu', 'frontier_assign.cu', 'slam_chain.cpp']
-HEADERS = ['common.cuh', 'beam_expand.cuh', 'block_ops.cuh', 'sincos_dd.cuh', os.path.join('..', '..', 'include', 'occgrid_b200.h')]
+HEADERS = ['common.cuh', 'beam_expand.cuh', 'block_ops.cuh', 'bulk_copy.cuh', 'sincos_dd.cuh', os.path.join('..', '..', 'include', 'occgrid_b200.h')]
 
 STRATEGY = {'auto': -1, 'global_atomic': 0, 'tiled': 1}
 COUNTER_NAMES = ('packets', 'accepted', 'dropped', 'bad_pose', 'beams', 'hits', 'updates', 'slowpath',
diff --git a/distributed-multi-agent-slam-swarm-robotics-system_b200/csrc/bulk_copy.cuh b/distributed-multi-agent-slam-swarm-robotics-system_b200/csrc/bulk_copy.cuh
--- /dev/null
+++ b/distributed-multi-agent-slam-swarm-robotics-system_b200/csrc/bulk_copy.cuh
@@ -0,0 +1,33 @@
+#pragma once
+#include <cuda_runtime.h>
+
+namespace occ {
+
+__device__ __forceinline__ unsigned int smem_u32(const void* p) { return (unsigned int)__cvta_generic_to_shared(p); }
+
+__device__ __forceinline__ void mbar_init(unsigned long long* bar, unsigned int count) {
+    asm volatile("mbarrier.init.shared::cta.b64 [%0], %1;" ::"r"(smem_u32(bar)), "r"(count) : "memory");
+}
+__device__ __forceinline__ void mbar_init_fence() {
+    asm volatile("fence.mbarrier_init.release.cluster;" ::: "memory");
+    asm volatile("fence.proxy.async.shared::cta;" ::: "memory");
+}
+__device__ __forceinline__ void fence_proxy_async_smem() { asm volatile("fence.proxy.async.shared::cta;" ::: "memory"); }
+__device__ __forceinline__ void mbar_expect_tx(unsigned long long* bar, unsigned int bytes) {
+    asm volatile("mbarrier.arrive.expect_tx.shared::cta.b64 _, [%0], %1;" ::"r"(smem_u32(bar)), "r"(bytes) : "memory");
+}
+__device__ __forceinline__ void mbar_wait(unsigned long long* bar, unsigned int parity) {
+    asm volatile(
+        "{\n\t.reg .pred p;\n\t"
+        "WAIT_%=:\n\t"
+        "mbarrier.try_wait.parity.shared::cta.b64 p, [%0], %1;\n\t"
+        "@p bra DONE_%=;\n\t"
+        "bra WAIT_%=;\n\t"
+        "DONE_%=:\n\t}" ::"r"(smem_u32(bar)), "r"(parity) : "memory");
+}
+__device__ __forceinline__ void bulk_load(void* smem_dst, const void* gmem_src, unsigned int bytes, unsigned long long* bar) {
+    asm volatile("cp.async.bulk.shared::cluster.global.mbarrier::complete_tx::bytes [%0], [%1], %2, [%3];"
+                 ::"r"(smem_u32(smem_dst)), "l"(gmem_src), "r"(bytes), "r"(smem_u32(bar)) : "memory");
+}
+
+}
diff --git a/distributed-multi-agent-slam-swarm-robotics-system_b200/csrc/common.cuh b/distributed-multi-agent-slam-swarm-robotics-system_b200/csrc/common.cuh
--- a/distributed-multi-agent-slam-swarm-robotics-system_b200/csrc/common.cuh
+++ b/distributed-multi-agent-slam-swarm-robotics-system_b200/csrc/common.cuh
@@ -7,6 +7,7 @@
 #include "../../include/occgrid_b200.h"
 #include "beam_expand.cuh"
 #include "block_ops.cuh"
+#include "bulk_copy.cuh"
 
 namespace occ {
 
diff --git a/distributed-multi-agent-slam-swarm-robotics-system_b200/csrc/mapmerge.cu b/distributed-multi-agent-slam-swarm-robotics-system_b200/csrc/mapmerge.cu
--- a/distributed-multi-agent-slam-swarm-robotics-system_b200/csrc/mapmerge.cu
+++ b/distributed-multi-agent-slam-swarm-robotics-system_b200/csrc/mapmerge.cu
@@ -179,28 +179,6 @@
 constexpr int kScanCtasPerSm = 3;
 constexpr int kScanStageBytes = kChunk;
 
-__device__ __forceinline__ unsigned int smem_u32(const void* p) { return (unsigned int)__cvta_generic_to_shared(p); }
-
-__device__ __forceinline__ void mbar_init(unsigned long long* bar, unsigned int count) {
-    asm volatile("mbarrier.init.shared::cta.b64 [%0], %1;" ::"r"(smem_u32(bar)), "r"(count) : "memory");
-}
-__device__ __forceinline__ void mbar_expect_tx(unsigned long long* bar, unsigned int bytes) {
-    asm volatile("mbarrier.arrive.expect_tx.shared::cta.b64 _, [%0], %1;" ::"r"(smem_u32(bar)), "r"(bytes) : "memory");
-}
-__device__ __forceinline__ void mbar_wait(unsigned long long* bar, unsigned int parity) {
-    asm volatile(
-        "{\n\t.reg .pred p;\n\t"
-        "WAIT_%=:\n\t"
-        "mbarrier.try_wait.parity.shared::cta.b64 p, [%0], %1;\n\t"
-        "@p bra DONE_%=;\n\t"
-        "bra WAIT_%=;\n\t"
-        "DONE_%=:\n\t}" ::"r"(smem_u32(bar)), "r"(parity) : "memory");
-}
-__device__ __forceinline__ void bulk_load(void* smem_dst, const void* gmem_src, unsigned int bytes, unsigned long long* bar) {
-    asm volatile("cp.async.bulk.shared::cluster.global.mbarrier::complete_tx::bytes [%0], [%1], %2, [%3];"
-                 ::"r"(smem_u32(smem_dst)), "l"(gmem_src), "r"(bytes), "r"(smem_u32(bar)) : "memory");
-}
-
 __device__ __forceinline__ unsigned int occupied_bits16(uint4 v) {
     const unsigned int w[4] = {v.x, v.y, v.z, v.w};
     unsigned int bits = 0;
@@ -232,8 +210,7 @@
     };
     if (threadIdx.x == 0) {
         for (int s = 0; s < kScanStages; ++s) mbar_init(&s_full[s], 1);
-        asm volatile("fence.mbarrier_init.release.cluster;" ::: "memory");
-        asm volatile("fence.proxy.async.shared::cta;" ::: "memory");
+        mbar_init_fence();
     }
     if (threadIdx.x < kScanStages) s_cnt[threadIdx.x] = 0u;
     __syncthreads();
diff --git a/distributed-multi-agent-slam-swarm-robotics-system_b200/csrc/occgrid_tiled.cu b/distributed-multi-agent-slam-swarm-robotics-system_b200/csrc/occgrid_tiled.cu
--- a/distributed-multi-agent-slam-swarm-robotics-system_b200/csrc/occgrid_tiled.cu
+++ b/distributed-multi-agent-slam-swarm-robotics-system_b200/csrc/occgrid_tiled.cu
@@ -72,166 +72,290 @@
         if (key[j] != kEmpty) s_vals[j * kTT + threadIdx.x] = off[j] + base[j];
 }
 
-constexpr size_t kBinSmem = (size_t)kTT * kMaxRecStride + 2 * kHash * sizeof(unsigned int) + kPkPerCta * sizeof(unsigned short);
+__device__ __forceinline__ void plan_tiles(unsigned int* __restrict__ tile_count, unsigned int* __restrict__ tile_offset,
+                                           unsigned int* __restrict__ tile_cursor, uint4* __restrict__ items, unsigned int max_items,
+                                           const unsigned int* __restrict__ active, unsigned long long max_records,
+                                           TilePlanHeader* __restrict__ hdr, uint64_t* counters, unsigned int target_items) {
+    __shared__ unsigned int s_warp[2][33];
+    __shared__ unsigned int s_carry[2];
+    __shared__ unsigned int s_total;
+    if (threadIdx.x < 2) s_carry[threadIdx.x] = 0;
+    if (threadIdx.x == 0) s_total = 0;
+    __syncthreads();
+    const int n_active = (int)__ldcg(&hdr->active_count);
+    const int lane = threadIdx.x & 31, warp = threadIdx.x >> 5, n_warps = (int)(blockDim.x >> 5);
+    {
+        unsigned int mine = 0;
+        for (int i = threadIdx.x; i < n_active; i += blockDim.x) mine += __ldcg(tile_count + __ldcg(active + i));
+#pragma unroll
+        for (int o = 16; o > 0; o >>= 1) mine += __shfl_xor_sync(0xffffffffu, mine, o);
+        if (lane == 0 && mine) atomicAdd(&s_total, mine);
+    }
+    __syncthreads();
+    unsigned int chunk_pk = (s_total / target_items + kChunkMin) / kChunkMin * kChunkMin;
+    chunk_pk = chunk_pk > (unsigned int)kChunkPk ? (unsigned int)kChunkPk : chunk_pk;
+    for (int start = 0; start < n_active; start += blockDim.x) {
+        const int i = start + threadIdx.x;
+        const unsigned int t = i < n_active ? __ldcg(active + i) : 0u;
+        const unsigned int cnt = i < n_active ? __ldcg(tile_count + t) : 0u;
+        unsigned int v[2] = {cnt, (cnt + chunk_pk - 1) / chunk_pk};
+        unsigned int ex[2];
+#pragma unroll
+        for (int j = 0; j < 2; ++j) {
+            unsigned int inc = v[j];
+#pragma unroll
+            for (int o = 1; o < 32; o <<= 1) { unsigned int u = __shfl_up_sync(0xffffffffu, inc, o); if (lane >= o) inc += u; }
+            if (lane == 31) s_warp[j][warp] = inc;
+            ex[j] = inc - v[j];
+        }
+        __syncthreads();
+        if (warp < 2) {
+            unsigned int w = lane < n_warps ? s_warp[warp][lane] : 0u, winc = w;
+#pragma unroll
+            for (int o = 1; o < 32; o <<= 1) { unsigned int u = __shfl_up_sync(0xffffffffu, winc, o); if (lane >= o) winc += u; }
+            s_warp[warp][lane] = winc - w;
+            if (lane == 31) s_warp[warp][32] = winc;
+        }
+        __syncthreads();
+        const unsigned int off = s_carry[0] + s_warp[0][warp] + ex[0];
+        const unsigned int item0 = s_carry[1] + s_warp[1][warp] + ex[1];
+        if (i < n_active) {
+            tile_offset[t] = off;
+            tile_cursor[t] = 0u;
+            tile_count[t] = 0u;
+            for (unsigned int j = 0; j < v[1]; ++j) {
+                const unsigned int b = off + j * chunk_pk;
+                const unsigned int e = min(off + cnt, b + chunk_pk);
+                if (item0 + j < max_items) items[item0 + j] = make_uint4(t, b, e, 0u);
+            }
+        }
+        __syncthreads();
+        if (threadIdx.x < 2) s_carry[threadIdx.x] += s_warp[threadIdx.x][32];
+        __syncthreads();
+    }
+    if (threadIdx.x == 0) {
+        TilePlanHeader h;
+        h.total_records = s_carry[0];
+        h.n_items = s_carry[1];
+        h.n_active = (unsigned int)n_active;
+        h.work_counter = 0;
+        h.resolve_counter = 0;
+        h.active_count = 0;
+        h.overflow = (s_carry[0] > max_records || s_carry[1] > max_items) ? 1u : 0u;
+        if (h.overflow) { h.n_items = 0; h.n_active = 0; }
+        h.pad = 0;
+        *hdr = h;
+        if (counters) atomicAdd(reinterpret_cast<unsigned long long*>(counters) + OCCGRID_C_RECORDS, (unsigned long long)s_carry[0]);
+    }
+}
+
+constexpr int kFrontStages = 3;
+constexpr size_t kFrontHashBytes = 2 * kHash * sizeof(unsigned int) + kPkPerCta * sizeof(unsigned short);
+static_assert(kFrontHashBytes % 128 == 0, "the staging ring starts 128-byte aligned");
+static_assert(kTT * 41 >= kPkPerCta * (int)sizeof(unsigned int), "a stage holds a segment's local-bin list");
 constexpr unsigned int kNoSlot = 0xffffu;
 
+inline size_t front_smem(int stride) { return kFrontHashBytes + (size_t)kFrontStages * kTT * stride; }
+
+struct FrontArgs {
+    Geom g; TileGeom tg;
+    const uint8_t* pkts; long long n; int stride;
+    const int32_t* agent_idx; const double* drift; const double* agent_off; int n_agents;
+    unsigned int *tile_count, *tile_offset, *tile_cursor, *active, *local_bins, *seg_count, *bins;
+    uint2* runs;
+    PoseRec* recs;
+    uint4* items;
+    unsigned int max_items, target_items;
+    unsigned long long max_records;
+    TilePlanHeader* hdr;
+    unsigned int* bar;
+    uint64_t* counters;
+};
+
 template <bool kMaps = false>
-__global__ void __launch_bounds__(kTT)
-k_home_bin(Geom g, TileGeom tg, const uint8_t* __restrict__ pkts, long long n, int stride,
-           const int32_t* __restrict__ agent_idx, const double* __restrict__ drift,
-           const double* __restrict__ agent_off, int n_agents,
-           unsigned int* __restrict__ tile_count, PoseRec* __restrict__ recs, unsigned int* __restrict__ local_bins, uint2* __restrict__ runs,
-           unsigned int* __restrict__ seg_count, unsigned int* __restrict__ active, TilePlanHeader* __restrict__ hdr,
-           uint64_t* counters) {
-    extern __shared__ __align__(16) uint8_t s_bin[];
-    uint8_t* const s_rec = s_bin;
-    unsigned int* const s_keys = reinterpret_cast<unsigned int*>(s_bin + kTT * kMaxRecStride);
+__global__ void __launch_bounds__(kTT, 3)
+k_tile_front(const FrontArgs A) {
+    extern __shared__ __align__(128) uint8_t s_front[];
+    unsigned int* const s_keys = reinterpret_cast<unsigned int*>(s_front);
     unsigned int* const s_vals = s_keys + kHash;
     unsigned short* const s_slot = reinterpret_cast<unsigned short*>(s_vals + kHash);
+    uint8_t* const s_ring = s_front + kFrontHashBytes;
+    __shared__ __align__(8) unsigned long long s_full[kFrontStages];
     __shared__ unsigned int s_wsum[kTT / 32];
+    const long long n = A.n;
+    const int stride = A.stride;
+    const unsigned int stage_bytes = (unsigned int)(kTT * stride);
+    const long long n_segs = (n + kPkPerCta - 1) / kPkPerCta;
+    const bool bulk = (reinterpret_cast<uintptr_t>(A.pkts) & 15) == 0;
+    auto sub_first = [&](long long q) {
+        return ((long long)blockIdx.x + (q / kSub) * gridDim.x) * kPkPerCta + (q % kSub) * kTT;
+    };
+    auto issue = [&](long long q) {
+        const long long first = sub_first(q);
+        if (!bulk || first >= n) return;
+        const unsigned int bytes = (unsigned int)(min((long long)kTT, n - first) * stride) & ~15u;
+        const int st = (int)(q % kFrontStages);
+        fence_proxy_async_smem();
+        mbar_expect_tx(&s_full[st], bytes);
+        bulk_load(s_ring + (size_t)st * stage_bytes, A.pkts + (size_t)first * stride, bytes, &s_full[st]);
+    };
+    if (threadIdx.x == 0) {
+        for (int s = 0; s < kFrontStages; ++s) mbar_init(&s_full[s], 1);
+        mbar_init_fence();
+    }
     for (int i = threadIdx.x; i < kHash; i += kTT) { s_keys[i] = kEmpty; s_vals[i] = 0u; }
+    __syncthreads();
+    if (threadIdx.x == 0)
+        for (int q = 0; q < kFrontStages - 1; ++q) issue(q);
     unsigned long long c[OCCGRID_C_HITS + 1] = {};
-    const long long cta_first = (long long)blockIdx.x * kPkPerCta;
-    constexpr int kVec = (kTT * kMaxRecStride / 16 + kTT - 1) / kTT;
-    uint4 pre[kVec];
-    auto prefetch = [&](int sub) {
-        const long long first = cta_first + (long long)sub * kTT;
-        const long long left = n - first;
-        const size_t bytes = left <= 0 ? 0 : (size_t)min((long long)kTT, left) * stride;
-        const uint4* s4 = reinterpret_cast<const uint4*>(pkts + (size_t)first * stride);
-#pragma unroll
-        for (int j = 0; j < kVec; ++j) {
-            const size_t i = (size_t)j * kTT + threadIdx.x;
-            pre[j] = (i * 16 + 16 <= bytes) ? __ldg(s4 + i) : make_uint4(0u, 0u, 0u, 0u);
-        }
-    };
-    const bool vec_ok = (reinterpret_cast<uintptr_t>(pkts) & 15) == 0 && ((kTT * stride) & 15) == 0;
-    if (vec_ok) prefetch(0);
-    for (int sub = 0; sub < kSub; ++sub) {
-        const long long first = cta_first + (long long)sub * kTT;
-        if (first >= n) break;
-        const int count = (int)min((long long)kTT, n - first);
-        __syncthreads();
-        if (vec_ok) {
-            const size_t bytes = (size_t)count * stride;
-            uint4* d4 = reinterpret_cast<uint4*>(s_rec);
-#pragma unroll
-            for (int j = 0; j < kVec; ++j) {
-                const size_t i = (size_t)j * kTT + threadIdx.x;
-                if (i * 16 + 16 <= bytes) d4[i] = pre[j];
-            }
-            for (size_t i = (bytes / 16) * 16 + threadIdx.x; i < bytes; i += kTT) s_rec[i] = __ldg(pkts + (size_t)first * stride + i);
-            if (sub + 1 < kSub) prefetch(sub + 1);
-        } else {
-            stage_records(pkts + (size_t)first * stride, (size_t)count * stride, s_rec);
-        }
-        __syncthreads();
-        if ((int)threadIdx.x < count) {
-            const long long k = first + threadIdx.x;
-            double rx, ry, ryaw;
-            float dist[4];
-            c[OCCGRID_C_PACKETS] += 1;
-            unsigned int slot = kNoSlot;
-            int agent = 1;
-            const int st = decode_packet(s_rec + threadIdx.x * stride, k, agent_idx, drift, agent_off, n_agents, &rx, &ry, &ryaw, dist,
-                                         kMaps ? &agent : nullptr);
-            if (st == PKT_DROPPED) c[OCCGRID_C_DROPPED] += 1;
-            else if (st == PKT_BAD_POSE) c[OCCGRID_C_BAD_POSE] += 1;
-            else {
-                c[OCCGRID_C_ACCEPTED] += 1;
-                c[OCCGRID_C_BEAMS] += 4;
-#pragma unroll
-                for (int s = 0; s < 4; ++s) {
-                    const double d = (double)dist[s];
-                    c[OCCGRID_C_HITS] += (OCC_MIN_DIST_M < d && d <= OCC_MAX_DIST_M) ? 1 : 0;
+    long long q = 0;
+    for (long long seg = blockIdx.x; seg < n_segs; seg += gridDim.x, q += kSub) {
+        const long long seg0 = seg * kPkPerCta;
+        for (int sub = 0; sub < kSub; ++sub) {
+            const long long first = seg0 + (long long)sub * kTT;
+            if (first >= n) break;
+            const int count = (int)min((long long)kTT, n - first);
+            const long long qs = q + sub;
+            uint8_t* const s_rec = s_ring + (size_t)(qs % kFrontStages) * stage_bytes;
+            if (bulk) {
+                const unsigned int bytes = (unsigned int)(count * stride);
+                mbar_wait(&s_full[qs % kFrontStages], (unsigned int)((qs / kFrontStages) & 1));
+                for (unsigned int i = (bytes & ~15u) + threadIdx.x; i < bytes; i += kTT) s_rec[i] = __ldg(A.pkts + (size_t)first * stride + i);
+            } else {
+                stage_records(A.pkts + (size_t)first * stride, (size_t)count * stride, s_rec);
+            }
+            __syncthreads();
+            if (threadIdx.x == 0) issue(qs + kFrontStages - 1);
+            if ((int)threadIdx.x < count) {
+                const long long k = first + threadIdx.x;
+                double rx, ry, ryaw;
+                float dist[4];
+                c[OCCGRID_C_PACKETS] += 1;
+                unsigned int slot = kNoSlot;
+                int agent = 1;
+                const int st = decode_packet(s_rec + threadIdx.x * stride, k, A.agent_idx, A.drift, A.agent_off, A.n_agents, &rx, &ry,
+                                             &ryaw, dist, kMaps ? &agent : nullptr);
+                if (st == PKT_DROPPED) c[OCCGRID_C_DROPPED] += 1;
+                else if (st == PKT_BAD_POSE) c[OCCGRID_C_BAD_POSE] += 1;
+                else {
+                    c[OCCGRID_C_ACCEPTED] += 1;
+                    c[OCCGRID_C_BEAMS] += 4;
+#pragma unroll
+                    for (int s = 0; s < 4; ++s) {
+                        const double d = (double)dist[s];
+                        c[OCCGRID_C_HITS] += (OCC_MIN_DIST_M < d && d <= OCC_MAX_DIST_M) ? 1 : 0;
+                    }
+                    int tile = home_tile(A.g, A.tg, rx, ry);
+                    if (kMaps && tile >= 0) tile += (agent - 1) * A.tg.n_tiles;
+                    if (tile >= 0) {
+                        slot = (unsigned int)hash_insert(s_keys, (unsigned int)tile);
+                        atomicAdd(&s_vals[slot], 1u);
+                        PoseRec r;
+                        r.rx = rx; r.ry = ry; r.yaw = (float)ryaw;
+                        r.d[0] = dist[0]; r.d[1] = dist[1]; r.d[2] = dist[2]; r.d[3] = dist[3];
+                        r.k = (unsigned int)k;
+                        r.tile = tile; r.pad = 0;
+                        A.recs[k] = r;
+                    }
                 }
-                int tile = home_tile(g, tg, rx, ry);
-                if (kMaps && tile >= 0) tile += (agent - 1) * tg.n_tiles;
-                if (tile >= 0) {
-                    slot = (unsigned int)hash_insert(s_keys, (unsigned int)tile);
-                    atomicAdd(&s_vals[slot], 1u);
-                    PoseRec r;
-                    r.rx = rx; r.ry = ry; r.yaw = (float)ryaw;
-                    r.d[0] = dist[0]; r.d[1] = dist[1]; r.d[2] = dist[2]; r.d[3] = dist[3];
-                    r.k = (unsigned int)k;
-                    r.tile = tile; r.pad = 0;
-                    recs[k] = r;
-                }
-            }
-            s_slot[sub * kTT + threadIdx.x] = (unsigned short)slot;
-        }
+                s_slot[sub * kTT + threadIdx.x] = (unsigned short)slot;
+            }
+        }
+        __syncthreads();
+        unsigned int key[kHashPerThread], rank[kHashPerThread];
+#pragma unroll
+        for (int j = 0; j < kHashPerThread; ++j) {
+            const int i = j * kTT + threadIdx.x;
+            key[j] = s_keys[i];
+            rank[j] = 0u;
+            if (key[j] != kEmpty) rank[j] = atomicAdd(&A.tile_count[key[j]], s_vals[i]);
+        }
+        const int lane = threadIdx.x & 31, warp = threadIdx.x >> 5;
+        unsigned int mine = 0u;
+#pragma unroll
+        for (int j = 0; j < kHashPerThread; ++j) mine += key[j] != kEmpty ? s_vals[j * kTT + threadIdx.x] + 0x10000u : 0u;
+        unsigned int inc = mine;
+#pragma unroll
+        for (int o = 1; o < 32; o <<= 1) { const unsigned int u = __shfl_up_sync(0xffffffffu, inc, o); if (lane >= o) inc += u; }
+        if (lane == 31) s_wsum[warp] = inc;
+        __syncthreads();
+        unsigned int pos = inc - mine, n_local = 0u;
+#pragma unroll
+        for (int w = 0; w < kTT / 32; ++w) {
+            pos += w < warp ? s_wsum[w] : 0u;
+            n_local += s_wsum[w];
+        }
+        n_local &= 0xffffu;
+        if (threadIdx.x == 0) A.seg_count[seg] = n_local;
+#pragma unroll
+        for (int j = 0; j < kHashPerThread; ++j) {
+            if (key[j] == kEmpty) continue;
+            const int i = j * kTT + threadIdx.x;
+            const unsigned int run = pos >> 16, begin = pos & 0xffffu;
+            A.runs[seg0 + run] = make_uint2(key[j], rank[j] - begin);
+            pos += s_vals[i] + 0x10000u;
+            s_keys[i] = run;
+            s_vals[i] = begin;
+            if (rank[j] == 0u) A.active[atomicAdd(&A.hdr->active_count, 1u)] = key[j];
+        }
+        __syncthreads();
+        unsigned int* const s_local = reinterpret_cast<unsigned int*>(s_ring + (size_t)((q + kSub - 1) % kFrontStages) * stage_bytes);
+        const int n_seg = (int)min((long long)kPkPerCta, n - seg0);
+        for (int j = threadIdx.x; j < n_seg; j += kTT) {
+            const unsigned int slot = s_slot[j];
+            if (slot != kNoSlot) s_local[atomicAdd(&s_vals[slot], 1u)] = (s_keys[slot] << 16) | (unsigned int)j;
+        }
+        __syncthreads();
+        for (unsigned int j = threadIdx.x; j < n_local; j += kTT) A.local_bins[seg0 + j] = s_local[j];
+        for (int i = threadIdx.x; i < kHash; i += kTT) { s_keys[i] = kEmpty; s_vals[i] = 0u; }
+        fence_proxy_async_smem();
     }
     __syncthreads();
-    unsigned int key[kHashPerThread], rank[kHashPerThread];
-#pragma unroll
-    for (int j = 0; j < kHashPerThread; ++j) {
-        const int i = j * kTT + threadIdx.x;
-        key[j] = s_keys[i];
-        rank[j] = 0u;
-        if (key[j] != kEmpty) rank[j] = atomicAdd(&tile_count[key[j]], s_vals[i]);
-    }
-    const int lane = threadIdx.x & 31, warp = threadIdx.x >> 5;
-    unsigned int mine = 0u;
-#pragma unroll
-    for (int j = 0; j < kHashPerThread; ++j) mine += key[j] != kEmpty ? s_vals[j * kTT + threadIdx.x] + 0x10000u : 0u;
-    unsigned int inc = mine;
-#pragma unroll
-    for (int o = 1; o < 32; o <<= 1) { const unsigned int u = __shfl_up_sync(0xffffffffu, inc, o); if (lane >= o) inc += u; }
-    if (lane == 31) s_wsum[warp] = inc;
-    __syncthreads();
-    unsigned int pos = inc - mine, n_local = 0u;
-#pragma unroll
-    for (int w = 0; w < kTT / 32; ++w) {
-        pos += w < warp ? s_wsum[w] : 0u;
-        n_local += s_wsum[w];
-    }
-    n_local &= 0xffffu;
-    if (threadIdx.x == 0) seg_count[blockIdx.x] = n_local;
-    const size_t seg0 = (size_t)blockIdx.x * kPkPerCta;
-#pragma unroll
-    for (int j = 0; j < kHashPerThread; ++j) {
-        if (key[j] == kEmpty) continue;
-        const int i = j * kTT + threadIdx.x;
-        const unsigned int run = pos >> 16, begin = pos & 0xffffu;
-        runs[seg0 + run] = make_uint2(key[j], rank[j] - begin);
-        pos += s_vals[i] + 0x10000u;
-        s_keys[i] = run;
-        s_vals[i] = begin;
-        if (rank[j] == 0u) active[atomicAdd(&hdr->active_count, 1u)] = key[j];
-    }
-    __syncthreads();
-    unsigned int* const s_local = reinterpret_cast<unsigned int*>(s_rec);
-    const int n_seg = (int)min((long long)kPkPerCta, n - (long long)seg0);
-    for (int j = threadIdx.x; j < n_seg; j += kTT) {
-        const unsigned int slot = s_slot[j];
-        if (slot != kNoSlot) s_local[atomicAdd(&s_vals[slot], 1u)] = (s_keys[slot] << 16) | (unsigned int)j;
-    }
-    __syncthreads();
-    for (unsigned int j = threadIdx.x; j < n_local; j += kTT) local_bins[seg0 + j] = s_local[j];
-    __syncthreads();
-    block_add_counters(c, reinterpret_cast<unsigned long long*>(s_rec), counters);
-}
-
-__global__ void __launch_bounds__(kTT)
-k_place_runs(const unsigned int* __restrict__ local_bins, const uint2* __restrict__ runs, const unsigned int* __restrict__ seg_count,
-             const unsigned int* __restrict__ tile_offset, const TilePlanHeader* __restrict__ hdr, unsigned int* __restrict__ bins) {
-    if (hdr->overflow) return;
-    const size_t seg0 = (size_t)blockIdx.x * kPkPerCta;
-    const int n_local = (int)seg_count[blockIdx.x];
-    unsigned int e[kSub], off[kSub];
-    uint2 d[kSub];
-#pragma unroll
-    for (int sub = 0; sub < kSub; ++sub) {
-        const int j = sub * kTT + threadIdx.x;
-        e[sub] = j < n_local ? local_bins[seg0 + j] : kEmpty;
-    }
-#pragma unroll
-    for (int sub = 0; sub < kSub; ++sub) d[sub] = e[sub] != kEmpty ? runs[seg0 + (e[sub] >> 16)] : make_uint2(0u, 0u);
-#pragma unroll
-    for (int sub = 0; sub < kSub; ++sub) off[sub] = e[sub] != kEmpty ? tile_offset[d[sub].x] : 0u;
-#pragma unroll
-    for (int sub = 0; sub < kSub; ++sub)
-        if (e[sub] != kEmpty) bins[off[sub] + d[sub].y + (unsigned int)(sub * kTT + threadIdx.x)] = (unsigned int)(seg0 + (e[sub] & 0xffffu));
+    block_add_counters(c, reinterpret_cast<unsigned long long*>(s_keys), A.counters);
+
+    unsigned int target = 0;
+    int* const abort_flag = reinterpret_cast<int*>(A.bar + 4);
+    bool alive = grid_barrier(A.bar, target, abort_flag);
+    if (blockIdx.x == 0) {
+        if (alive) {
+            plan_tiles(A.tile_count, A.tile_offset, A.tile_cursor, A.items, A.max_items, A.active, A.max_records, A.hdr, A.counters,
+                       A.target_items);
+        } else if (threadIdx.x == 0) {
+            TilePlanHeader h = {};
+            h.overflow = 1u;
+            *A.hdr = h;
+        }
+    }
+    int overflow = 1;
+    if (alive)
+        alive = grid_barrier(A.bar, target, abort_flag, &overflow,
+                             [&] { return (int)*reinterpret_cast<volatile unsigned int*>(&A.hdr->overflow); });
+    if (!alive) return;
+    if (!overflow) {
+        for (long long seg = blockIdx.x; seg < n_segs; seg += gridDim.x) {
+            const size_t seg0 = (size_t)seg * kPkPerCta;
+            const int n_local = (int)__ldcg(A.seg_count + seg);
+            unsigned int e[kSub], off[kSub];
+            uint2 d[kSub];
+#pragma unroll
+            for (int sub = 0; sub < kSub; ++sub) {
+                const int j = sub * kTT + threadIdx.x;
+                e[sub] = j < n_local ? __ldcg(A.local_bins + seg0 + j) : kEmpty;
+            }
+#pragma unroll
+            for (int sub = 0; sub < kSub; ++sub) d[sub] = e[sub] != kEmpty ? __ldcg(A.runs + seg0 + (e[sub] >> 16)) : make_uint2(0u, 0u);
+#pragma unroll
+            for (int sub = 0; sub < kSub; ++sub) off[sub] = e[sub] != kEmpty ? __ldcg(A.tile_offset + d[sub].x) : 0u;
+#pragma unroll
+            for (int sub = 0; sub < kSub; ++sub)
+                if (e[sub] != kEmpty) A.bins[off[sub] + d[sub].y + (unsigned int)(sub * kTT + threadIdx.x)] = (unsigned int)(seg0 + (e[sub] & 0xffffu));
+        }
+    }
+    if (threadIdx.x == 0 && atomicAdd(A.bar + 1, 1u) == gridDim.x - 1u) {
+        A.bar[0] = 0u; A.bar[2] = 0u; A.bar[3] = 0u;
+        __threadfence();
+        A.bar[1] = 0u;
+    }
 }
 
 __device__ __forceinline__ int chunk_valid(const SegInfo& seg, long long chunk, long long* addr0) {
@@ -353,77 +477,7 @@
             unsigned int* __restrict__ tile_cursor, uint4* __restrict__ items, unsigned int max_items,
             const unsigned int* __restrict__ active, unsigned long long max_records, TilePlanHeader* __restrict__ hdr,
             uint64_t* counters, unsigned int target_items) {
-    __shared__ unsigned int s_warp[2][33];
-    __shared__ unsigned int s_carry[2];
-    __shared__ unsigned int s_total;
-    if (threadIdx.x < 2) s_carry[threadIdx.x] = 0;
-    if (threadIdx.x == 0) s_total = 0;
-    __syncthreads();
-    const int n_active = (int)hdr->active_count;
-    const int lane = threadIdx.x & 31, warp = threadIdx.x >> 5;
-    {
-        unsigned int mine = 0;
-        for (int i = threadIdx.x; i < n_active; i += blockDim.x) mine += tile_count[active[i]];
-#pragma unroll
-        for (int o = 16; o > 0; o >>= 1) mine += __shfl_xor_sync(0xffffffffu, mine, o);
-        if (lane == 0 && mine) atomicAdd(&s_total, mine);
-    }
-    __syncthreads();
-    unsigned int chunk_pk = (s_total / target_items + kChunkMin) / kChunkMin * kChunkMin;
-    chunk_pk = chunk_pk > (unsigned int)kChunkPk ? (unsigned int)kChunkPk : chunk_pk;
-    for (int start = 0; start < n_active; start += blockDim.x) {
-        const int i = start + threadIdx.x;
-        const unsigned int t = i < n_active ? active[i] : 0u;
-        const unsigned int cnt = i < n_active ? tile_count[t] : 0u;
-        unsigned int v[2] = {cnt, (cnt + chunk_pk - 1) / chunk_pk};
-        unsigned int ex[2];
-#pragma unroll
-        for (int j = 0; j < 2; ++j) {
-            unsigned int inc = v[j];
-#pragma unroll
-            for (int o = 1; o < 32; o <<= 1) { unsigned int u = __shfl_up_sync(0xffffffffu, inc, o); if (lane >= o) inc += u; }
-            if (lane == 31) s_warp[j][warp] = inc;
-            ex[j] = inc - v[j];
-        }
-        __syncthreads();
-        if (warp < 2) {
-            unsigned int w = s_warp[warp][lane], winc = w;
-#pragma unroll
-            for (int o = 1; o < 32; o <<= 1) { unsigned int u = __shfl_up_sync(0xffffffffu, winc, o); if (lane >= o) winc += u; }
-            s_warp[warp][lane] = winc - w;
-            if (lane == 31) s_warp[warp][32] = winc;
-        }
-        __syncthreads();
-        const unsigned int off = s_carry[0] + s_warp[0][warp] + ex[0];
-        const unsigned int item0 = s_carry[1] + s_warp[1][warp] + ex[1];
-        if (i < n_active) {
-            tile_offset[t] = off;
-            tile_cursor[t] = 0u;
-            tile_count[t] = 0u;
-            for (unsigned int j = 0; j < v[1]; ++j) {
-                const unsigned int b = off + j * chunk_pk;
-                const unsigned int e = min(off + cnt, b + chunk_pk);
-                if (item0 + j < max_items) items[item0 + j] = make_uint4(t, b, e, 0u);
-            }
-        }
-        __syncthreads();
-        if (threadIdx.x < 2) s_carry[threadIdx.x] += s_warp[threadIdx.x][32];
-        __syncthreads();
-    }
-    if (threadIdx.x == 0) {
-        TilePlanHeader h;
-        h.total_records = s_carry[0];
-        h.n_items = s_carry[1];
-        h.n_active = (unsigned int)n_active;
-        h.work_counter = 0;
-        h.resolve_counter = 0;
-        h.active_count = 0;
-        h.overflow = (s_carry[0] > max_records || s_carry[1] > max_items) ? 1u : 0u;
-        if (h.overflow) { h.n_items = 0; h.n_active = 0; }
-        h.pad = 0;
-        *hdr = h;
-        if (counters) atomicAdd(reinterpret_cast<unsigned long long*>(counters) + OCCGRID_C_RECORDS, (unsigned long long)s_carry[0]);
-    }
+    plan_tiles(tile_count, tile_offset, tile_cursor, items, max_items, active, max_records, hdr, counters, target_items);
 }
 
 __device__ __noinline__ void draw_beam_smem(unsigned int* __restrict__ s_win, int side, int pitch, int x, int y,
@@ -989,11 +1043,14 @@
 void set_raycast_cta_cap(int cap) { g_raycast_cta_cap = cap < 0 ? 0 : cap; }
 
 struct TiledLayout {
-    size_t off_stamps, off_count, off_offset, off_cursor, off_active, off_hdr, off_items, off_ids, off_bins, off_local, off_runs,
-        off_segs, off_recs, total;
+    size_t off_stamps, off_count, off_offset, off_cursor, off_active, off_hdr, off_bar, off_items, off_ids, off_bins, off_local,
+        off_runs, off_segs, off_recs, total;
     unsigned long long max_records;
     unsigned int max_items;
 };
+
+constexpr size_t kBarOffset = 64;
+static_assert(sizeof(TilePlanHeader) <= kBarOffset && kBarOffset + 5 * sizeof(unsigned int) <= 256, "header slot layout");
 
 static TiledLayout tiled_layout(const occgrid_geom* geom, int64_t max_records, bool packets, int n_maps = 1) {
     TiledLayout L;
@@ -1009,7 +1066,7 @@
     L.off_offset = o; o += align_up((n_keys + 1) * 4, 256);
     L.off_cursor = o; o += align_up((n_keys + 1) * 4, 256);
     L.off_active = o; o += align_up((n_keys + 1) * 4, 256);
-    L.off_hdr = o;    o += 256;
+    L.off_hdr = o;    L.off_bar = o + kBarOffset; o += 256;
     L.off_items = o;  o += align_up((size_t)L.max_items * sizeof(uint4), 256);
     L.off_ids = o;    o += packets ? 0 : align_up((size_t)L.max_records * sizeof(int), 256);
     L.off_bins = o;   o += align_up((size_t)L.max_records * sizeof(unsigned int), 256);
@@ -1035,7 +1092,7 @@
 }
 
 struct TiledPtrs {
-    unsigned int *stamps, *tile_count, *tile_offset, *tile_cursor, *active, *bins, *local_bins, *seg_count;
+    unsigned int *stamps, *tile_count, *tile_offset, *tile_cursor, *active, *bins, *local_bins, *seg_count, *bar;
     TilePlanHeader* hdr;
     uint4* items;
     int* tile_ids;
@@ -1052,6 +1109,7 @@
     p.tile_cursor = reinterpret_cast<unsigned int*>(ws + L.off_cursor);
     p.active = reinterpret_cast<unsigned int*>(ws + L.off_active);
     p.hdr = reinterpret_cast<TilePlanHeader*>(ws + L.off_hdr);
+    p.bar = reinterpret_cast<unsigned int*>(ws + L.off_bar);
     p.items = reinterpret_cast<uint4*>(ws + L.off_items);
     p.bins = reinterpret_cast<unsigned int*>(ws + L.off_bins);
     p.tile_ids = reinterpret_cast<int*>(ws + L.off_ids);
@@ -1112,31 +1170,49 @@
     const PoseRec* recs = d_poses ? d_poses : P.recs;
     const Geom g = to_geom(geom);
     const TileGeom tg = tile_geom(geom);
-    const unsigned int blocks = (unsigned int)((n + kPkPerCta - 1) / kPkPerCta);
-    SegInfo seg;
-    seg.n_segs = 1; seg.seg_cap = (unsigned int)align_up((size_t)n, kSegChunk); seg.d_counts = nullptr; seg.host_count = (unsigned int)n;
-    const long long n_chunks = (n + kSegChunk - 1) / kSegChunk;
-    {
-        ProfileScope ps(K_TILE_COUNT, st);
-        if (d_poses) {
+    if (d_poses) {
+        SegInfo seg;
+        seg.n_segs = 1; seg.seg_cap = (unsigned int)align_up((size_t)n, kSegChunk); seg.d_counts = nullptr; seg.host_count = (unsigned int)n;
+        const long long n_chunks = (n + kSegChunk - 1) / kSegChunk;
+        {
+            ProfileScope ps(K_TILE_COUNT, st);
             k_home_count_poses<<<grid_chunks(n_chunks), kTT, 0, st>>>(g, tg, d_poses, nullptr, seg, n_chunks, 0, P.tile_count, P.tile_ids, P.active,
                                                                       P.hdr, d_counters);
-        } else {
-            const auto bin = maps ? k_home_bin<true> : k_home_bin<false>;
-            OCC_CUDA_TRY(cudaFuncSetAttribute(bin, cudaFuncAttributeMaxDynamicSharedMemorySize, (int)kBinSmem));
-            bin<<<blocks, kTT, kBinSmem, st>>>(g, tg, batch.pkts, n, batch.stride, batch.agent_idx, batch.drift, batch.agent_off, batch.n_agents,
-                                               P.tile_count, P.recs, P.local_bins, P.runs, P.seg_count, P.active, P.hdr, d_counters);
-        }
-    }
-    {
-        ProfileScope ps(K_TILE_SCAN, st);
-        k_tile_plan<<<1, 1024, 0, st>>>(P.tile_count, P.tile_offset, P.tile_cursor, P.items, L.max_items, P.active, L.max_records, P.hdr,
-                                        d_counters, plan_target_items());
-    }
-    {
-        ProfileScope ps(K_TILE_SCATTER, st);
-        if (d_poses) k_home_scatter_segs<<<grid_chunks(n_chunks), kTT, 0, st>>>(seg, n_chunks, P.tile_ids, P.tile_offset, P.tile_cursor, P.hdr, P.bins);
-        else         k_place_runs<<<blocks, kTT, 0, st>>>(P.local_bins, P.runs, P.seg_count, P.tile_offset, P.hdr, P.bins);
+        }
+        {
+            ProfileScope ps(K_TILE_SCAN, st);
+            k_tile_plan<<<1, 1024, 0, st>>>(P.tile_count, P.tile_offset, P.tile_cursor, P.items, L.max_items, P.active, L.max_records, P.hdr,
+                                            d_counters, plan_target_items());
+        }
+        {
+            ProfileScope ps(K_TILE_SCATTER, st);
+            k_home_scatter_segs<<<grid_chunks(n_chunks), kTT, 0, st>>>(seg, n_chunks, P.tile_ids, P.tile_offset, P.tile_cursor, P.hdr, P.bins);
+        }
+    } else {
+        FrontArgs A;
+        A.g = g; A.tg = tg;
+        A.pkts = batch.pkts; A.n = n; A.stride = batch.stride;
+        A.agent_idx = batch.agent_idx; A.drift = batch.drift; A.agent_off = batch.agent_off; A.n_agents = batch.n_agents;
+        A.tile_count = P.tile_count; A.tile_offset = P.tile_offset; A.tile_cursor = P.tile_cursor; A.active = P.active;
+        A.local_bins = P.local_bins; A.seg_count = P.seg_count; A.bins = P.bins; A.runs = P.runs; A.recs = P.recs; A.items = P.items;
+        A.max_items = L.max_items; A.target_items = plan_target_items(); A.max_records = L.max_records;
+        A.hdr = P.hdr; A.bar = P.bar; A.counters = d_counters;
+        const void* front = maps ? (const void*)k_tile_front<true> : (const void*)k_tile_front<false>;
+        const size_t smem = front_smem(batch.stride);
+        static thread_local size_t configured[2] = {0, 0};
+        static thread_local int ctas_per_sm[2] = {0, 0};
+        if (configured[maps] != smem) {
+            OCC_CUDA_TRY(cudaFuncSetAttribute(front, cudaFuncAttributeMaxDynamicSharedMemorySize, (int)front_smem(kMaxRecStride)));
+            OCC_CUDA_TRY(cudaOccupancyMaxActiveBlocksPerMultiprocessor(&ctas_per_sm[maps], front, kTT, smem));
+            if (ctas_per_sm[maps] < 1) { set_last_error("TILED: the bin kernel does not fit on an SM (%zu B of shared memory)", smem); return OCCGRID_E_CUDA; }
+            configured[maps] = smem;
+        }
+        const long long n_segs = (n + kPkPerCta - 1) / kPkPerCta;
+        const long long resident = (long long)device_sm_count() * ctas_per_sm[maps];
+        const unsigned int grid = (unsigned int)(n_segs < resident ? n_segs : resident);
+        void* args[] = {&A};
+        ProfileScope ps(K_TILE_COUNT, st);
+        OCC_CUDA_TRY(cudaLaunchCooperativeKernel(front, dim3(grid), dim3(kTT), args, smem, st));
     }
     RouteJob none = {};
     unsigned int* const plane = kind == Output::kCounts ? reinterpret_cast<unsigned int*>(d_out) : P.stamps;
```

Result: no change. 676.1 billion (median of 6 runs) (+0.3%).
